# serviceberry3/weiner_slamit_v2

Measured on AMD Instinct MI355X. Metric: frames/sec ORB extract+match @640x480x8lvl, higher is better.
Workload: dtype u8; 1 GPU; BASELINE configs[1]: 640x480 8-level ORB extract (1000 features, FAST 20/7) + brute-force 256-bit Hamming best/second match vs the stream's previous frame; 256 independent streams per GPU per step; distinct_frame_pairs_per_gpu=16, parallelism=streams sharded over 1 GPU(s), no data-path collective

## Files before the change

include/slamit.h:

```cpp
#ifndef SLAMIT_H
#define SLAMIT_H

#include <stddef.h>
#include <stdint.h>

#ifdef __cplusplus
extern "C" {
#endif

#define SLAMIT_OK 0
#define SLAMIT_ERR_ARG (-1)
#define SLAMIT_ERR_DEVICE (-2)
#define SLAMIT_ERR_CAPACITY (-3)
#define SLAMIT_ERR_STATE (-4)

#define SLAMIT_DESC_BYTES 32
#define SLAMIT_EDGE_THRESHOLD 19

typedef struct slamit_kp {
    float x, y;
    float size;
    float angle;
    float response;
    int32_t octave;
    int32_t class_id;
} slamit_kp;


typedef struct slamit_orb_params {
    int32_t nfeatures;
    float scale_factor;
    int32_t nlevels;
    int32_t ini_th_fast;
    int32_t min_th_fast;
    int32_t width, height;
    int32_t max_batch;
} slamit_orb_params;

#define SLAMIT_MAX_LEVELS 16

typedef struct slamit_orb slamit_orb;

int slamit_orb_create(const slamit_orb_params* params, int device, slamit_orb** out);
void slamit_orb_destroy(slamit_orb* h);

int slamit_orb_tables(const slamit_orb* h, float* scale, float* inv_scale, float* sigma2,
                      float* inv_sigma2, int32_t* features_per_level);

int slamit_orb_max_keypoints(const slamit_orb* h);

int slamit_orb_extract(slamit_orb* h, const uint8_t* gray, size_t stride, slamit_kp* kps,
                       uint8_t* desc, int cap, int* n_out);

int slamit_orb_extract_batch(slamit_orb* h, const uint8_t* gray, size_t stride,
                             size_t frame_stride, int nframes, slamit_kp* kps, uint8_t* desc,
                             int cap, int* n_out);

int slamit_orb_extract_batch_dev(slamit_orb* h, const uint8_t* d_gray, size_t stride,
                                 size_t frame_stride, int nframes, slamit_kp* d_kps,
                                 uint8_t* d_desc, int cap, int32_t* d_n_out, void* stream);

#define SLAMIT_ORB_STAGES 6
int slamit_orb_profile(slamit_orb* h, int enable, float* stage_ms, int32_t* stage_calls, int nstages);

int slamit_orb_level(slamit_orb* h, int frame, int level, uint8_t* dst, size_t dst_bytes, int* w,
                     int* h_out);

int slamit_orb_debug_candidates(slamit_orb* h, int frame, int level, int32_t* xys, int cap,
                                int* n_out);
int slamit_orb_debug_blurred(slamit_orb* h, int frame, int level, uint8_t* dst, size_t dst_bytes, int* w,
                             int* h_out);


#define SLAMIT_HAMMING_MAX_TRAIN 65535
int slamit_hamming_best2(const uint8_t* q, int nq, const uint8_t* t, int nt, int32_t* best_idx,
                         int32_t* best, int32_t* second);

int slamit_hamming_best2_batch_dev(const uint8_t* d_q, const int32_t* d_nq, size_t q_stride,
                                   const uint8_t* d_t, const int32_t* d_nt, size_t t_stride,
                                   int npairs, int max_n, int32_t* d_best_idx, int32_t* d_best,
                                   int32_t* d_second, size_t out_stride, int device, void* stream);

#define SLAMIT_DISTINCTIVE_MAX 128
int slamit_distinctive_batch(const uint8_t* desc, const int32_t* offsets, int npoints, int32_t* best_idx,
                             int32_t* best_median);

typedef struct slamit_frame_view {
    int32_t n;
    const float* kp_xy;
    const int32_t* kp_octave;
    const uint8_t* desc;
    const uint8_t* kp_taken;
    float min_x, min_y;
    float inv_w, inv_h;
} slamit_frame_view;

typedef struct slamit_search_queries {
    int32_t m;
    const float* uvr;
    const int32_t* level_min;
    const int32_t* level_max;
    const uint8_t* desc;
    const uint8_t* valid;
    const uint8_t* takes;
} slamit_search_queries;

typedef struct slamit_search_rule {
    int32_t th_dist;
    int32_t use_ratio;
    float nnratio;
    float chi2_gate;
    float inv_level_sigma2[16];
    int32_t mode;
} slamit_search_rule;

#define SLAMIT_SEARCH_MAX_KP 8191
#define SLAMIT_SEARCH_MAX_CAND 1024
int slamit_guided_search(int device, const slamit_frame_view* frame, const slamit_search_queries* queries,
                         const slamit_search_rule* rule, int32_t* match_kp, int32_t* nmatches, int32_t* best_dist,
                         int32_t* best_level, int32_t* second_dist, int32_t* second_level);

typedef struct slamit_bow_groups {
    int32_t n_groups;
    const int32_t* q_ptr;
    const int32_t* q_idx;
    const int32_t* c_ptr;
    const int32_t* c_idx;
} slamit_bow_groups;

typedef struct slamit_bow_rule {
    int32_t mode;
    int32_t th;
    int32_t th_inclusive;
    float nnratio;
    float F12[9];
    float ex, ey;
    const float* kp1_xy;
    const float* kp2_xy;
    const int32_t* kp2_octave;
    float scale_factor[16];
    float level_sigma2[16];
} slamit_bow_rule;

#define SLAMIT_BOW_MAX_GROUP 2048
int slamit_bow_search(int device, const uint8_t* desc1, int32_t n1, const uint8_t* valid1, const uint8_t* desc2, int32_t n2,
                      const uint8_t* valid2, const slamit_bow_groups* groups, const slamit_bow_rule* rule, int32_t* match12,
                      int32_t* dist12, int32_t* nmatches);

#define SLAMIT_VOC_MAX_K 20
#define SLAMIT_VOC_MAX_L 10
#define SLAMIT_VOC_MAX_FEATURES 8191

typedef struct slamit_voc_desc {
    int32_t k, L;
    int32_t scoring;
    int32_t weighting;
    int32_t n_nodes;
    const int32_t* parent;
    const uint8_t* is_leaf;
    const uint8_t* desc;
    const double* weight;
} slamit_voc_desc;

typedef struct slamit_voc slamit_voc;

int slamit_voc_create(const slamit_voc_desc* desc, int device, slamit_voc** out);
int slamit_voc_load_text(const char* path, int device, slamit_voc** out);
void slamit_voc_destroy(slamit_voc* v);
int slamit_voc_info(const slamit_voc* v, int32_t* k, int32_t* L, int32_t* n_nodes, int32_t* n_words);

int slamit_voc_transform(const slamit_voc* v, const uint8_t* desc, int n, int levelsup, int32_t* word_id, int32_t* node_id,
                         int32_t* bow_n, int32_t* bow_word, double* bow_value, int32_t* fv_n, int32_t* fv_node,
                         int32_t* fv_ptr, int32_t* fv_items);

size_t slamit_voc_transform_workspace(int nframes, int cap);
int slamit_voc_transform_batch_dev(const slamit_voc* v, const uint8_t* d_desc, const int32_t* d_n, int cap, int nframes,
                                   int levelsup, int32_t* d_word_id, int32_t* d_node_id, int32_t* d_bow_n,
                                   int32_t* d_bow_word, double* d_bow_value, int32_t* d_fv_n, int32_t* d_fv_node,
                                   int32_t* d_fv_ptr, int32_t* d_fv_items, void* d_workspace, size_t workspace_bytes,
                                   void* stream);

typedef struct slamit_kfdb slamit_kfdb;

int slamit_kfdb_create(int max_kf, int max_words, int device, slamit_kfdb** out);
void slamit_kfdb_destroy(slamit_kfdb* db);
int slamit_kfdb_clear(slamit_kfdb* db);
int slamit_kfdb_info(const slamit_kfdb* db, int32_t* max_kf, int32_t* max_words, int32_t* n_live);
int slamit_kfdb_add(slamit_kfdb* db, const int32_t* bow_word, const double* bow_value, int n, int32_t* slot);
int slamit_kfdb_add_dev(slamit_kfdb* db, const int32_t* d_bow_n, const int32_t* d_bow_word, const double* d_bow_value,
                        void* stream, int32_t* slot);
int slamit_kfdb_erase(slamit_kfdb* db, int slot);
int slamit_kfdb_query(slamit_kfdb* db, const int32_t* bow_word, const double* bow_value, int n, int32_t* common,
                      int32_t* first_word, int64_t* seq, double* score);
int slamit_kfdb_query_batch_dev(slamit_kfdb* db, const int32_t* d_bow_n, const int32_t* d_bow_word, const double* d_bow_value,
                                int cap, int nq, int32_t* d_common, int32_t* d_first_word, double* d_score, void* stream);

typedef struct slamit_camera {
    float fx, fy, cx, cy;
    float k1, k2, p1, p2, k3;
} slamit_camera;

#define SLAMIT_FRAME_GRID_COLS 64
#define SLAMIT_FRAME_GRID_ROWS 48
#define SLAMIT_FRAME_GRID_CELLS (SLAMIT_FRAME_GRID_COLS * SLAMIT_FRAME_GRID_ROWS)
#define SLAMIT_FRAME_MAX_KP 30000

int slamit_undistort_points(int device, const slamit_camera* cam, const float* xy_in, int n, float* xy_out);

int slamit_frame_finish(int device, const slamit_camera* cam, const slamit_kp* kps, int n, float min_x, float min_y,
                        float inv_w, float inv_h, slamit_kp* kps_un, int32_t* cell_start, int32_t* cell_items);

int slamit_frame_finish_batch_dev(int device, const slamit_camera* cam, const slamit_kp* d_kps, const int32_t* d_n, int cap,
                                  int nframes, float min_x, float min_y, float inv_w, float inv_h, slamit_kp* d_kps_un,
                                  int32_t* d_cell_start, int32_t* d_cell_items, void* stream);

#define SLAMIT_SEARCH_BATCH_CAND 128
typedef struct slamit_search_batch {
    int32_t nframes, kp_cap, q_cap;
    const int32_t* d_n;
    const slamit_kp* d_kps_un;
    const uint8_t* d_desc;
    const uint8_t* d_kp_taken;
    float min_x, min_y, inv_w, inv_h;
    const int32_t* d_m;
// ... 256 lines not shown
```

weiner_slamit_v2_amd/api.py:

```python
import ctypes as C
import math
import os

import numpy as np

HERE = os.path.dirname(os.path.abspath(__file__))
LIB_PATH = os.environ.get("SLAMIT_LIB", os.path.join(HERE, "libslamit_hip.so"))

KP_DTYPE = np.dtype(
    [("x", "<f4"), ("y", "<f4"), ("size", "<f4"), ("angle", "<f4"), ("response", "<f4"),
     ("octave", "<i4"), ("class_id", "<i4")]
)

MAX_ITS = 32


class SlamitError(RuntimeError):
    pass


class OrbParams(C.Structure):
    _fields_ = [("nfeatures", C.c_int32), ("scale_factor", C.c_float), ("nlevels", C.c_int32),
                ("ini_th_fast", C.c_int32), ("min_th_fast", C.c_int32), ("width", C.c_int32),
                ("height", C.c_int32), ("max_batch", C.c_int32)]
# ... 18 lines not shown
                ("lambda_", (C.c_double * MAX_ITS) * 2), ("trials", (C.c_int32 * MAX_ITS) * 2),
                ("chi2_init", C.c_double * 2)]


class BaResult(C.Structure):
    _fields_ = [("kf_pose", C.c_void_p), ("pt_xyz", C.c_void_p), ("edge_chi2", C.c_void_p),
                ("edge_outlier", C.c_void_p), ("edge_stage1_outlier", C.c_void_p), ("stats", C.c_void_p)]


class FrameView(C.Structure):
    _fields_ = [("n", C.c_int32), ("kp_xy", C.c_void_p), ("kp_octave", C.c_void_p), ("desc", C.c_void_p),
                ("kp_taken", C.c_void_p), ("min_x", C.c_float), ("min_y", C.c_float), ("inv_w", C.c_float),
                ("inv_h", C.c_float)]


class SearchQueries(C.Structure):
    _fields_ = [("m", C.c_int32), ("uvr", C.c_void_p), ("level_min", C.c_void_p), ("level_max", C.c_void_p),
                ("desc", C.c_void_p), ("valid", C.c_void_p), ("takes", C.c_void_p)]


class SearchRule(C.Structure):
    _fields_ = [("th_dist", C.c_int32), ("use_ratio", C.c_int32), ("nnratio", C.c_float), ("chi2_gate", C.c_float),
                ("inv_level_sigma2", C.c_float * 16), ("mode", C.c_int32)]


def _search_rule(th_dist, use_ratio, nnratio, chi2_gate=0.0, inv_level_sigma2=None, mode=0):
    sig = [1.0] * 16
    if inv_level_sigma2 is not None:
        for i, v in enumerate(list(inv_level_sigma2)[:16]):
            sig[i] = float(v)
    return SearchRule(int(th_dist), int(bool(use_ratio)), float(nnratio), float(chi2_gate), (C.c_float * 16)(*sig), int(mode))


class BowGroups(C.Structure):
    _fields_ = [("n_groups", C.c_int32), ("q_ptr", C.c_void_p), ("q_idx", C.c_void_p), ("c_ptr", C.c_void_p), ("c_idx", C.c_void_p)]


class BowRule(C.Structure):
    _fields_ = [("mode", C.c_int32), ("th", C.c_int32), ("th_inclusive", C.c_int32), ("nnratio", C.c_float),
                ("F12", C.c_float * 9), ("ex", C.c_float), ("ey", C.c_float), ("kp1_xy", C.c_void_p), ("kp2_xy", C.c_void_p),
                ("kp2_octave", C.c_void_p), ("scale_factor", C.c_float * 16), ("level_sigma2", C.c_float * 16)]


class Sim3Problem(C.Structure):
    _fields_ = [("n", C.c_int32), ("p1", C.c_void_p), ("p2", C.c_void_p), ("obs1", C.c_void_p), ("obs2", C.c_void_p),
                ("inv_sigma2_1", C.c_void_p), ("inv_sigma2_2", C.c_void_p), ("intr1", C.c_double * 4), ("intr2", C.c_double * 4),
                ("r12", C.c_double * 9), ("t12", C.c_double * 3), ("s12", C.c_double), ("th2", C.c_double), ("fix_scale", C.c_int32)]


class Sim3Result(C.Structure):
    _fields_ = [("r12", C.c_double * 9), ("t12", C.c_double * 3), ("s12", C.c_double), ("inlier", C.c_void_p), ("n_inliers", C.c_int32),
                ("n_its", C.c_int32 * 2), ("chi2", C.c_double * 2)]


class Sim3RansacProblem(C.Structure):
    _fields_ = [("n", C.c_int32), ("x1", C.c_void_p), ("x2", C.c_void_p), ("max_err1", C.c_void_p), ("max_err2", C.c_void_p),
                ("intr1", C.c_float * 4), ("intr2", C.c_float * 4), ("fix_scale", C.c_int32), ("n_hyp", C.c_int32), ("triples", C.c_void_p)]


class Sim3RansacResult(C.Structure):
    _fields_ = [("t12", C.c_void_p), ("n_inliers", C.c_void_p), ("inlier_bits", C.c_void_p)]


SIM3_RANSAC_MAX_N, SIM3_RANSAC_MAX_HYP = 8192, 1024


class TriangulateProblem(C.Structure):
    _fields_ = [("Tcw1", C.c_float * 12), ("Tcw2", C.c_float * 12), ("intr1", C.c_float * 6), ("intr2", C.c_float * 6), ("n", C.c_int32),
                ("n_levels", C.c_int32), ("kp1_xy", C.c_void_p), ("kp2_xy", C.c_void_p), ("octave1", C.c_void_p), ("octave2", C.c_void_p),
                ("scale_factors1", C.c_void_p), ("level_sigma2_1", C.c_void_p), ("scale_factors2", C.c_void_p), ("level_sigma2_2", C.c_void_p),
                ("ratio_factor", C.c_float)]


class TriangulateResult(C.Structure):
    _fields_ = [("status", C.c_void_p), ("x3d", C.c_void_p), ("n_accepted", C.c_int32)]


TRIANGULATE_MAX_N, MAX_LEVELS = 8192, 16


class FrustumFrame(C.Structure):
    _fields_ = [("Rcw", C.c_float * 9), ("tcw", C.c_float * 3), ("Ow", C.c_float * 3), ("fx", C.c_float), ("fy", C.c_float), ("cx", C.c_float),
                ("cy", C.c_float), ("bf", C.c_float), ("min_x", C.c_float), ("max_x", C.c_float), ("min_y", C.c_float), ("max_y", C.c_float),
                ("view_cos_limit", C.c_float), ("log_scale_factor", C.c_float), ("th", C.c_float), ("n_levels", C.c_int32),
                ("scale_factors", C.c_float * 16)]


class FrustumProblem(C.Structure):
    _fields_ = [("frame", FrustumFrame), ("n", C.c_int32), ("pos", C.c_void_p), ("normal", C.c_void_p), ("max_dist", C.c_void_p),
                ("min_dist", C.c_void_p), ("skip", C.c_void_p)]


class FrustumResult(C.Structure):
    _fields_ = [("status", C.c_void_p), ("proj", C.c_void_p), ("view_cos", C.c_void_p), ("level", C.c_void_p), ("uvr", C.c_void_p),
                ("level_min", C.c_void_p), ("level_max", C.c_void_p), ("valid", C.c_void_p), ("n_in_view", C.c_int32)]


class FrustumBatchRec(C.Structure):
    _fields_ = [("nframes", C.c_int32), ("q_cap", C.c_int32), ("d_frames", C.c_void_p), ("d_m", C.c_void_p), ("d_pos", C.c_void_p),
                ("d_normal", C.c_void_p), ("d_max_dist", C.c_void_p), ("d_min_dist", C.c_void_p), ("d_skip", C.c_void_p), ("d_uvr", C.c_void_p),
                ("d_level_min", C.c_void_p), ("d_level_max", C.c_void_p), ("d_valid", C.c_void_p), ("d_status", C.c_void_p),
                ("d_proj", C.c_void_p), ("d_view_cos", C.c_void_p), ("d_level", C.c_void_p), ("d_n_in_view", C.c_void_p)]


FRUSTUM_MAX_N = 65536
FRUSTUM_FRAME_DTYPE = np.dtype([("Rcw", "<f4", 9), ("tcw", "<f4", 3), ("Ow", "<f4", 3), ("fx", "<f4"), ("fy", "<f4"), ("cx", "<f4"), ("cy", "<f4"),
                                ("bf", "<f4"), ("min_x", "<f4"), ("max_x", "<f4"), ("min_y", "<f4"), ("max_y", "<f4"), ("view_cos_limit", "<f4"),
                                ("log_scale_factor", "<f4"), ("th", "<f4"), ("n_levels", "<i4"), ("scale_factors", "<f4", 16)])


class VocDesc(C.Structure):
    _fields_ = [("k", C.c_int32), ("L", C.c_int32), ("scoring", C.c_int32), ("weighting", C.c_int32), ("n_nodes", C.c_int32),
                ("parent", C.c_void_p), ("is_leaf", C.c_void_p), ("desc", C.c_void_p), ("weight", C.c_void_p)]


VOC_MAX_K, VOC_MAX_L, VOC_MAX_FEATURES = 20, 10, 8191


class SearchBatch(C.Structure):
    _fields_ = [("nframes", C.c_int32), ("kp_cap", C.c_int32), ("q_cap", C.c_int32), ("d_n", C.c_void_p),
                ("d_kps_un", C.c_void_p), ("d_desc", C.c_void_p), ("d_kp_taken", C.c_void_p), ("min_x", C.c_float),
                ("min_y", C.c_float), ("inv_w", C.c_float), ("inv_h", C.c_float), ("d_m", C.c_void_p), ("d_uvr", C.c_void_p),
                ("d_level_min", C.c_void_p), ("d_level_max", C.c_void_p), ("d_qdesc", C.c_void_p), ("d_valid", C.c_void_p),
                ("d_takes", C.c_void_p)]


class Camera(C.Structure):
    _fields_ = [("fx", C.c_float), ("fy", C.c_float), ("cx", C.c_float), ("cy", C.c_float), ("k1", C.c_float),
                ("k2", C.c_float), ("p1", C.c_float), ("p2", C.c_float), ("k3", C.c_float)]


class BaProfile(C.Structure):
    _fields_ = [("phase_ms", C.c_double * 5), ("slots", C.c_int32), ("nwin", C.c_int32), ("schur_exec_mflop", C.c_double)]


BA_PHASES = ("linearize", "schur", "solve", "update", "residuals")


class PoseProblem(C.Structure):
    _fields_ = [("n", C.c_int32), ("pose", C.c_void_p), ("intr", C.c_void_p), ("xw", C.c_void_p),
                ("uv", C.c_void_p), ("inv_sigma2", C.c_void_p), ("ur", C.c_void_p), ("bf", C.c_double)]


class PoseResult(C.Structure):
    _fields_ = [("pose", C.c_void_p), ("outlier", C.c_void_p), ("n_inliers", C.c_int32),
                ("n_its", C.c_int32 * 4), ("chi2", C.c_double * 4)]


_lib = None

EXPORTS = [
    "slamit_orb_create", "slamit_orb_destroy", "slamit_orb_tables", "slamit_orb_max_keypoints",
    "slamit_orb_extract", "slamit_orb_extract_batch", "slamit_orb_extract_batch_dev", "slamit_orb_level",
    "slamit_orb_debug_candidates", "slamit_orb_debug_blurred", "slamit_orb_profile", "slamit_hamming_best2", "slamit_hamming_best2_batch_dev",
    "slamit_hamming_matrix", "slamit_distinctive_batch", "slamit_guided_search", "slamit_guided_search_workspace", "slamit_guided_search_batch_dev", "slamit_bow_search", "slamit_voc_create", "slamit_voc_load_text", "slamit_voc_destroy", "slamit_voc_info",
    "slamit_voc_transform", "slamit_voc_transform_workspace", "slamit_voc_transform_batch_dev",
    "slamit_kfdb_create", "slamit_kfdb_destroy", "slamit_kfdb_clear", "slamit_kfdb_info", "slamit_kfdb_add", "slamit_kfdb_add_dev", "slamit_kfdb_erase",
    "slamit_kfdb_query", "slamit_kfdb_query_batch_dev", "slamit_undistort_points", "slamit_frame_finish",
    "slamit_frame_finish_batch_dev", "slamit_ba_create", "slamit_ba_create_ex", "slamit_ba_destroy", "slamit_ba_solve",
    "slamit_ba_solve_batch", "slamit_ba_profile", "slamit_ba_profile_read", "slamit_pose_optimize", "slamit_pose_optimize_batch", "slamit_sim3_optimize", "slamit_sim3_optimize_batch", "slamit_sim3_ransac", "slamit_sim3_ransac_batch", "slamit_triangulate", "slamit_triangulate_batch", "slamit_frustum", "slamit_frustum_batch", "slamit_frustum_batch_dev", "slamit_last_error", "slamit_version", "slamit_device_count", "slamit_set_device", "slamit_release_thread_scratch",
]


def lib():
    global _lib
    if _lib is None:
        if not os.path.exists(LIB_PATH):
            raise SlamitError(
                "libslamit_hip.so is not built: run `python -m weiner_slamit_v2_amd.build` "
                "(there is no CPU fallback)")
        try:
            import torch
        except ImportError:
            pass
        L = C.CDLL(LIB_PATH)
        vp, i32, sz = C.c_void_p, C.c_int, C.c_size_t
        L.slamit_orb_create.argtypes = [C.POINTER(OrbParams), i32, C.POINTER(vp)]
        L.slamit_orb_destroy.argtypes = [vp]
        L.slamit_orb_destroy.restype = None
        L.slamit_orb_tables.argtypes = [vp] + [vp] * 5
        L.slamit_orb_max_keypoints.argtypes = [vp]
        L.slamit_orb_extract.argtypes = [vp, vp, sz, vp, vp, i32, vp]
        L.slamit_orb_extract_batch.argtypes = [vp, vp, sz, sz, i32, vp, vp, i32, vp]
        L.slamit_orb_extract_batch_dev.argtypes = [vp, vp, sz, sz, i32, vp, vp, i32, vp, vp]
        L.slamit_orb_level.argtypes = [vp, i32, i32, vp, sz, vp, vp]
        L.slamit_orb_debug_blurred.argtypes = [vp, i32, i32, vp, sz, vp, vp]
        L.slamit_orb_profile.argtypes = [vp, i32, vp, vp, i32]
        L.slamit_orb_debug_candidates.argtypes = [vp, i32, i32, vp, i32, vp]
        L.slamit_hamming_best2.argtypes = [vp, i32, vp, i32, vp, vp, vp]
        L.slamit_hamming_best2_batch_dev.argtypes = [vp, vp, sz, vp, vp, sz, i32, i32, vp, vp, vp, sz, i32, vp]
        L.slamit_hamming_matrix.argtypes = [vp, i32, vp, i32, vp]
        L.slamit_distinctive_batch.argtypes = [vp, vp, i32, vp, vp]
        L.slamit_guided_search.argtypes = [i32, C.POINTER(FrameView), C.POINTER(SearchQueries), C.POINTER(SearchRule),
                                           vp, vp, vp, vp, vp, vp]
        L.slamit_guided_search_workspace.argtypes = [i32, i32]
        L.slamit_guided_search_workspace.restype = sz
        L.slamit_guided_search_batch_dev.argtypes = [i32, C.POINTER(SearchBatch), C.POINTER(SearchRule), vp, vp, vp, vp, sz, vp]
        f32 = C.c_float
        L.slamit_sim3_optimize_batch.argtypes = [i32, i32, C.POINTER(Sim3Problem), C.POINTER(Sim3Result)]
        L.slamit_sim3_optimize.argtypes = [i32, C.POINTER(Sim3Problem), C.POINTER(Sim3Result)]
        L.slamit_sim3_ransac_batch.argtypes = [i32, i32, C.POINTER(Sim3RansacProblem), C.POINTER(Sim3RansacResult)]
        L.slamit_sim3_ransac.argtypes = [i32, C.POINTER(Sim3RansacProblem), C.POINTER(Sim3RansacResult)]
        L.slamit_triangulate_batch.argtypes = [i32, i32, C.POINTER(TriangulateProblem), C.POINTER(TriangulateResult)]
        L.slamit_triangulate.argtypes = [i32, C.POINTER(TriangulateProblem), C.POINTER(TriangulateResult)]
        L.slamit_frustum_batch.argtypes = [i32, i32, C.POINTER(FrustumProblem), C.POINTER(FrustumResult)]
        L.slamit_frustum.argtypes = [i32, C.POINTER(FrustumProblem), C.POINTER(FrustumResult)]
        L.slamit_frustum_batch_dev.argtypes = [i32, C.POINTER(FrustumBatchRec), vp]
        L.slamit_bow_search.argtypes = [i32, vp, i32, vp, vp, i32, vp, C.POINTER(BowGroups), C.POINTER(BowRule), vp, vp, vp]
        L.slamit_voc_create.argtypes = [C.POINTER(VocDesc), i32, C.POINTER(vp)]
        L.slamit_voc_load_text.argtypes = [C.c_char_p, i32, C.POINTER(vp)]
        L.slamit_voc_destroy.argtypes = [vp]
        L.slamit_voc_destroy.restype = None
        L.slamit_voc_info.argtypes = [vp, vp, vp, vp, vp]
        L.slamit_voc_transform.argtypes = [vp, vp, i32, i32] + [vp] * 9
        L.slamit_voc_transform_workspace.argtypes = [i32, i32]
        L.slamit_voc_transform_workspace.restype = sz
        L.slamit_voc_transform_batch_dev.argtypes = [vp, vp, vp, i32, i32, i32] + [vp] * 9 + [vp, sz, vp]
        L.slamit_kfdb_create.argtypes = [i32, i32, i32, C.POINTER(vp)]
        L.slamit_kfdb_destroy.argtypes = [vp]
        L.slamit_kfdb_destroy.restype = None
        L.slamit_kfdb_clear.argtypes = [vp]
        L.slamit_kfdb_info.argtypes = [vp, vp, vp, vp]
        L.slamit_kfdb_add.argtypes = [vp, vp, vp, i32, vp]
        L.slamit_kfdb_add_dev.argtypes = [vp, vp, vp, vp, vp, vp]
        L.slamit_kfdb_erase.argtypes = [vp, i32]
        L.slamit_kfdb_query.argtypes = [vp, vp, vp, i32, vp, vp, vp, vp]
        L.slamit_kfdb_query_batch_dev.argtypes = [vp, vp, vp, vp, i32, i32, vp, vp, vp, vp]
        L.slamit_undistort_points.argtypes = [i32, C.POINTER(Camera), vp, i32, vp]
        L.slamit_frame_finish.argtypes = [i32, C.POINTER(Camera), vp, i32, f32, f32, f32, f32, vp, vp, vp]
        L.slamit_frame_finish_batch_dev.argtypes = [i32, C.POINTER(Camera), vp, vp, i32, i32, f32, f32, f32, f32, vp, vp, vp, vp]
        if hasattr(L, "slamit_ba_create"):
            L.slamit_ba_create.argtypes = [i32, i32, i32, i32, i32, C.POINTER(vp)]
            if hasattr(L, "slamit_ba_create_ex"):
                L.slamit_ba_create_ex.argtypes = [i32, i32, i32, i32, i32, i32, C.POINTER(vp)]
            L.slamit_ba_destroy.argtypes = [vp]
            L.slamit_ba_destroy.restype = None
            L.slamit_ba_solve.argtypes = [vp, C.POINTER(BaProblem), C.POINTER(BaOpts), C.POINTER(BaResult)]
            L.slamit_ba_solve_batch.argtypes = [vp, i32, C.POINTER(BaProblem), C.POINTER(BaOpts), C.POINTER(BaResult)]
            if hasattr(L, "slamit_ba_profile"):
                L.slamit_ba_profile.argtypes = [vp, i32]
                L.slamit_ba_profile_read.argtypes = [vp, C.POINTER(BaProfile)]
        if hasattr(L, "slamit_pose_optimize_batch"):
            L.slamit_pose_optimize_batch.argtypes = [i32, i32, C.POINTER(PoseProblem), C.POINTER(PoseResult)]
            L.slamit_pose_optimize.argtypes = [i32, C.POINTER(PoseProblem), C.POINTER(PoseResult)]
        L.slamit_last_error.restype = C.c_char_p
        L.slamit_version.restype = C.c_char_p
        _lib = L
    return _lib


def _check(rc, what):
    if rc != 0:
        raise SlamitError("%s failed (%d): %s" % (what, rc, lib().slamit_last_error().decode()))


def device_count():
    return lib().slamit_device_count()


def _np_ptr(a):
    return a.ctypes.data_as(C.c_void_p)


class ORBextractor:

    def __init__(self, nfeatures=1000, scaleFactor=1.2, nlevels=8, iniThFAST=20, minThFAST=7,
                 device=0, max_batch=1):
        self.params = (int(nfeatures), float(scaleFactor), int(nlevels), int(iniThFAST), int(minThFAST))
        self.device = device
        self.max_batch = max_batch
        self._h = None
        self._geom = None

    def _bind(self, width, height, batch=1):
        if self._h is not None and self._geom == (width, height) and batch <= self.max_batch:
            return
        self.close()
        self.max_batch = max(self.max_batch, batch)
        p = OrbParams(self.params[0], self.params[1], self.params[2], self.params[3], self.params[4],
                      width, height, self.max_batch)
        h = C.c_void_p()
        _check(lib().slamit_orb_create(C.byref(p), self.device, C.byref(h)), "slamit_orb_create")
        self._h = h
        self._geom = (width, height)
        self.max_keypoints = lib().slamit_orb_max_keypoints(h)

    def close(self):
        if self._h is not None:
            lib().slamit_orb_destroy(self._h)
            self._h = None

    def __del__(self):
        try:
            self.close()
        except Exception:
            pass

    def GetLevels(self):
        return self.params[2]

    def GetScaleFactor(self):
        return self.params[1]

    def _tables(self):
        if self._h is None:
            self._bind(640, 480)
        n = self.params[2]
        out = [np.zeros(n, np.float32) for _ in range(4)] + [np.zeros(n, np.int32)]
        _check(lib().slamit_orb_tables(self._h, *[_np_ptr(a) for a in out]), "slamit_orb_tables")
        return out

    def GetScaleFactors(self):
        return self._tables()[0]

    def GetInverseScaleFactors(self):
        return self._tables()[1]

    def GetScaleSigmaSquares(self):
        return self._tables()[2]

    def GetInverseScaleSigmaSquares(self):
        return self._tables()[3]

    def features_per_level(self):
        return self._tables()[4]

    def __call__(self, image, mask=None):
        image = np.asarray(image)
        if image.size == 0:
            return np.zeros(0, KP_DTYPE), np.zeros((0, 32), np.uint8)
        assert image.dtype == np.uint8 and image.ndim == 2, "CV_8UC1 expected (ORBextractor.cc:1075)"
        k, d = self.extract_batch(image[None])
        return k[0], d[0]

    def extract_batch(self, frames):
        frames = np.ascontiguousarray(frames, dtype=np.uint8)
        b, hh, ww = frames.shape
        self._bind(ww, hh, b)
        cap = self.max_keypoints
        kps = np.zeros((b, cap), KP_DTYPE)
        desc = np.zeros((b, cap, 32), np.uint8)
        n = np.zeros(b, np.int32)
        _check(lib().slamit_orb_extract_batch(self._h, _np_ptr(frames), ww, ww * hh, b, _np_ptr(kps), _np_ptr(desc),
                                              cap, _np_ptr(n)), "slamit_orb_extract_batch")
        return [kps[i, :n[i]].copy() for i in range(b)], [desc[i, :n[i]].copy() for i in range(b)]

    def extract_batch_dev(self, d_frames, d_kps, d_desc, d_n, stream=None):
        b, hh, ww = d_frames.shape
        self._bind(ww, hh, b)
        cap = d_kps.shape[1]
        _check(lib().slamit_orb_extract_batch_dev(
            self._h, d_frames.data_ptr(), d_frames.stride(1), d_frames.stride(0), b, d_kps.data_ptr(),
            d_desc.data_ptr(), cap, d_n.data_ptr(), stream), "slamit_orb_extract_batch_dev")

    STAGES = ("resize", "fast", "octree", "angle", "blur", "describe")

    def profile(self, enable):
        ms = np.zeros(6, np.float32)
        calls = np.zeros(6, np.int32)
        _check(lib().slamit_orb_profile(self._h, int(enable), _np_ptr(ms), _np_ptr(calls), 6), "slamit_orb_profile")
        return {s: (float(ms[i]), int(calls[i])) for i, s in enumerate(self.STAGES)}

    def level(self, frame, level):
        w, h = C.c_int(), C.c_int()
        _check(lib().slamit_orb_level(self._h, frame, level, None, 0, C.byref(w), C.byref(h)), "slamit_orb_level")
        out = np.zeros((h.value + 38, w.value + 38), np.uint8)
        _check(lib().slamit_orb_level(self._h, frame, level, _np_ptr(out), out.size, C.byref(w), C.byref(h)),
               "slamit_orb_level")
        return out

    def blurred(self, frame, level):
        w, h = C.c_int(), C.c_int()
        _check(lib().slamit_orb_debug_blurred(self._h, frame, level, None, 0, C.byref(w), C.byref(h)), "slamit_orb_debug_blurred")
        out = np.zeros((h.value, w.value), np.uint8)
        _check(lib().slamit_orb_debug_blurred(self._h, frame, level, _np_ptr(out), out.size, C.byref(w), C.byref(h)),
               "slamit_orb_debug_blurred")
        return out

    def debug_candidates(self, frame, level):
        n = C.c_int()
        _check(lib().slamit_orb_debug_candidates(self._h, frame, level, None, 0, C.byref(n)), "debug_candidates")
        out = np.zeros((max(n.value, 1), 3), np.int32)
        _check(lib().slamit_orb_debug_candidates(self._h, frame, level, _np_ptr(out), n.value, C.byref(n)),
               "debug_candidates")
        return out[:n.value]


GRID_COLS, GRID_ROWS = 64, 48


class Frame:

    @staticmethod
    def undistort_points(cam9, xy, device=0):
        cam = Camera(*[float(v) for v in cam9])
        xy = np.ascontiguousarray(xy, np.float32).reshape(-1, 2)
        out = np.zeros_like(xy)
        _check(lib().slamit_undistort_points(device, C.byref(cam), _np_ptr(xy), len(xy), _np_ptr(out)), "slamit_undistort_points")
        return out

    @staticmethod
    def ComputeImageBounds(cam9, cols, rows, device=0):
        f32 = np.float32
        if f32(cam9[4]) != 0:
            m = Frame.undistort_points(cam9, [[0, 0], [cols, 0], [0, rows], [cols, rows]], device)
            b = (min(m[0, 0], m[2, 0]), max(m[1, 0], m[3, 0]), min(m[0, 1], m[1, 1]), max(m[2, 1], m[3, 1]))
        else:
            b = (f32(0), f32(cols), f32(0), f32(rows))
        b = tuple(f32(v) for v in b)
        return b + (f32(GRID_COLS) / f32(b[1] - b[0]), f32(GRID_ROWS) / f32(b[3] - b[2]))

    @staticmethod
    def finish(cam9, kps, min_x, min_y, inv_w, inv_h, device=0):
        cam = Camera(*[float(v) for v in cam9])
        kps = np.ascontiguousarray(kps)
        n = len(kps)
        un = np.zeros(max(n, 1), KP_DTYPE)
        start, items = np.zeros(GRID_COLS * GRID_ROWS + 1, np.int32), np.zeros(max(n, 1), np.int32)
        _check(lib().slamit_frame_finish(device, C.byref(cam), _np_ptr(kps), n, float(min_x), float(min_y), float(inv_w),
                                         float(inv_h), _np_ptr(un), _np_ptr(start), _np_ptr(items)), "slamit_frame_finish")
        return un[:n], start, items[:start[-1]]

    @staticmethod
    def finish_batch_dev(cam9, d_kps, d_n, min_x, min_y, inv_w, inv_h, d_kps_un, d_cell_start, d_cell_items, device=0, stream=None):
        cam = Camera(*[float(v) for v in cam9])
        b, cap = d_kps.shape[0], d_kps.shape[1]
        _check(lib().slamit_frame_finish_batch_dev(device, C.byref(cam), d_kps.data_ptr(), d_n.data_ptr(), cap, b, float(min_x),
                                                   float(min_y), float(inv_w), float(inv_h), d_kps_un.data_ptr(),
                                                   d_cell_start.data_ptr(), d_cell_items.data_ptr(), stream),
               "slamit_frame_finish_batch_dev")


class ORBmatcher:
    TH_HIGH = 100
    TH_LOW = 50
    HISTO_LENGTH = 30

    def __init__(self, nnratio=0.6, checkOri=True):
        self.mfNNratio = nnratio
        self.mbCheckOrientation = checkOri

    @staticmethod
    def DescriptorDistance(a, b):
        a = np.ascontiguousarray(a, np.uint8).reshape(1, 32)
        b = np.ascontiguousarray(b, np.uint8).reshape(1, 32)
        return int(ORBmatcher.distance_matrix(a, b)[0, 0])

    @staticmethod
    def distance_matrix(q, t):
        q = np.ascontiguousarray(q, np.uint8).reshape(-1, 32)
        t = np.ascontiguousarray(t, np.uint8).reshape(-1, 32)
        out = np.zeros((len(q), len(t)), np.uint16)
        _check(lib().slamit_hamming_matrix(_np_ptr(q), len(q), _np_ptr(t), len(t), _np_ptr(out)), "slamit_hamming_matrix")
        return out

    @staticmethod
    def best2(q, t):
        q = np.ascontiguousarray(q, np.uint8).reshape(-1, 32)
        t = np.ascontiguousarray(t, np.uint8).reshape(-1, 32)
        idx, best, second = (np.zeros(len(q), np.int32) for _ in range(3))
        _check(lib().slamit_hamming_best2(_np_ptr(q), len(q), _np_ptr(t), len(t), _np_ptr(idx), _np_ptr(best),
                                          _np_ptr(second)), "slamit_hamming_best2")
        return idx, best, second

    @staticmethod
    def distinctive(desc, offsets):
        desc = np.ascontiguousarray(desc, np.uint8).reshape(-1, 32)
        offsets = np.ascontiguousarray(offsets, np.int32)
        n = len(offsets) - 1
        idx, med = np.zeros(max(n, 1), np.int32), np.zeros(max(n, 1), np.int32)
        _check(lib().slamit_distinctive_batch(_np_ptr(desc), _np_ptr(offsets), n, _np_ptr(idx), _np_ptr(med)),
               "slamit_distinctive_batch")
        return idx[:n], med[:n]

    @staticmethod
    def guided_search(frame, queries, th_dist=100, use_ratio=True, nnratio=0.8, device=0, chi2_gate=0.0, inv_level_sigma2=None, mode=0):
        f = dict(kp_xy=np.ascontiguousarray(frame["kp_xy"], np.float32).reshape(-1, 2),
                 kp_octave=np.ascontiguousarray(frame["kp_octave"], np.int32),
                 desc=np.ascontiguousarray(frame["desc"], np.uint8).reshape(-1, 32),
                 kp_taken=np.ascontiguousarray(frame["kp_taken"], np.uint8))
        uvr = np.ascontiguousarray(queries["uvr"], np.float32).reshape(-1, 3)
        m, n = len(uvr), len(f["kp_xy"])
        q = dict(level_min=np.ascontiguousarray(queries["level_min"], np.int32),
                 level_max=np.ascontiguousarray(queries["level_max"], np.int32),
                 desc=np.ascontiguousarray(queries["desc"], np.uint8).reshape(-1, 32),
                 valid=np.ascontiguousarray(queries.get("valid", np.ones(m)), np.uint8),
                 takes=np.ascontiguousarray(queries.get("takes", np.ones(m)), np.uint8))
        for k, a in list(f.items())[1:]:
            if len(a) != n:
                raise SlamitError("guided_search: frame[%s] has %d rows, expected %d" % (k, len(a), n))
        for k, a in q.items():
            if len(a) != m:
                raise SlamitError("guided_search: queries[%s] has %d rows, expected %d" % (k, len(a), m))
        fv = FrameView(n, _np_ptr(f["kp_xy"]), _np_ptr(f["kp_octave"]), _np_ptr(f["desc"]), _np_ptr(f["kp_taken"]),
                       frame["min_x"], frame["min_y"], frame["inv_w"], frame["inv_h"])
        sq = SearchQueries(m, _np_ptr(uvr), _np_ptr(q["level_min"]), _np_ptr(q["level_max"]), _np_ptr(q["desc"]),
                           _np_ptr(q["valid"]), _np_ptr(q["takes"]))
        rule = _search_rule(th_dist, use_ratio, nnratio, chi2_gate, inv_level_sigma2, mode)
        match = np.full(max(m, 1), -1, np.int32)
        out4 = np.zeros((4, max(m, 1)), np.int32)
        nm = C.c_int32(0)
        _check(lib().slamit_guided_search(device, C.byref(fv), C.byref(sq), C.byref(rule), _np_ptr(match), C.byref(nm),
                                          _np_ptr(out4[0]), _np_ptr(out4[1]), _np_ptr(out4[2]), _np_ptr(out4[3])),
               "slamit_guided_search")
        return match[:m], nm.value, out4[:, :m].T.copy()

    @staticmethod
    def guided_search_batch_dev(t, bounds, th_dist=100, use_ratio=True, nnratio=0.8, device=0, stream=None, chi2_gate=0.0,
                                inv_level_sigma2=None):
        b, kp_cap, q_cap = t["kps_un"].shape[0], t["kps_un"].shape[1], t["uvr"].shape[1]
        sb = SearchBatch(b, kp_cap, q_cap, t["n"].data_ptr(), t["kps_un"].data_ptr(), t["desc"].data_ptr(), t["kp_taken"].data_ptr(),
                         float(bounds[0]), float(bounds[1]), float(bounds[2]), float(bounds[3]), t["m"].data_ptr(), t["uvr"].data_ptr(),
                         t["level_min"].data_ptr(), t["level_max"].data_ptr(), t["qdesc"].data_ptr(), t["valid"].data_ptr(),
                         t["takes"].data_ptr())
        rule = _search_rule(th_dist, use_ratio, nnratio, chi2_gate, inv_level_sigma2)
        out4 = t.get("out4")
        _check(lib().slamit_guided_search_batch_dev(device, C.byref(sb), C.byref(rule), t["match_kp"].data_ptr(), t["nmatches"].data_ptr(),
                                                    out4.data_ptr() if out4 is not None else None, t["workspace"].data_ptr(),
                                                    t["workspace"].numel(), stream), "slamit_guided_search_batch_dev")

    @staticmethod
    def guided_search_workspace(nframes, q_cap):
        return int(lib().slamit_guided_search_workspace(nframes, q_cap))

    @staticmethod
    def search_for_initialization(f1, prev_xy, f2, window=100, nnratio=0.9, th_low=50, device=0):
        o1 = np.ascontiguousarray(f1["kp_octave"], np.int32)
        n1 = len(o1)
        pv = np.ascontiguousarray(prev_xy, np.float32).reshape(-1, 2)
        q = dict(uvr=np.concatenate([pv, np.full((n1, 1), float(window), np.float32)], 1), level_min=np.zeros(n1, np.int32),
                 level_max=np.zeros(n1, np.int32), desc=f1["desc"], valid=(o1 <= 0).astype(np.uint8), takes=np.zeros(n1, np.uint8))
# ... 715 lines not shown
```

weiner_slamit_v2_amd/csrc/orb_api.hip:

```cpp
#include <hip/hip_runtime.h>
#include <math.h>
#include <stdio.h>
#include <stdlib.h>
#include <string.h>

#include <algorithm>
#include <vector>

#include "../../include/slamit.h"
#include "orb_plan.h"
#include "slamit_internal.h"

hipError_t orbk_upload_pattern(hipStream_t st);
void orbk_resize(hipStream_t st, const uint8_t* src, int sw, int sh, size_t sstride, size_t sframe,
                 uint8_t* dst, int dw, int dh, size_t dstride, size_t dframe, const int* xofs,
                 const short* ialpha, const int* yofs, const short* ibeta, int nframes);
void orbk_resize_rows4(hipStream_t st, const uint8_t* src, size_t sstride, size_t sframe, int sh, uint8_t* dst, int dw, int dh,
                       size_t dstride, size_t dframe, const uint32_t* d_col, const uint32_t* d_row, int nframes);
void orbk_resize_rows8(hipStream_t st, const uint8_t* src, size_t sstride, size_t sframe, int sh, uint8_t* dst, int dw, int dh,
                       size_t dstride, size_t dframe, const uint32_t* d_col8, const uint32_t* d_row, int nframes);
hipError_t orbk_pyramid_bands_prepare(int smem_bytes);
void orbk_pyramid_bands(hipStream_t st, const BandTab& tab, const uint8_t* d_tables, const BandRows* d_rows, int first, int last, int nbands,
                        const uint8_t* src, size_t sstride, size_t sframe, int sh, uint8_t* pyr, size_t pyr_frame, int tile0, int smem, int nframes);
hipError_t orbk_pyramid_prepare(int smem_bytes);
void orbk_pyramid(hipStream_t st, const OrbLevel* levels, int nlevels, const PyrBox* boxes, const PyrTabs* tabs,
                  int nregions, const uint8_t* img0, size_t img0_stride, size_t img0_frame, uint8_t* pyr, int bufA_bytes,
                  int smem_bytes, int nframes, int l_first, int l_last);
hipError_t orbk_fast_prepare(int max_wcell, int max_hcell);
void orbk_fast(hipStream_t st, const FastTab& tab, int nlevels, const uint32_t* d_cells, int cells_per_frame, const uint8_t* img0,
               size_t img0_stride, size_t img0_frame, const uint8_t* pyr, unsigned long long* cand,
               size_t cand_frame_stride, int* cand_count, int iniTh, int minTh, int max_wcell, int max_hcell, int nframes);
hipError_t orbk_octree_prepare(int node_cap, int key_cap);
void orbk_octree(hipStream_t st, const OrbLevel* levels, int nlevels, const unsigned long long* cand,
                 size_t cand_frame_stride, int* cand_count, uint32_t* ws_xy, uint16_t* ws_node,
                 OrbLevelKp* lkp, size_t kp_frame_stride, int* kp_count, int node_cap, int key_cap, int nframes,
                 int level_override);
void orbk_ic_angle(hipStream_t st, const OrbLevel* levels, int nlevels, const uint8_t* img0, size_t img0_stride,
                   size_t img0_frame, const uint8_t* pyr, OrbLevelKp* lkp, size_t kp_frame_stride,
                   const int* kp_count, int max_kp, int nframes);
void orbk_blur_stream(hipStream_t st, const OrbLevel* levels, const uint32_t* d_tiles, int ntiles, const uint8_t* img0,
                      size_t img0_stride, size_t img0_frame, const uint8_t* pyr, uint8_t* blur, int nframes, bool edge);
void orbk_blur(hipStream_t st, const OrbLevel* levels, const uint32_t* d_tiles, int total_tiles, const uint8_t* img0,
               size_t img0_stride, size_t img0_frame, const uint8_t* pyr, uint8_t* blur, int nframes);
void orbk_describe(hipStream_t st, const OrbLevel* levels, int nlevels, const uint8_t* blur,
                   const OrbLevelKp* lkp, size_t kp_frame_stride, const int* kp_count, slamit_kp* out_kps,
                   uint8_t* out_desc, int out_cap, int* out_n, int max_kp, int nframes);
void orbk_pad(hipStream_t st, const uint8_t* src, int w, int h, size_t sstride, uint8_t* dst);
void orbk_decode_candidates(hipStream_t st, const OrbLevel* levels, int level, const unsigned long long* K, int n,
                            unsigned long long* order_out, int* xys);

namespace {

inline size_t round_up(size_t v, size_t a) { return (v + a - 1) / a * a; }

}

#define ORB_BLUR_SPLIT 1

struct slamit_orb {
    slamit_orb_params p;
    int device;
    hipStream_t stream;
    hipStream_t stream_b;
    hipEvent_t ev_pyr, ev_mid, ev_blur;
    SlamitSwitches sw;
    int nlevels;
    OrbPlan pl;
    bool blur_stream_on;
    uint8_t* d_tables;
    const OrbLevel* d_levels;
    uint8_t* d_pyr;
    uint8_t* d_blur;
    unsigned long long* d_cand;
    uint32_t* d_ws_xy;
    uint16_t* d_ws_node;
    int* d_counts;
    bool counters_clean;
    OrbLevelKp* d_lkp;
    uint8_t* d_in;
    size_t d_in_stride, d_in_frame;
    slamit_kp* d_out_kps;
    uint8_t* d_out_desc;
    int* d_out_n;
    uint8_t* h_out;
    uint8_t* d_scratch;
    size_t scratch_bytes;
    int prof_on;
    long prof_call;
    std::vector<hipEvent_t> prof_ev;
    std::vector<int> prof_stage;
    const uint8_t* last_img0;
    size_t last_stride, last_frame;
    int last_nframes;
};

template <typename T>
static const T* dtab(const slamit_orb* h, size_t off) { return reinterpret_cast<const T*>(h->d_tables + off); }

static void orb_free(slamit_orb* h) {
    if (!h) return;
    SlamitDeviceGuard guard(h->device);
    hipFree(h->d_tables); hipFree(h->d_pyr); hipFree(h->d_blur); hipFree(h->d_cand); hipFree(h->d_ws_xy);
    hipFree(h->d_ws_node); hipFree(h->d_counts); hipFree(h->d_lkp); hipFree(h->d_in); hipFree(h->d_out_kps);
    hipFree(h->d_out_desc); hipFree(h->d_out_n); if (h->h_out) hipHostFree(h->h_out); hipFree(h->d_scratch);
    for (hipEvent_t e : h->prof_ev) hipEventDestroy(e);
    if (h->ev_pyr) hipEventDestroy(h->ev_pyr);
    if (h->ev_mid) hipEventDestroy(h->ev_mid);
    if (h->ev_blur) hipEventDestroy(h->ev_blur);
    if (h->stream_b) hipStreamDestroy(h->stream_b);
    if (h->stream) hipStreamDestroy(h->stream);
    delete h;
}

extern "C" {

int slamit_orb_create(const slamit_orb_params* p, int device, slamit_orb** out) {
    if (!p || !out) return slamit_fail(SLAMIT_ERR_ARG, "slamit_orb_create: null argument");
    *out = nullptr;
    if (p->nlevels < 1 || p->nlevels > ORB_MAX_LEVELS || p->nfeatures < 1 || !(p->scale_factor > 1.f) ||
        p->ini_th_fast < 1 || p->ini_th_fast > 255 || p->min_th_fast < 1 || p->min_th_fast > 255 ||
        p->width < 0 || p->height < 0 || p->max_batch < 1)
        return slamit_fail(SLAMIT_ERR_ARG, "slamit_orb_create: parameter out of range");
    SLAMIT_USE_DEVICE(device);
    slamit_orb* h = new slamit_orb();
    h->p = *p;
    h->device = device;
    h->sw = slamit_read_switches();
    const int nl = h->nlevels = p->nlevels;
    const char* why = "";
    if (!orb_plan(*p, OrbPlanOptions{h->sw.resize_no8}, h->pl, &why)) {
        delete h;
        return slamit_fail(SLAMIT_ERR_ARG, why);
    }
    const OrbPlan& P = h->pl;
    const bool empty = P.levels.empty();
    h->blur_stream_on = !empty && !h->sw.blur_no_stream;

    const size_t B = (size_t)p->max_batch;
    const size_t counts_bytes = sizeof(int) * ((ORB_CC_PAD + 1) * B * nl + 2 * ORB_CC_PAD);
    h->d_in_stride = round_up((size_t)std::max(p->width, 1), 64);
    h->d_in_frame = h->d_in_stride * std::max(p->height, 1);
    h->scratch_bytes = std::max<size_t>((size_t)(p->width + 38) * (p->height + 38),
                                        (sizeof(unsigned long long) + 3 * sizeof(int)) * (P.cand_frame_stride + 64));
    hipError_t e = hipSuccess;
#define ALLOC(ptr, bytes) if (e == hipSuccess) e = hipMalloc((void**)&(ptr), std::max<size_t>((bytes), 256))
    ALLOC(h->d_tables, P.table_bytes);
    ALLOC(h->d_pyr, P.pyr_frame_total * B);
    ALLOC(h->d_blur, P.blur_frame_total * B + 256);
    ALLOC(h->d_cand, sizeof(unsigned long long) * P.cand_frame_stride * B);
    ALLOC(h->d_ws_xy, sizeof(uint32_t) * P.cand_frame_stride * B);
    ALLOC(h->d_ws_node, sizeof(uint16_t) * P.cand_frame_stride * B);
    ALLOC(h->d_counts, counts_bytes);
    ALLOC(h->d_lkp, sizeof(OrbLevelKp) * P.kp_frame_stride * B);
    ALLOC(h->d_in, h->d_in_frame * B);
    ALLOC(h->d_out_kps, sizeof(slamit_kp) * (size_t)P.max_out * B);
    ALLOC(h->d_out_desc, (size_t)SLAMIT_DESC_BYTES * P.max_out * B);
    ALLOC(h->d_out_n, sizeof(int) * B);
    ALLOC(h->d_scratch, h->scratch_bytes);
#undef ALLOC
    if (e == hipSuccess) e = hipHostMalloc((void**)&h->h_out, 256 + (size_t)B * 256 + (sizeof(slamit_kp) + SLAMIT_DESC_BYTES) * (size_t)P.max_out * B, hipHostMallocDefault);
    if (e == hipSuccess) e = hipStreamCreateWithFlags(&h->stream, hipStreamNonBlocking);
    if (e == hipSuccess) e = hipStreamCreateWithFlags(&h->stream_b, hipStreamNonBlocking);
    if (e == hipSuccess) e = hipEventCreateWithFlags(&h->ev_pyr, hipEventDisableTiming);
    if (e == hipSuccess) e = hipEventCreateWithFlags(&h->ev_mid, hipEventDisableTiming);
    if (e == hipSuccess) e = hipEventCreateWithFlags(&h->ev_blur, hipEventDisableTiming);
    if (e == hipSuccess && P.table_bytes) {
        std::vector<uint8_t> img;
        orb_plan_image(P, h->d_tables, img);
        e = hipMemcpy(h->d_tables, img.data(), img.size(), hipMemcpyHostToDevice);
    }
    h->d_levels = dtab<OrbLevel>(h, P.levels_off);
    if (e == hipSuccess && P.pyr_regions) e = orbk_pyramid_prepare(P.pyr_smem);
    for (const OrbBandSeg& G : P.bands) if (e == hipSuccess) e = orbk_pyramid_bands_prepare(G.smem);
    if (e == hipSuccess) e = orbk_upload_pattern(h->stream);
    if (e == hipSuccess) e = orbk_octree_prepare(P.node_cap, P.oct_key_cap);
    if (e == hipSuccess && !empty) e = orbk_fast_prepare(P.max_wcell, P.max_hcell);
    if (e == hipSuccess) e = hipMemset(h->d_counts, 0, counts_bytes);
    if (e == hipSuccess) e = hipStreamSynchronize(h->stream);
    if (e != hipSuccess) {
        orb_free(h);
        return slamit_fail_hip(e, "slamit_orb_create");
    }
    *out = h;
    return SLAMIT_OK;
}
void slamit_orb_destroy(slamit_orb* h) { orb_free(h); }

int slamit_orb_tables(const slamit_orb* h, float* scale, float* inv_scale, float* sigma2, float* inv_sigma2,
                      int32_t* features_per_level) {
    if (!h) return slamit_fail(SLAMIT_ERR_ARG, "slamit_orb_tables: null handle");
    for (int i = 0; i < h->nlevels; ++i) {
        if (scale) scale[i] = h->pl.scale[i];
        if (inv_scale) inv_scale[i] = h->pl.inv_scale[i];
        if (sigma2) sigma2[i] = h->pl.sigma2[i];
        if (inv_sigma2) inv_sigma2[i] = h->pl.inv_sigma2[i];
        if (features_per_level) features_per_level[i] = h->pl.per_level[i];
    }
    return SLAMIT_OK;
}

int slamit_orb_max_keypoints(const slamit_orb* h) { return h ? h->pl.max_out : 0; }

enum { ST_RESIZE = 0, ST_FAST, ST_OCTREE, ST_ANGLE, ST_BLUR, ST_DESCRIBE, ST_COUNT };

static void prof_mark(slamit_orb* h, hipStream_t st, int stage, bool begin) {
    if (!h->prof_on || h->prof_ev.size() >= 2 * 16384) return;
    if (h->prof_on >= 2 && (stage != ST_FAST || h->prof_call % (h->prof_on - 1) != 0)) return;
    hipEvent_t e;
    if (hipEventCreate(&e) != hipSuccess) return;
    hipEventRecord(e, st);
    h->prof_ev.push_back(e);
    if (begin) h->prof_stage.push_back(stage);
}

int slamit_orb_extract_batch_dev(slamit_orb* h, const uint8_t* d_gray, size_t stride, size_t frame_stride,
                                 int nframes, slamit_kp* d_kps, uint8_t* d_desc, int cap, int32_t* d_n_out,
                                 void* stream) {
    if (!h || !d_n_out || nframes < 0) return slamit_fail(SLAMIT_ERR_ARG, "slamit_orb_extract_batch_dev: bad argument");
    if (nframes > h->p.max_batch) return slamit_fail(SLAMIT_ERR_CAPACITY, "slamit_orb_extract_batch_dev: nframes > max_batch");
    if (nframes == 0) return SLAMIT_OK;
    SLAMIT_USE_DEVICE(h->device);
    hipStream_t st = stream ? (hipStream_t)stream : h->stream;
    const int nl = h->nlevels;
    const OrbPlan& P = h->pl;
    if (h->p.width == 0 || h->p.height == 0) {
        HIP_TRY(hipMemsetAsync(d_n_out, 0, sizeof(int) * nframes, st));
        h->last_nframes = 0;
        return SLAMIT_OK;
    }
    if (!d_gray || !d_kps || !d_desc) return slamit_fail(SLAMIT_ERR_ARG, "slamit_orb_extract_batch_dev: null buffer");
    if (cap < P.max_out) return slamit_fail(SLAMIT_ERR_CAPACITY, "slamit_orb_extract_batch_dev: cap < slamit_orb_max_keypoints()");
    if (stride < (size_t)h->p.width || (nframes > 1 && frame_stride < stride * (size_t)h->p.height))
        return slamit_fail(SLAMIT_ERR_ARG, "slamit_orb_extract_batch_dev: stride smaller than the frame");
    if (stride >= ((size_t)1 << 24)) return slamit_fail(SLAMIT_ERR_ARG, "slamit_orb_extract_batch_dev: row pitch of 16 MiB or more");
    int* cand_count = h->d_counts;
    int* kp_count = h->d_counts + (size_t)h->p.max_batch * nl * ORB_CC_PAD;
    if (!h->counters_clean) HIP_TRY(hipMemsetAsync(h->d_counts, 0, sizeof(int) * (size_t)h->p.max_batch * nl * ORB_CC_PAD, st));
    h->counters_clean = false;
    const bool blur_src_aligned = ((((uintptr_t)d_gray) | stride | frame_stride) & 3) == 0;
    auto launch_blur = [&](hipStream_t bs, int l0, int l1) {
        auto strips = [&](const OrbStrips& S) { return dtab<uint32_t>(h, S.off) + 4 * (size_t)S.base[l0]; };
        auto nstrips = [&](const OrbStrips& S) { return S.base[l1] - S.base[l0]; };
        if (h->blur_stream_on && blur_src_aligned) {
            orbk_blur_stream(bs, h->d_levels, strips(P.blur_str), nstrips(P.blur_str), d_gray, stride, frame_stride, h->d_pyr, h->d_blur, nframes, false);
            orbk_blur_stream(bs, h->d_levels, strips(P.blur_edge), nstrips(P.blur_edge), d_gray, stride, frame_stride, h->d_pyr, h->d_blur, nframes, true);
        } else {
            orbk_blur(bs, h->d_levels, strips(P.blur_all), nstrips(P.blur_all), d_gray, stride, frame_stride, h->d_pyr, h->d_blur, nframes);
        }
    };
    prof_mark(h, st, ST_RESIZE, true);
    const bool src0_aligned = ((((uintptr_t)d_gray) | stride | frame_stride) & 3) == 0;
    const bool side = h->prof_on != 1;
    const bool early_blur = side && ORB_BLUR_SPLIT < nl - 1;
    int early_done = -1;
    auto fork_early_blur = [&](int l) -> hipError_t {
        hipError_t e = hipEventRecord(h->ev_mid, st);
        if (e == hipSuccess) e = hipStreamWaitEvent(h->stream_b, h->ev_mid, 0);
        if (e != hipSuccess) return e;
        launch_blur(h->stream_b, 0, l + 1);
        early_done = l;
        return hipSuccess;
    };
    if (!P.bands.empty() && src0_aligned) {
        for (const OrbBandSeg& G : P.bands) {
            const OrbLevel& S = P.levels[G.first];
            orbk_pyramid_bands(st, P.band_tab, h->d_tables, dtab<BandRows>(h, G.rows_off), G.first, G.last, G.nbands,
                               G.first == 0 ? d_gray : h->d_pyr + S.plane_off, G.first == 0 ? stride : (size_t)S.stride,
                               G.first == 0 ? frame_stride : P.pyr_frame_total, S.h, h->d_pyr, P.pyr_frame_total, G.tile0, G.smem, nframes);
            if (early_blur && G.last < nl - 1 && early_done < 0) HIP_TRY(fork_early_blur(G.last));
        }
    } else if (P.rows4_ok && src0_aligned) {
        for (int l = 1; l < nl; ++l) {
            const OrbLevel& S = P.levels[l - 1];
            const OrbLevel& D = P.levels[l];
            const uint8_t* src = l == 1 ? d_gray : h->d_pyr + S.plane_off;
            const OrbResizeTabs& T = P.rs[l];
            if (!T.col8.empty())
                orbk_resize_rows8(st, src, l == 1 ? stride : (size_t)S.stride, l == 1 ? frame_stride : P.pyr_frame_total, S.h,
                                  h->d_pyr + D.plane_off, D.w, D.h, (size_t)D.stride, P.pyr_frame_total, dtab<uint32_t>(h, T.col8_off),
                                  dtab<uint32_t>(h, T.row4_off), nframes);
            else
                orbk_resize_rows4(st, src, l == 1 ? stride : (size_t)S.stride, l == 1 ? frame_stride : P.pyr_frame_total, S.h,
                                  h->d_pyr + D.plane_off, D.w, D.h, (size_t)D.stride, P.pyr_frame_total, dtab<uint32_t>(h, T.col4_off),
                                  dtab<uint32_t>(h, T.row4_off), nframes);
            if (early_blur && l == ORB_BLUR_SPLIT) HIP_TRY(fork_early_blur(l));
        }
    } else if (P.pyr_regions) {
        orbk_pyramid(st, h->d_levels, nl, dtab<PyrBox>(h, P.boxes_off), dtab<PyrTabs>(h, P.tabs_off), P.pyr_regions, d_gray, stride, frame_stride,
                     h->d_pyr, P.pyr_bufA, P.pyr_smem, nframes, 0, nl - 1);
    } else {
        for (int l = 1; l < nl; ++l) {
            const OrbLevel& S = P.levels[l - 1];
            const OrbLevel& D = P.levels[l];
            const uint8_t* src = l == 1 ? d_gray : h->d_pyr + S.plane_off;
            size_t sstride = l == 1 ? stride : (size_t)S.stride;
            size_t sframe = l == 1 ? frame_stride : P.pyr_frame_total;
            const OrbResizeTabs& T = P.rs[l];
            orbk_resize(st, src, S.w, S.h, sstride, sframe, h->d_pyr + D.plane_off, D.w, D.h, (size_t)D.stride,
                        P.pyr_frame_total, dtab<int>(h, T.xofs_off), dtab<short>(h, T.ialpha_off), dtab<int>(h, T.yofs_off),
                        dtab<short>(h, T.ibeta_off), nframes);
        }
    }
    prof_mark(h, st, ST_RESIZE, false);
    prof_mark(h, st, ST_FAST, true);
    orbk_fast(st, P.fast, nl, dtab<uint32_t>(h, P.cells_off), (int)(P.cells.size() / 4), d_gray, stride, frame_stride, h->d_pyr, h->d_cand,
              P.cand_frame_stride, cand_count, h->p.ini_th_fast, h->p.min_th_fast, P.max_wcell, P.max_hcell, nframes);
    prof_mark(h, st, ST_FAST, false);
    if (side) {
        HIP_TRY(hipEventRecord(h->ev_pyr, st));
        HIP_TRY(hipStreamWaitEvent(h->stream_b, h->ev_pyr, 0));
        launch_blur(h->stream_b, early_done + 1, nl);
        HIP_TRY(hipEventRecord(h->ev_blur, h->stream_b));
    }
    prof_mark(h, st, ST_OCTREE, true);
    orbk_octree(st, h->d_levels, nl, h->d_cand, P.cand_frame_stride, cand_count, h->d_ws_xy, h->d_ws_node, h->d_lkp,
                P.kp_frame_stride, kp_count, P.node_cap, P.oct_key_cap, nframes, -1);
    prof_mark(h, st, ST_OCTREE, false);
    prof_mark(h, st, ST_ANGLE, true);
    orbk_ic_angle(st, h->d_levels, nl, d_gray, stride, frame_stride, h->d_pyr, h->d_lkp, P.kp_frame_stride, kp_count,
                  P.max_kp_level, nframes);
    prof_mark(h, st, ST_ANGLE, false);
    if (side) {
        HIP_TRY(hipStreamWaitEvent(st, h->ev_blur, 0));
    } else {
        prof_mark(h, st, ST_BLUR, true);
        launch_blur(st, 0, nl);
        prof_mark(h, st, ST_BLUR, false);
    }
    prof_mark(h, st, ST_DESCRIBE, true);
    orbk_describe(st, h->d_levels, nl, h->d_blur, h->d_lkp, P.kp_frame_stride, kp_count, d_kps, d_desc, cap, d_n_out,
                  P.max_kp_level, nframes);
    prof_mark(h, st, ST_DESCRIBE, false);
    ++h->prof_call;
    HIP_TRY(hipGetLastError());
    h->counters_clean = true;
    h->last_img0 = d_gray; h->last_stride = stride; h->last_frame = frame_stride; h->last_nframes = nframes;
    return SLAMIT_OK;
}

int slamit_orb_extract_batch(slamit_orb* h, const uint8_t* gray, size_t stride, size_t frame_stride, int nframes,
                             slamit_kp* kps, uint8_t* desc, int cap, int* n_out) {
    if (!h || !n_out || nframes < 0) return slamit_fail(SLAMIT_ERR_ARG, "slamit_orb_extract_batch: bad argument");
    if (nframes > h->p.max_batch) return slamit_fail(SLAMIT_ERR_CAPACITY, "slamit_orb_extract_batch: nframes > max_batch");
    if (nframes == 0) return SLAMIT_OK;
    if (h->p.width == 0 || h->p.height == 0) {
        for (int f = 0; f < nframes; ++f) n_out[f] = 0;
        return SLAMIT_OK;
    }
    if (!gray || !kps || !desc) return slamit_fail(SLAMIT_ERR_ARG, "slamit_orb_extract_batch: null buffer");
    if (cap < h->pl.max_out) return slamit_fail(SLAMIT_ERR_CAPACITY, "slamit_orb_extract_batch: cap < slamit_orb_max_keypoints()");
    SLAMIT_USE_DEVICE(h->device);
    const int W = h->p.width, H = h->p.height;
    for (int f = 0; f < nframes; ++f)
        HIP_TRY(hipMemcpy2DAsync(h->d_in + f * h->d_in_frame, h->d_in_stride, gray + (size_t)f * frame_stride, stride, W, H,
                                 hipMemcpyHostToDevice, h->stream));
    int rc = slamit_orb_extract_batch_dev(h, h->d_in, h->d_in_stride, h->d_in_frame, nframes, h->d_out_kps, h->d_out_desc,
                                          h->pl.max_out, h->d_out_n, h->stream);
    if (rc != SLAMIT_OK) return rc;
    const size_t o_k = ((sizeof(int) * (size_t)nframes + 255) & ~(size_t)255), kb = sizeof(slamit_kp) * (size_t)h->pl.max_out * nframes;
    const size_t o_d = (o_k + kb + 255) & ~(size_t)255, db = (size_t)SLAMIT_DESC_BYTES * h->pl.max_out * nframes;
    HIP_TRY(hipMemcpyAsync(h->h_out, h->d_out_n, sizeof(int) * nframes, hipMemcpyDeviceToHost, h->stream));
    HIP_TRY(hipMemcpyAsync(h->h_out + o_k, h->d_out_kps, kb, hipMemcpyDeviceToHost, h->stream));
    HIP_TRY(hipMemcpyAsync(h->h_out + o_d, h->d_out_desc, db, hipMemcpyDeviceToHost, h->stream));
    HIP_TRY(hipStreamSynchronize(h->stream));
    memcpy(n_out, h->h_out, sizeof(int) * nframes);
    for (int f = 0; f < nframes; ++f) {
        const int n = n_out[f];
        if (n > 0) {
            memcpy(kps + (size_t)f * cap, h->h_out + o_k + sizeof(slamit_kp) * (size_t)f * h->pl.max_out, sizeof(slamit_kp) * n);
            memcpy(desc + (size_t)f * cap * SLAMIT_DESC_BYTES, h->h_out + o_d + (size_t)SLAMIT_DESC_BYTES * f * h->pl.max_out, (size_t)SLAMIT_DESC_BYTES * n);
        }
    }
    return SLAMIT_OK;
}

int slamit_orb_extract(slamit_orb* h, const uint8_t* gray, size_t stride, slamit_kp* kps, uint8_t* desc, int cap,
                       int* n_out) {
    return slamit_orb_extract_batch(h, gray, stride, stride * (size_t)(h ? h->p.height : 0), 1, kps, desc, cap, n_out);
}

int slamit_orb_profile(slamit_orb* h, int enable, float* stage_ms, int32_t* stage_calls, int nstages) {
    if (!h) return slamit_fail(SLAMIT_ERR_ARG, "slamit_orb_profile: null handle");
    SLAMIT_USE_DEVICE(h->device);
    if (stage_ms || stage_calls) {
        for (int i = 0; i < nstages; ++i) { if (stage_ms) stage_ms[i] = 0.f; if (stage_calls) stage_calls[i] = 0; }
        for (size_t i = 0; i < h->prof_stage.size() && 2 * i + 1 < h->prof_ev.size(); ++i) {
            HIP_TRY(hipEventSynchronize(h->prof_ev[2 * i + 1]));
            float ms = 0.f;
            HIP_TRY(hipEventElapsedTime(&ms, h->prof_ev[2 * i], h->prof_ev[2 * i + 1]));
            int s = h->prof_stage[i];
            if (s < nstages) { if (stage_ms) stage_ms[s] += ms; if (stage_calls) stage_calls[s] += 1; }
        }
    }
    for (hipEvent_t e : h->prof_ev) hipEventDestroy(e);
    h->prof_ev.clear(); h->prof_stage.clear();
    h->prof_on = enable;
    h->prof_call = 0;
    return SLAMIT_OK;
}

int slamit_orb_level(slamit_orb* h, int frame, int level, uint8_t* dst, size_t dst_bytes, int* w, int* h_out) {
    if (!h || level < 0 || level >= h->nlevels) return slamit_fail(SLAMIT_ERR_ARG, "slamit_orb_level: bad level");
    if (h->p.width == 0 || h->p.height == 0) return slamit_fail(SLAMIT_ERR_STATE, "slamit_orb_level: empty image");
    const OrbLevel& L = h->pl.levels[level];
    if (w) *w = L.w;
    if (h_out) *h_out = L.h;
    if (!dst) return SLAMIT_OK;
    if (frame < 0 || frame >= h->last_nframes || !h->last_img0) return slamit_fail(SLAMIT_ERR_STATE, "slamit_orb_level: no such frame in the last extract call");
    size_t need = (size_t)(L.w + 38) * (L.h + 38);
    if (dst_bytes < need) return slamit_fail(SLAMIT_ERR_CAPACITY, "slamit_orb_level: dst too small");
    SLAMIT_USE_DEVICE(h->device);
    const uint8_t* src = level == 0 ? h->last_img0 + (size_t)frame * h->last_frame
                                    : h->d_pyr + L.plane_off + (size_t)frame * h->pl.pyr_frame_total;
    orbk_pad(h->stream, src, L.w, L.h, level == 0 ? h->last_stride : (size_t)L.stride, h->d_scratch);
    HIP_TRY(hipMemcpyAsync(dst, h->d_scratch, need, hipMemcpyDeviceToHost, h->stream));
    HIP_TRY(hipStreamSynchronize(h->stream));
    return SLAMIT_OK;
}

int slamit_orb_debug_blurred(slamit_orb* h, int frame, int level, uint8_t* dst, size_t dst_bytes, int* w, int* h_out) {
    if (!h || level < 0 || level >= h->nlevels) return slamit_fail(SLAMIT_ERR_ARG, "slamit_orb_debug_blurred: bad level");
    if (h->p.width == 0 || h->p.height == 0) return slamit_fail(SLAMIT_ERR_STATE, "slamit_orb_debug_blurred: empty image");
    const OrbLevel& L = h->pl.levels[level];
    if (w) *w = L.w;
    if (h_out) *h_out = L.h;
    if (!dst) return SLAMIT_OK;
    if (frame < 0 || frame >= h->last_nframes) return slamit_fail(SLAMIT_ERR_STATE, "slamit_orb_debug_blurred: no such frame in the last extract call");
    if (dst_bytes < (size_t)L.w * L.h) return slamit_fail(SLAMIT_ERR_CAPACITY, "slamit_orb_debug_blurred: dst too small");
    SLAMIT_USE_DEVICE(h->device);
    HIP_TRY(hipMemcpy2DAsync(dst, (size_t)L.w, h->d_blur + L.blur_off + (size_t)frame * h->pl.blur_frame_total, (size_t)L.stride, (size_t)L.w,
                             (size_t)L.h, hipMemcpyDeviceToHost, h->stream));
    HIP_TRY(hipStreamSynchronize(h->stream));
    return SLAMIT_OK;
}

int slamit_orb_debug_candidates(slamit_orb* h, int frame, int level, int32_t* xys, int cap, int* n_out) {
    if (!h || level < 0 || level >= h->nlevels || !n_out) return slamit_fail(SLAMIT_ERR_ARG, "slamit_orb_debug_candidates: bad argument");
    if (frame < 0 || frame >= h->last_nframes) return slamit_fail(SLAMIT_ERR_STATE, "slamit_orb_debug_candidates: no such frame");
    SLAMIT_USE_DEVICE(h->device);
    const OrbLevel& L = h->pl.levels[level];
    int n = 0;
    HIP_TRY(hipMemcpy(&n, h->d_counts + (size_t)(frame * h->nlevels + level) * ORB_CC_PAD + 1, sizeof(int), hipMemcpyDeviceToHost));
    n = std::min(n, L.cand_cap);
    *n_out = n;
    if (!xys || n == 0) return SLAMIT_OK;
    if (cap < n) return slamit_fail(SLAMIT_ERR_CAPACITY, "slamit_orb_debug_candidates: cap too small");
    unsigned long long* d_order = (unsigned long long*)h->d_scratch;
    int* d_xys = (int*)(d_order + round_up((size_t)n, 64));
    orbk_decode_candidates(h->stream, h->d_levels, level, h->d_cand + L.cand_off + (size_t)frame * h->pl.cand_frame_stride, n, d_order, d_xys);
    std::vector<unsigned long long> order(n);
    std::vector<int> raw(3 * (size_t)n);
    HIP_TRY(hipMemcpyAsync(order.data(), d_order, sizeof(unsigned long long) * n, hipMemcpyDeviceToHost, h->stream));
    HIP_TRY(hipMemcpyAsync(raw.data(), d_xys, sizeof(int) * 3 * n, hipMemcpyDeviceToHost, h->stream));
    HIP_TRY(hipStreamSynchronize(h->stream));
    std::vector<int> idx(n);
    for (int i = 0; i < n; ++i) idx[i] = i;
    std::sort(idx.begin(), idx.end(), [&](int a, int b) { return order[a] < order[b]; });
    for (int i = 0; i < n; ++i) { xys[3 * i] = raw[3 * idx[i]]; xys[3 * i + 1] = raw[3 * idx[i] + 1]; xys[3 * i + 2] = raw[3 * idx[i] + 2]; }
    return SLAMIT_OK;
}

}
```

weiner_slamit_v2_amd/csrc/orb_kernels.hip:

```cpp
#include <hip/hip_runtime.h>
#include <stdint.h>

#include <algorithm>

#include "orb_types.h"
#include "slamit_math.h"
#include "wave_ops.h"
#include "../../include/slamit.h"
#include "../../include/slamit_orb_pattern.h"

#define WAVE 64

__global__ __launch_bounds__(256) void resize_level_kernel(
    const uint8_t* __restrict__ src, int sw, int sh, size_t sstride, size_t sframe,
    uint8_t* __restrict__ dst, int dw, int dh, size_t dstride, size_t dframe,
    const int* __restrict__ xofs, const short* __restrict__ ialpha,
    const int* __restrict__ yofs, const short* __restrict__ ibeta) {
    const int x4 = (blockIdx.x * 64 + (threadIdx.x & 63)) * 4;
    const int y = blockIdx.y * 4 + (threadIdx.x >> 6);
    const int f = blockIdx.z;
    if (x4 >= dw || y >= dh) return;
    const uint8_t* S = src + (size_t)f * sframe;
    int sy = yofs[y];
    int sy0 = min(max(sy, 0), sh - 1), sy1 = min(max(sy + 1, 0), sh - 1);
    const uint8_t* S0 = S + (size_t)sy0 * sstride;
    const uint8_t* S1 = S + (size_t)sy1 * sstride;
    int b0 = ibeta[2 * y], b1 = ibeta[2 * y + 1];
    uint32_t out = 0;
#pragma unroll
    for (int i = 0; i < 4; ++i) {
        int x = x4 + i;
        if (x < dw) {
            int sx = xofs[x];
            int sx1 = min(sx + 1, sw - 1);
            int a0 = ialpha[2 * x], a1 = ialpha[2 * x + 1];
            int r0 = S0[sx] * a0 + S0[sx1] * a1;
            int r1 = S1[sx] * a0 + S1[sx1] * a1;
            int v = ((((b0 * (r0 >> 4)) >> 16) + ((b1 * (r1 >> 4)) >> 16) + 2) >> 2) & 0xFF;
            out |= (uint32_t)v << (8 * i);
        }
    }
    *reinterpret_cast<uint32_t*>(dst + (size_t)f * dframe + (size_t)y * dstride + x4) = out;
}

typedef unsigned short rs_us2 __attribute__((ext_vector_type(2)));
typedef unsigned rs_u3 __attribute__((ext_vector_type(3)));
__device__ __forceinline__ uint32_t rs_dot2(uint32_t taps, uint32_t alpha) {
    return __builtin_amdgcn_udot2(__builtin_bit_cast(rs_us2, taps), __builtin_bit_cast(rs_us2, alpha), 0u, false);
}

#define RS_RP 2

template <int RP>
__device__ __forceinline__ void rs_item(const int item, const uint8_t* S, const unsigned ss, const unsigned sbytes, uint8_t* D, const unsigned dstride,
                                        const uint4* __restrict__ coltab, const uint2* __restrict__ rowtab, const int ngroups,
                                        const unsigned inv_groups, const int dh) {
    const int yq = (int)__umulhi((unsigned)item, inv_groups);
    const int g = item - yq * ngroups;
    const uint8_t* ct = reinterpret_cast<const uint8_t*>(coltab) + 48u * (unsigned)g;
    const uint4 c0 = *reinterpret_cast<const uint4*>(ct), c1 = *reinterpret_cast<const uint4*>(ct + 16u);
    const uint32_t c2x = *reinterpret_cast<const uint32_t*>(ct + 32u);
    int yrow[2 * RP];
    uint2 rt[2 * RP];
    {
        const uint4* rp4 = reinterpret_cast<const uint4*>(reinterpret_cast<const uint8_t*>(rowtab) + 16u * (unsigned)(RP * yq));
#pragma unroll
        for (int r = 0; r < RP; ++r) {
            const uint4 v = rp4[r];
            rt[2 * r] = make_uint2(v.x, v.y); rt[2 * r + 1] = make_uint2(v.z, v.w);
        }
#pragma unroll
        for (int r = 0; r < 2 * RP; ++r) yrow[r] = min(2 * RP * yq + r, dh - 1);
    }
    const unsigned b = c0.x & 0xFFFFu, sh = (c0.x >> 16) & 3u, off1 = (c0.x >> 20) & 15u, off2 = (c0.x >> 24) & 15u;
    const uint32_t sel[4] = {c0.y, c0.z, c0.w, c1.x}, al[4] = {c1.y, c1.z, c1.w, c2x};
    uint32_t w[4 * RP][3];
    const __amdgpu_buffer_rsrc_t rsrc = __builtin_amdgcn_make_buffer_rsrc(const_cast<uint8_t*>(S), 0, sbytes, 0x00020000);
    (void)off1; (void)off2;
#pragma unroll
    for (int r = 0; r < 4 * RP; ++r) {
        const unsigned srow = (r & 1) ? (rt[r >> 1].x >> 16) : (rt[r >> 1].x & 0xFFFFu);
        const unsigned ro = __umul24(srow, ss) + b;
        const rs_u3 v = __builtin_amdgcn_raw_buffer_load_b96(rsrc, (int)ro, 0, 0);
        w[r][0] = v.x; w[r][1] = v.y; w[r][2] = v.z;
    }
#pragma unroll
    for (int k = 0; k < 2 * RP; ++k) {
        uint32_t h[2][4];
#pragma unroll
        for (int r = 0; r < 2; ++r) {
            const uint32_t lo = __builtin_amdgcn_alignbyte(w[2 * k + r][1], w[2 * k + r][0], sh), hi = __builtin_amdgcn_alignbyte(w[2 * k + r][2], w[2 * k + r][1], sh);
#pragma unroll
            for (int j = 0; j < 4; ++j) h[r][j] = rs_dot2(__builtin_amdgcn_perm(hi, lo, sel[j]), al[j]) >> 4;
        }
        const unsigned b0 = rt[k].y & 0xFFFFu, b1 = rt[k].y >> 16;
        uint32_t out = 0;
#pragma unroll
        for (int j = 0; j < 4; ++j) {
            const uint32_t v = ((__umul24(b0, h[0][j]) >> 16) + (__umul24(b1, h[1][j]) >> 16) + 2u) >> 2;
            out |= (v & 0xFFu) << (8 * j);
        }
        *reinterpret_cast<uint32_t*>(D + (__umul24((unsigned)yrow[k], dstride) + 4u * (unsigned)g)) = out;
    }
}

template <int RP>
__global__ __launch_bounds__(256) void resize_rows4_kernel(
    const uint8_t* __restrict__ src, size_t sstride, size_t sframe,
    uint8_t* __restrict__ dst, size_t dstride, size_t dframe,
    const uint4* __restrict__ coltab, const uint2* __restrict__ rowtab, int ngroups, unsigned inv_groups, int nitems, int dh, unsigned sbytes) {
    const int item = blockIdx.x * 256 + threadIdx.x;
    if (item >= nitems) return;
    rs_item<RP>(item, src + (size_t)blockIdx.y * sframe, (unsigned)sstride, sbytes, dst + (size_t)blockIdx.y * dframe, (unsigned)dstride, coltab, rowtab,
                ngroups, inv_groups, dh);
}

typedef unsigned rs_u4 __attribute__((ext_vector_type(4)));
template <int RP>
__device__ __forceinline__ void rs_item8(const int item, const uint8_t* S, const unsigned ss, const unsigned sbytes, uint8_t* D, const unsigned dstride,
                                         const uint4* __restrict__ coltab, const uint2* __restrict__ rowtab, const int ngroups,
                                         const unsigned inv_groups, const int dh) {
    const int yq = (int)__umulhi((unsigned)item, inv_groups);
    const int g = item - yq * ngroups;
    const uint8_t* ct = reinterpret_cast<const uint8_t*>(coltab) + 80u * (unsigned)g;
    const uint4 c0 = *reinterpret_cast<const uint4*>(ct), c1 = *reinterpret_cast<const uint4*>(ct + 16u), c2 = *reinterpret_cast<const uint4*>(ct + 32u),
                c3 = *reinterpret_cast<const uint4*>(ct + 48u);
    const uint32_t c4x = *reinterpret_cast<const uint32_t*>(ct + 64u);
    int yrow[2 * RP];
    uint2 rt[2 * RP];
    {
        const uint4* rp4 = reinterpret_cast<const uint4*>(reinterpret_cast<const uint8_t*>(rowtab) + 16u * (unsigned)(RP * yq));
#pragma unroll
        for (int r = 0; r < RP; ++r) {
            const uint4 v = rp4[r];
            rt[2 * r] = make_uint2(v.x, v.y); rt[2 * r + 1] = make_uint2(v.z, v.w);
        }
#pragma unroll
        for (int r = 0; r < 2 * RP; ++r) yrow[r] = min(2 * RP * yq + r, dh - 1);
    }
    const unsigned b = c0.x & 0xFFFFu, sh = (c0.x >> 16) & 3u;
    const uint32_t sel[8] = {c0.y, c0.z, c0.w, c1.x, c1.y, c1.z, c1.w, c2.x}, al[8] = {c2.y, c2.z, c2.w, c3.x, c3.y, c3.z, c3.w, c4x};
    uint32_t w[4 * RP][4];
    const __amdgpu_buffer_rsrc_t rsrc = __builtin_amdgcn_make_buffer_rsrc(const_cast<uint8_t*>(S), 0, sbytes, 0x00020000);
#pragma unroll
    for (int r = 0; r < 4 * RP; ++r) {
        const unsigned srow = (r & 1) ? (rt[r >> 1].x >> 16) : (rt[r >> 1].x & 0xFFFFu);
        const unsigned ro = __umul24(srow, ss) + b;
        const rs_u4 v = __builtin_amdgcn_raw_buffer_load_b128(rsrc, (int)ro, 0, 0);
        w[r][0] = v.x; w[r][1] = v.y; w[r][2] = v.z; w[r][3] = v.w;
    }
#pragma unroll
    for (int k = 0; k < 2 * RP; ++k) {
        uint32_t h[2][8];
#pragma unroll
        for (int r = 0; r < 2; ++r) {
            const uint32_t* ww = w[2 * k + r];
            const uint32_t a0 = __builtin_amdgcn_alignbyte(ww[1], ww[0], sh), a1 = __builtin_amdgcn_alignbyte(ww[2], ww[1], sh), a2 = __builtin_amdgcn_alignbyte(ww[3], ww[2], sh);
#pragma unroll
            for (int j = 0; j < 4; ++j) h[r][j] = rs_dot2(__builtin_amdgcn_perm(a1, a0, sel[j]), al[j]) >> 4;
#pragma unroll
            for (int j = 4; j < 8; ++j) h[r][j] = rs_dot2(__builtin_amdgcn_perm(a2, a1, sel[j]), al[j]) >> 4;
        }
        const unsigned b0 = rt[k].y & 0xFFFFu, b1 = rt[k].y >> 16;
        uint32_t out[2] = {0, 0};
#pragma unroll
        for (int j = 0; j < 8; ++j) {
            const uint32_t v = ((__umul24(b0, h[0][j]) >> 16) + (__umul24(b1, h[1][j]) >> 16) + 2u) >> 2;
            out[j >> 2] |= (v & 0xFFu) << (8 * (j & 3));
        }
        *reinterpret_cast<uint2*>(D + (__umul24((unsigned)yrow[k], dstride) + 8u * (unsigned)g)) = make_uint2(out[0], out[1]);
    }
}

template <int RP>
__global__ __launch_bounds__(256) void resize_rows8_kernel(
    const uint8_t* __restrict__ src, size_t sstride, size_t sframe,
    uint8_t* __restrict__ dst, size_t dstride, size_t dframe,
    const uint4* __restrict__ coltab, const uint2* __restrict__ rowtab, int ngroups, unsigned inv_groups, int nitems, int dh, unsigned sbytes) {
    const int item = blockIdx.x * 256 + threadIdx.x;
    if (item >= nitems) return;
    rs_item8<RP>(item, src + (size_t)blockIdx.y * sframe, (unsigned)sstride, sbytes, dst + (size_t)blockIdx.y * dframe, (unsigned)dstride, coltab, rowtab,
                 ngroups, inv_groups, dh);
}

void orbk_resize_rows8(hipStream_t st, const uint8_t* src, size_t sstride, size_t sframe, int sh, uint8_t* dst, int dw, int dh,
                       size_t dstride, size_t dframe, const uint32_t* d_col8, const uint32_t* d_row, int nframes) {
    const int ng = (dw + 7) / 8, nitems = ng * ((dh + 2 * RS_RP - 1) / (2 * RS_RP));
    const unsigned inv = (unsigned)((0x100000000ull + (unsigned)ng - 1) / (unsigned)ng);
    hipLaunchKernelGGL(resize_rows8_kernel<RS_RP>, dim3((nitems + 255) / 256, nframes), dim3(256), 0, st, src, sstride, sframe, dst, dstride, dframe,
                       reinterpret_cast<const uint4*>(d_col8), reinterpret_cast<const uint2*>(d_row), ng, inv, nitems, dh, (unsigned)(sstride * (size_t)sh));
}

void orbk_resize_rows4(hipStream_t st, const uint8_t* src, size_t sstride, size_t sframe, int sh, uint8_t* dst, int dw, int dh,
                       size_t dstride, size_t dframe, const uint32_t* d_col, const uint32_t* d_row, int nframes) {
    const int ng = (dw + 3) / 4, nitems = ng * ((dh + 2 * RS_RP - 1) / (2 * RS_RP));
    const unsigned inv = (unsigned)((0x100000000ull + (unsigned)ng - 1) / (unsigned)ng);
    hipLaunchKernelGGL(resize_rows4_kernel<RS_RP>, dim3((nitems + 255) / 256, nframes), dim3(256), 0, st, src, sstride, sframe, dst, dstride, dframe,
                       reinterpret_cast<const uint4*>(d_col), reinterpret_cast<const uint2*>(d_row), ng, inv, nitems, dh, (unsigned)(sstride * (size_t)sh));
}

#define BAND_THREADS 256

template <bool FROM_LDS, bool TO_LDS>
__device__ __forceinline__ void band_item(const int item, const BandLevel& V, const uint8_t* __restrict__ tables, const BandRows R,
                                          const __amdgpu_buffer_rsrc_t rsrc, const unsigned ss, const uint8_t* stile, const int srow0,
                                          const unsigned spitch, uint8_t* dtile, uint8_t* D) {
    const int yq = (int)__umulhi((unsigned)item, V.inv_groups);
    const int g = item - yq * V.ngroups;
    const uint8_t* ct = tables + V.col_off + 80u * (unsigned)g;
    const uint4 c0 = *reinterpret_cast<const uint4*>(ct), c1 = *reinterpret_cast<const uint4*>(ct + 16u), c2 = *reinterpret_cast<const uint4*>(ct + 32u),
                c3 = *reinterpret_cast<const uint4*>(ct + 48u);
    const uint32_t c4x = *reinterpret_cast<const uint32_t*>(ct + 64u);
    int yrow[4];
    uint2 rt[4];
    const uint8_t* rtab = tables + V.row_off;
#pragma unroll
    for (int r = 0; r < 4; ++r) {
        yrow[r] = min((int)R.cmp0 + 4 * yq + r, (int)R.cmp1 - 1);
        rt[r] = *reinterpret_cast<const uint2*>(rtab + 8u * (unsigned)yrow[r]);
    }
    const unsigned b = c0.x & 0xFFFFu, sh = (c0.x >> 16) & 3u;
    const uint32_t sel[8] = {c0.y, c0.z, c0.w, c1.x, c1.y, c1.z, c1.w, c2.x}, al[8] = {c2.y, c2.z, c2.w, c3.x, c3.y, c3.z, c3.w, c4x};
    uint32_t w[8][4];
#pragma unroll
    for (int r = 0; r < 8; ++r) {
        const unsigned srow = (r & 1) ? (rt[r >> 1].x >> 16) : (rt[r >> 1].x & 0xFFFFu);
        if (FROM_LDS) {
            const uint32_t* p = reinterpret_cast<const uint32_t*>(stile + (__umul24(srow - (unsigned)srow0, spitch) + b));
            w[r][0] = p[0]; w[r][1] = p[1]; w[r][2] = p[2]; w[r][3] = p[3];
        } else {
            const rs_u4 v = __builtin_amdgcn_raw_buffer_load_b128(rsrc, (int)(__umul24(srow, ss) + b), 0, 0);
            w[r][0] = v.x; w[r][1] = v.y; w[r][2] = v.z; w[r][3] = v.w;
        }
    }
#pragma unroll
    for (int k = 0; k < 4; ++k) {
        uint32_t h[2][8];
#pragma unroll
        for (int r = 0; r < 2; ++r) {
            const uint32_t* ww = w[2 * k + r];
            const uint32_t a0 = __builtin_amdgcn_alignbyte(ww[1], ww[0], sh), a1 = __builtin_amdgcn_alignbyte(ww[2], ww[1], sh), a2 = __builtin_amdgcn_alignbyte(ww[3], ww[2], sh);
#pragma unroll
            for (int j = 0; j < 4; ++j) h[r][j] = rs_dot2(__builtin_amdgcn_perm(a1, a0, sel[j]), al[j]) >> 4;
#pragma unroll
            for (int j = 4; j < 8; ++j) h[r][j] = rs_dot2(__builtin_amdgcn_perm(a2, a1, sel[j]), al[j]) >> 4;
        }
        const unsigned b0 = rt[k].y & 0xFFFFu, b1 = rt[k].y >> 16;
        uint32_t out[2] = {0, 0};
#pragma unroll
        for (int j = 0; j < 8; ++j) {
            const uint32_t v = ((__umul24(b0, h[0][j]) >> 16) + (__umul24(b1, h[1][j]) >> 16) + 2u) >> 2;
            out[j >> 2] |= (v & 0xFFu) << (8 * (j & 3));
        }
        if (TO_LDS) *reinterpret_cast<uint2*>(dtile + (__umul24((unsigned)(yrow[k] - (int)R.cmp0), (unsigned)V.pitch) + 8u * (unsigned)g)) = make_uint2(out[0], out[1]);
        if (yrow[k] >= (int)R.own0 && yrow[k] < (int)R.own1)
            *reinterpret_cast<uint2*>(D + (__umul24((unsigned)yrow[k], (unsigned)V.dstride) + 8u * (unsigned)g)) = make_uint2(out[0], out[1]);
    }
}

__global__ __launch_bounds__(BAND_THREADS) void pyramid_bands_kernel(
    const BandTab tab, const uint8_t* __restrict__ tables, const BandRows* __restrict__ rows, const int first, const int last, const int nbands,
    const uint8_t* __restrict__ src, const unsigned sstride, const size_t sframe, const unsigned sbytes,
    uint8_t* __restrict__ pyr, const size_t pyr_frame, const int tile0, const int xcd_frames) {
    extern __shared__ __attribute__((aligned(16))) uint8_t band_lds[];
    int frame, band;
    if (xcd_frames) {
        const unsigned w = blockIdx.x, k = w >> 3, fq = k / (unsigned)nbands;
        frame = (int)(8u * fq + ((w + fq) & 7u));
        if (frame >= xcd_frames) return;
        band = (int)(k - fq * (unsigned)nbands);
    } else { band = blockIdx.x; frame = blockIdx.y; }
    const int nlv = last - first;
    const BandRows* BR = rows + (size_t)band * nlv;
    const __amdgpu_buffer_rsrc_t rsrc = __builtin_amdgcn_make_buffer_rsrc(const_cast<uint8_t*>(src + (size_t)frame * sframe), 0, sbytes, 0x00020000);
    uint8_t* planes = pyr + (size_t)frame * pyr_frame;
    int srow0 = 0;
    for (int k = 0; k < nlv; ++k) {
        const BandLevel& V = tab.lv[first + 1 + k];
        const BandRows R = BR[k];
        uint8_t* dtile = band_lds + ((k & 1) ? tile0 : 0);
        const uint8_t* stile = band_lds + ((k & 1) ? 0 : tile0);
        const unsigned spitch = (unsigned)tab.lv[first + k].pitch;
        uint8_t* D = planes + V.plane_off;
        const int nitems = V.ngroups * (((int)R.cmp1 - (int)R.cmp0 + 3) >> 2);
        const bool to_lds = k + 1 < nlv;
        for (int item = threadIdx.x; item < nitems; item += BAND_THREADS) {
            if (k == 0) {
                if (to_lds) band_item<false, true>(item, V, tables, R, rsrc, sstride, stile, srow0, spitch, dtile, D);
                else band_item<false, false>(item, V, tables, R, rsrc, sstride, stile, srow0, spitch, dtile, D);
            } else {
                if (to_lds) band_item<true, true>(item, V, tables, R, rsrc, sstride, stile, srow0, spitch, dtile, D);
                else band_item<true, false>(item, V, tables, R, rsrc, sstride, stile, srow0, spitch, dtile, D);
            }
        }
        srow0 = R.cmp0;
        if (to_lds) __syncthreads();
    }
}

void orbk_pyramid_bands(hipStream_t st, const BandTab& tab, const uint8_t* d_tables, const BandRows* d_rows, int first, int last, int nbands,
                        const uint8_t* src, size_t sstride, size_t sframe, int sh, uint8_t* pyr, size_t pyr_frame, int tile0, int smem, int nframes) {
    const int xcd_frames = nframes >= 16 ? nframes : 0;
    const dim3 grid = xcd_frames ? dim3((unsigned)(((nframes + 7) / 8) * 8) * (unsigned)nbands) : dim3(nbands, nframes);
    hipLaunchKernelGGL(pyramid_bands_kernel, grid, dim3(BAND_THREADS), smem, st, tab, d_tables, d_rows, first, last, nbands, src, (unsigned)sstride, sframe,
                       (unsigned)(sstride * (size_t)sh), pyr, pyr_frame, tile0, xcd_frames);
}

hipError_t orbk_pyramid_bands_prepare(int smem_bytes) {
    static int prepared = 0;
    if (smem_bytes <= prepared) return hipSuccess;
    prepared = smem_bytes;
    return hipFuncSetAttribute(reinterpret_cast<const void*>(pyramid_bands_kernel), hipFuncAttributeMaxDynamicSharedMemorySize, smem_bytes);
}

#define PYR_THREADS 512

__global__ __launch_bounds__(PYR_THREADS) void pyramid_fused_kernel(
    const OrbLevel* __restrict__ levels, int nlevels, const PyrBox* __restrict__ boxes,
    const PyrTabs* __restrict__ tabs, const uint8_t* __restrict__ img0, size_t img0_stride, size_t img0_frame,
    uint8_t* __restrict__ pyr, int bufA_bytes, int l_first, int l_last) {
    extern __shared__ __attribute__((aligned(16))) uint8_t pbuf[];
    uint8_t* buf[2] = {pbuf, pbuf + bufA_bytes};
    const int tx = threadIdx.x & 63, ty = threadIdx.x >> 6;
    const int PYR_ROWS = blockDim.x >> 6, NT = blockDim.x;
    const int frame = blockIdx.y;
    const PyrBox* B = boxes + (size_t)blockIdx.x * nlevels;
    {
        const PyrBox b = B[l_first];
        const int nw = b.nx1 - b.nx0, pitch = (nw + 3) & ~3;
        const uint8_t* S;
        size_t sstride;
        if (l_first == 0) { S = img0 + (size_t)frame * img0_frame; sstride = img0_stride; }
        else { S = pyr + levels[l_first].plane_off + (size_t)frame * levels[l_first].plane_bytes; sstride = (size_t)levels[l_first].stride; }
        const bool aligned = ((((uintptr_t)S) | sstride) & 3) == 0;
        const int w0 = levels[l_first].w;
        if (aligned) {
            const int nd = pitch >> 2;
            for (int y = b.ny0 + ty; y < b.ny1; y += PYR_ROWS)
                for (int d = tx; d < nd; d += 64) {
                    const int x = b.nx0 + 4 * d;
                    uint32_t v;
                    if (x + 4 <= w0) v = *reinterpret_cast<const uint32_t*>(S + (size_t)y * sstride + x);
                    else { v = 0; for (int j = 0; j < 4; ++j) if (x + j < w0) v |= (uint32_t)S[(size_t)y * sstride + x + j] << (8 * j); }
                    *reinterpret_cast<uint32_t*>(&buf[0][(y - b.ny0) * pitch + 4 * d]) = v;
                }
        } else {
            for (int y = b.ny0 + ty; y < b.ny1; y += PYR_ROWS)
                for (int x = b.nx0 + tx; x < b.nx1; x += 64)
                    buf[0][(y - b.ny0) * pitch + (x - b.nx0)] = S[(size_t)y * sstride + x];
        }
    }
    __syncthreads();
    for (int l = l_first + 1; l <= l_last; ++l) {
        const PyrBox b = B[l], pb = B[l - 1];
        const OrbLevel& L = levels[l];
        const int sw = levels[l - 1].w, sh = levels[l - 1].h;
        const PyrTabs T = tabs[l];
        const uint8_t* src = buf[(l - 1 - l_first) & 1];
        uint8_t* dst = buf[(l - l_first) & 1];
        const int spitch = ((pb.nx1 - pb.nx0) + 3) & ~3, dpitch = ((b.nx1 - b.nx0) + 3) & ~3;
        uint8_t* plane = pyr + L.plane_off + (size_t)frame * L.plane_bytes;
        const int nw = b.nx1 - b.nx0;
        int cx0[4], cx1[4], ca0[4], ca1[4];
        unsigned ownmask = 0;
#pragma unroll
        for (int j = 0; j < 4; ++j) {
            const int x = b.nx0 + tx + 64 * j;
            if (tx + 64 * j < nw) {
                const int sx = T.xofs[x];
                cx0[j] = sx - pb.nx0;
                cx1[j] = min(sx + 1, sw - 1) - pb.nx0;
                ca0[j] = T.ialpha[2 * x];
                ca1[j] = T.ialpha[2 * x + 1];
                if (x >= b.ox0 && x < b.ox1) ownmask |= 1u << j;
            } else { cx0[j] = cx1[j] = 0; ca0[j] = ca1[j] = 0; }
        }
        __shared__ int s_sy0[256], s_sy1[256], s_b01[256];
        const int nh = b.ny1 - b.ny0;
        for (int i = threadIdx.x; i < nh; i += NT) {
            const int y = b.ny0 + i, sy = T.yofs[y];
            s_sy0[i] = min(max(sy, 0), sh - 1) - pb.ny0;
            s_sy1[i] = min(max(sy + 1, 0), sh - 1) - pb.ny0;
            s_b01[i] = (int)(unsigned short)T.ibeta[2 * y] | ((int)T.ibeta[2 * y + 1] << 16);
        }
        __syncthreads();
        const int wy = __builtin_amdgcn_readfirstlane(ty);
        for (int y = b.ny0 + wy; y < b.ny1; y += PYR_ROWS) {
            const int sy0 = s_sy0[y - b.ny0], sy1 = s_sy1[y - b.ny0];
            const int b01 = s_b01[y - b.ny0];
            const int b0 = (short)(b01 & 0xFFFF), b1 = b01 >> 16;
            const uint8_t* S0 = src + sy0 * spitch;
            const uint8_t* S1 = src + sy1 * spitch;
            const bool own_y = y >= b.oy0 && y < b.oy1;
            uint8_t* drow = dst + (y - b.ny0) * dpitch + tx;
            uint8_t* prow = plane + (size_t)y * L.stride + b.nx0 + tx;
#pragma unroll
            for (int j = 0; j < 4; ++j) {
                if (tx + 64 * j < nw) {
                    const int r0 = S0[cx0[j]] * ca0[j] + S0[cx1[j]] * ca1[j];
                    const int r1 = S1[cx0[j]] * ca0[j] + S1[cx1[j]] * ca1[j];
                    const int v = ((((b0 * (r0 >> 4)) >> 16) + ((b1 * (r1 >> 4)) >> 16) + 2) >> 2) & 0xFF;
                    drow[64 * j] = (uint8_t)v;
                    if (own_y && ((ownmask >> j) & 1)) prow[64 * j] = (uint8_t)v;
                }
            }
        }
        __syncthreads();
    }
}
// ... 884 lines not shown

__device__ __forceinline__ int reflect101(int p, int len) {
    p = p < 0 ? -p : p;
    p = p >= len ? 2 * len - 2 - p : p;
    return min(max(p, 0), len - 1);
}


typedef unsigned short blur_us2 __attribute__((ext_vector_type(2)));
__device__ __forceinline__ uint32_t udot2(uint32_t a, uint32_t b, uint32_t c) {
    return __builtin_amdgcn_udot2(__builtin_bit_cast(blur_us2, a), __builtin_bit_cast(blur_us2, b), c, false);
}

__device__ __forceinline__ uint32_t blur_fetch(const uint8_t* S, unsigned sstride, bool whole, int w, int h, int gx0, int row) {
    const unsigned ro = (unsigned)reflect101(row, h) * sstride;
    if (whole) return *reinterpret_cast<const uint32_t*>(S + (ro + (unsigned)gx0));
    if (gx0 >= w + 3) return 0u;
    uint32_t v = 0;
#pragma unroll
    for (int j = 0; j < 4; ++j) v |= (uint32_t)S[ro + (unsigned)reflect101(gx0 + j, w)] << (8 * j);
    return v;
}

struct BlurCol { unsigned a0, a1, sel; };
__device__ __forceinline__ BlurCol blur_col(int g, int w, unsigned ss) {
#define BLUR_SEL(i0, i1, i2, i3) ((unsigned)(i0) | ((unsigned)(i1) << 8) | ((unsigned)(i2) << 16) | ((unsigned)(i3) << 24))
    BlurCol c;
    if (g < 0) { c.a0 = 0u; c.a1 = 4u; c.sel = BLUR_SEL(4, 3, 2, 1); }
    else if (g + 4 <= w) { c.a0 = c.a1 = (unsigned)g; c.sel = BLUR_SEL(0, 1, 2, 3); }
    else if (g < w) {
        const int q = w - g;
        unsigned idx[4];
#pragma unroll
        for (int j = 0; j < 4; ++j) idx[j] = (unsigned)(j < q ? 4 + j : 2 * q + 2 - j);
        c.a0 = (unsigned)(g - 4); c.a1 = (unsigned)g; c.sel = BLUR_SEL(idx[0], idx[1], idx[2], idx[3]);
    } else if (g <= w + 2) {
        const int t = g - w, gb = (w - 4) & ~3;
        unsigned idx[4];
#pragma unroll
        for (int j = 0; j < 4; ++j) idx[j] = j <= 2 - t ? (unsigned)(w - 2 - t - j - gb) : 0x0Cu;
        c.a0 = (unsigned)gb; c.a1 = min((unsigned)gb + 4u, ss - 4u); c.sel = BLUR_SEL(idx[0], idx[1], idx[2], idx[3]);
    } else { c.a0 = c.a1 = 0u; c.sel = BLUR_SEL(0x0C, 0x0C, 0x0C, 0x0C); }
#undef BLUR_SEL
    return c;
}
__device__ __forceinline__ uint32_t blur_fetch2(const uint8_t* S, unsigned ss, int h, int row, const BlurCol c) {
    const unsigned ro = __umul24((unsigned)reflect101(row, h), ss);
    return __builtin_amdgcn_perm(*reinterpret_cast<const uint32_t*>(S + (ro + c.a1)), *reinterpret_cast<const uint32_t*>(S + (ro + c.a0)), c.sel);
}

template <bool INTERIOR>
__device__ __forceinline__ void blur_strip(uint8_t (*in)[72], uint32_t (*rp)[64], const uint8_t* S, const size_t sstride, const bool aligned,
                                           uint8_t* D, const unsigned dstride, const int w, const int h, const int bx, const int by0, const int tid) {
    const int i0 = tid, i1 = tid + 256;
    const bool has1 = i1 < 22 * 18;
    const int r0 = i0 / 18, r1 = i1 / 18;
    const int g0 = bx - 4 + 4 * (i0 - r0 * 18), g1 = bx - 4 + 4 * (i1 - r1 * 18);
    const bool whole0 = aligned && g0 >= 0 && g0 + 4 <= w, whole1 = aligned && g1 >= 0 && g1 + 4 <= w;
    uint32_t* const st0 = reinterpret_cast<uint32_t*>(&in[r0][4 * (i0 - r0 * 18)]);
    uint32_t* const st1 = reinterpret_cast<uint32_t*>(&in[has1 ? r1 : 0][has1 ? 4 * (i1 - r1 * 18) : 0]);
    const unsigned ss = (unsigned)sstride;
    const BlurCol bc0 = blur_col(g0, w, ss), bc1 = blur_col(g1, w, ss);
    uint32_t v0 = INTERIOR ? *reinterpret_cast<const uint32_t*>(S + (__umul24((unsigned)(by0 + r0 - 3), ss) + (unsigned)g0))
                           : aligned ? blur_fetch2(S, ss, h, by0 + r0 - 3, bc0) : blur_fetch(S, ss, whole0, w, h, g0, by0 + r0 - 3);
    uint32_t v1 = !has1 ? 0u : INTERIOR ? *reinterpret_cast<const uint32_t*>(S + (__umul24((unsigned)(by0 + r1 - 3), ss) + (unsigned)g1))
                                        : aligned ? blur_fetch2(S, ss, h, by0 + r1 - 3, bc1) : blur_fetch(S, ss, whole1, w, h, g1, by0 + r1 - 3);
    *st0 = v0;
    if (has1) *st1 = v1;
    __syncthreads();
    const uint32_t TA = 18u | (34u << 8) | (49u << 16) | (55u << 24), TB = 49u | (34u << 8) | (18u << 16);
    const int cy = tid >> 4, cx4 = (tid & 15) * 4;
    const bool odd = cy & 1;
    const uint32_t k0 = odd ? (18u << 16) : (18u | (34u << 16)), k1 = odd ? (34u | (49u << 16)) : (49u | (55u << 16));
    const uint32_t k2 = odd ? (55u | (49u << 16)) : (49u | (34u << 16)), k3 = odd ? (34u | (18u << 16)) : 18u;
#pragma unroll 1
    for (int s = 0; s < BLUR_STEPS; ++s) {
        const int by = by0 + 16 * s;
        const bool more = s + 1 < BLUR_STEPS && (INTERIOR || by + 16 < h);
        if (more) {
            if (INTERIOR) {
                v0 = *reinterpret_cast<const uint32_t*>(S + (__umul24((unsigned)(by + 16 + r0 - 3), ss) + (unsigned)g0));
                if (has1) v1 = *reinterpret_cast<const uint32_t*>(S + (__umul24((unsigned)(by + 16 + r1 - 3), ss) + (unsigned)g1));
            } else {
                if (aligned) {
                    v0 = blur_fetch2(S, ss, h, by + 16 + r0 - 3, bc0);
                    if (has1) v1 = blur_fetch2(S, ss, h, by + 16 + r1 - 3, bc1);
                } else {
                    v0 = blur_fetch(S, ss, whole0, w, h, g0, by + 16 + r0 - 3);
                    if (has1) v1 = blur_fetch(S, ss, whole1, w, h, g1, by + 16 + r1 - 3);
                }
            }
        }
        if (tid < 11 * 16) {
            const int p = tid >> 4, c = (tid & 15) * 4;
            uint32_t o[2][4];
#pragma unroll
            for (int rr = 0; rr < 2; ++rr) {
                const uint32_t* pw = reinterpret_cast<const uint32_t*>(&in[2 * p + rr][c]);
                const uint32_t w0 = pw[0], w1 = pw[1], w2 = pw[2];
                o[rr][0] = __builtin_amdgcn_udot4(__builtin_amdgcn_alignbyte(w2, w1, 1), TB, __builtin_amdgcn_udot4(__builtin_amdgcn_alignbyte(w1, w0, 1), TA, 0u, false), false);
                o[rr][1] = __builtin_amdgcn_udot4(__builtin_amdgcn_alignbyte(w2, w1, 2), TB, __builtin_amdgcn_udot4(__builtin_amdgcn_alignbyte(w1, w0, 2), TA, 0u, false), false);
                o[rr][2] = __builtin_amdgcn_udot4(__builtin_amdgcn_alignbyte(w2, w1, 3), TB, __builtin_amdgcn_udot4(__builtin_amdgcn_alignbyte(w1, w0, 3), TA, 0u, false), false);
                o[rr][3] = __builtin_amdgcn_udot4(w2, TB, __builtin_amdgcn_udot4(w1, TA, 0u, false), false);
            }
            *reinterpret_cast<uint4*>(&rp[p][c]) = make_uint4(o[0][0] | (o[1][0] << 16), o[0][1] | (o[1][1] << 16),
                                                               o[0][2] | (o[1][2] << 16), o[0][3] | (o[1][3] << 16));
        }
        __syncthreads();
        if (more) {
            *st0 = v0;
            if (has1) *st1 = v1;
        }
        if (INTERIOR || (bx + cx4 < w && by + cy < h)) {
            const int pb = cy >> 1;
            const uint4 a0 = *reinterpret_cast<const uint4*>(&rp[pb][cx4]), a1 = *reinterpret_cast<const uint4*>(&rp[pb + 1][cx4]);
            const uint4 a2 = *reinterpret_cast<const uint4*>(&rp[pb + 2][cx4]), a3 = *reinterpret_cast<const uint4*>(&rp[pb + 3][cx4]);
#define BLUR_COL(f) min((udot2(a3.f, k3, udot2(a2.f, k2, udot2(a1.f, k1, udot2(a0.f, k0, 1u << 15)))) >> 16), 255u)
            const uint32_t out = BLUR_COL(x) | (BLUR_COL(y) << 8) | (BLUR_COL(z) << 16) | (BLUR_COL(w) << 24);
#undef BLUR_COL
            *reinterpret_cast<uint32_t*>(D + (__umul24((unsigned)(by + cy), dstride) + (unsigned)(bx + cx4))) = out;
        }
        if (!more) break;
        __syncthreads();
    }
}

__global__ __launch_bounds__(256) void blur_all_kernel(
    const OrbLevel* __restrict__ levels, const uint4* __restrict__ tiles,
    const uint8_t* __restrict__ img0, size_t img0_stride, size_t img0_frame,
    const uint8_t* __restrict__ pyr, uint8_t* __restrict__ blur, unsigned ntiles, unsigned inv_tiles, unsigned total) {
    __shared__ __attribute__((aligned(16))) uint8_t in[22][72];
    __shared__ __attribute__((aligned(16))) uint32_t rp[11][64];
    const int tid = threadIdx.x;
    const unsigned lin = blockIdx.x, per_xcd = (total + 7u) >> 3;
    const unsigned logical = (lin & 7u) * per_xcd + (lin >> 3);
    if (logical >= total) return;
    int frame = (int)__umulhi(logical, inv_tiles);
    if ((unsigned)frame * ntiles > logical) --frame;
    const uint4 tt = tiles[logical - (unsigned)frame * ntiles];
    const int level = (int)tt.x, bx = (int)tt.y, by0 = (int)tt.z;
    const OrbLevel& L = levels[level];
    const int w = L.w, h = L.h;
    const uint8_t* S;
    size_t sstride;
    if (level == 0) { S = img0 + (size_t)frame * img0_frame; sstride = img0_stride; }
    else { S = pyr + L.plane_off + (size_t)frame * L.plane_bytes; sstride = (size_t)L.stride; }
    const bool aligned = ((((uintptr_t)S) | sstride) & 3) == 0;
    uint8_t* D = blur + L.blur_off + (size_t)frame * L.blur_bytes;
    const bool interior = aligned && bx >= 4 && bx + 68 <= w && by0 >= 3 && by0 + ORB_BLUR_STRIP_H + 3 <= h;
    if (interior) blur_strip<true>(in, rp, S, sstride, aligned, D, (unsigned)L.stride, w, h, bx, by0, tid);
    else blur_strip<false>(in, rp, S, sstride, aligned, D, (unsigned)L.stride, w, h, bx, by0, tid);
}

template <bool EDGE>
__global__ __launch_bounds__(256) void blur_stream_kernel(
    const OrbLevel* __restrict__ levels, const uint4* __restrict__ tiles,
    const uint8_t* __restrict__ img0, size_t img0_stride, size_t img0_frame,
    const uint8_t* __restrict__ pyr, uint8_t* __restrict__ blur, unsigned ntiles) {
    const unsigned tile = blockIdx.x * 16u + (threadIdx.x >> 4);
    if (tile >= ntiles) return;
    const int frame = blockIdx.y;
    const uint4 tt = tiles[tile];
    const int level = (int)tt.x, by0 = (int)tt.z;
    const int x0 = (int)tt.y + 4 * (int)(threadIdx.x & 15);
    const OrbLevel& L = levels[level];
    const int h = L.h;
    const uint8_t* S;
    unsigned ss;
    if (level == 0) { S = img0 + (size_t)frame * img0_frame; ss = (unsigned)img0_stride; }
    else { S = pyr + L.plane_off + (size_t)frame * L.plane_bytes; ss = (unsigned)L.stride; }
    if (EDGE && x0 >= L.w) return;
    BlurCol bc[3];
    if (EDGE) {
#pragma unroll
        for (int k = 0; k < 3; ++k) bc[k] = blur_col(x0 - 4 + 4 * k, L.w, ss);
    } else S += x0 - 4;
    uint8_t* D = blur + L.blur_off + (size_t)frame * L.blur_bytes + x0;
    const unsigned ds = (unsigned)L.stride;
    const uint32_t TA = 18u | (34u << 8) | (49u << 16) | (55u << 24), TB = 49u | (34u << 8) | (18u << 16);
    const uint32_t kA0 = 18u | (34u << 16), kA1 = 49u | (55u << 16), kA2 = 49u | (34u << 16), kA3 = 18u;
    const uint32_t kB0 = 18u << 16, kB1 = 34u | (49u << 16), kB2 = 55u | (49u << 16), kB3 = 34u | (18u << 16);
    const int ylast = min(by0 + ORB_BLUR_STRIP_H, h) - 1;
    const int p0 = (by0 - 3) >> 1, p1 = (ylast + 3) >> 1;
    typedef unsigned blur_u3 __attribute__((ext_vector_type(3)));
    auto fetch = [&](int yy) -> blur_u3 {
        int r = yy < 0 ? -yy : yy;
        r = r >= h ? 2 * h - 2 - r : r;
        r = min(max(r, 0), h - 1);
        if (EDGE) {
            const uint8_t* R = S + __umul24((unsigned)r, ss);
            blur_u3 v;
            v.x = __builtin_amdgcn_perm(*reinterpret_cast<const uint32_t*>(R + bc[0].a1), *reinterpret_cast<const uint32_t*>(R + bc[0].a0), bc[0].sel);
            v.y = __builtin_amdgcn_perm(*reinterpret_cast<const uint32_t*>(R + bc[1].a1), *reinterpret_cast<const uint32_t*>(R + bc[1].a0), bc[1].sel);
            v.z = __builtin_amdgcn_perm(*reinterpret_cast<const uint32_t*>(R + bc[2].a1), *reinterpret_cast<const uint32_t*>(R + bc[2].a0), bc[2].sel);
            return v;
        }
        return *reinterpret_cast<const blur_u3*>(S + __umul24((unsigned)r, ss));
    };
    auto rowpass = [&](const blur_u3 v, uint32_t* o) {
        o[0] = __builtin_amdgcn_udot4(__builtin_amdgcn_alignbyte(v.z, v.y, 1), TB, __builtin_amdgcn_udot4(__builtin_amdgcn_alignbyte(v.y, v.x, 1), TA, 0u, false), false);
        o[1] = __builtin_amdgcn_udot4(__builtin_amdgcn_alignbyte(v.z, v.y, 2), TB, __builtin_amdgcn_udot4(__builtin_amdgcn_alignbyte(v.y, v.x, 2), TA, 0u, false), false);
        o[2] = __builtin_amdgcn_udot4(__builtin_amdgcn_alignbyte(v.z, v.y, 3), TB, __builtin_amdgcn_udot4(__builtin_amdgcn_alignbyte(v.y, v.x, 3), TA, 0u, false), false);
        o[3] = __builtin_amdgcn_udot4(v.z, TB, __builtin_amdgcn_udot4(v.y, TA, 0u, false), false);
    };
    uint32_t P0[4] = {0, 0, 0, 0}, P1[4] = {0, 0, 0, 0}, P2[4] = {0, 0, 0, 0}, P3[4];
    blur_u3 va = fetch(2 * p0), vb = fetch(2 * p0 + 1), va1 = fetch(2 * p0 + 2), vb1 = fetch(2 * p0 + 3), va2 = fetch(2 * p0 + 4), vb2 = fetch(2 * p0 + 5);
#pragma unroll 4
    for (int p = p0; p <= p1; ++p) {
        const blur_u3 ca = va, cb = vb;
        va = va1; vb = vb1; va1 = va2; vb1 = vb2;
        va2 = fetch(2 * p + 6); vb2 = fetch(2 * p + 7);
        uint32_t oa[4], ob[4];
        rowpass(ca, oa); rowpass(cb, ob);
#pragma unroll
        for (int j = 0; j < 4; ++j) P3[j] = oa[j] | (ob[j] << 16);
        const int ya = 2 * p - 3, yb = 2 * p - 2;
#define BLUR_OUT(k0, k1, k2, k3, j) min((udot2(P3[j], k3, udot2(P2[j], k2, udot2(P1[j], k1, udot2(P0[j], k0, 1u << 15)))) >> 16), 255u)
        if (ya >= by0 && ya <= ylast)
            *reinterpret_cast<uint32_t*>(D + __umul24((unsigned)ya, ds)) = BLUR_OUT(kA0, kA1, kA2, kA3, 0) | (BLUR_OUT(kA0, kA1, kA2, kA3, 1) << 8) | (BLUR_OUT(kA0, kA1, kA2, kA3, 2) << 16) | (BLUR_OUT(kA0, kA1, kA2, kA3, 3) << 24);
        if (yb >= by0 && yb <= ylast)
            *reinterpret_cast<uint32_t*>(D + __umul24((unsigned)yb, ds)) = BLUR_OUT(kB0, kB1, kB2, kB3, 0) | (BLUR_OUT(kB0, kB1, kB2, kB3, 1) << 8) | (BLUR_OUT(kB0, kB1, kB2, kB3, 2) << 16) | (BLUR_OUT(kB0, kB1, kB2, kB3, 3) << 24);
#undef BLUR_OUT
#pragma unroll
        for (int j = 0; j < 4; ++j) { P0[j] = P1[j]; P1[j] = P2[j]; P2[j] = P3[j]; }
    }
}

__constant__ __attribute__((aligned(16))) signed char c_pattern[SLAMIT_ORB_PATTERN_INTS];
#define DESC_KP_PER_WAVE 4
#define DESC_R 18
#define DESC_ROWS (2 * DESC_R + 1)
#define DESC_PITCH 48
#define DESC_LOADS 2

__global__ __launch_bounds__(256) void describe_kernel(
    const OrbLevel* __restrict__ levels, int nlevels,
    const uint8_t* __restrict__ blur,
    const OrbLevelKp* __restrict__ lkp, size_t kp_frame_stride, const int* __restrict__ kp_count,
    slamit_kp* __restrict__ out_kps, uint8_t* __restrict__ out_desc, int out_cap,
    int* __restrict__ out_n, int xcd_frames , int kblocks) {
    const int lane = threadIdx.x & 63;
    int level, frame, kb;
    if (xcd_frames) {
        const unsigned w = blockIdx.x, k = w >> 3, P = (unsigned)(nlevels * kblocks), fq = k / P, local = k - fq * P;
        frame = (int)(8u * fq + ((w + fq) & 7u));
        if (frame >= xcd_frames) return;
        level = (int)(local / (unsigned)kblocks); kb = (int)(local - (unsigned)level * (unsigned)kblocks);
    } else { level = blockIdx.y; frame = blockIdx.z; kb = blockIdx.x; }
    const int i0 = (kb * 4 + (threadIdx.x >> 6)) * DESC_KP_PER_WAVE;
    const OrbLevel& L = levels[level];
    const int* counts = kp_count + frame * nlevels;
    int offset = 0, total = 0;
    for (int l = 0; l < nlevels; ++l) {
        int c = counts[l];
        if (l < level) offset += c;
        total += c;
    }
    if (level == 0 && i0 == 0 && lane == 0) out_n[frame] = min(total, out_cap);
    const int count = counts[level];
    if (i0 >= count) return;
    const int4 pw = reinterpret_cast<const int4*>(c_pattern)[lane];
    const int pt[4] = {pw.x, pw.y, pw.z, pw.w};
    float px0[4], py0[4], px1[4], py1[4];
#pragma unroll
    for (int t = 0; t < 4; ++t) {
        px0[t] = (float)(signed char)(pt[t] & 0xFF); py0[t] = (float)(signed char)((pt[t] >> 8) & 0xFF);
        px1[t] = (float)(signed char)((pt[t] >> 16) & 0xFF); py1[t] = (float)(signed char)((pt[t] >> 24) & 0xFF);
    }
    const uint8_t* img = blur + L.blur_off + (size_t)frame * L.blur_bytes;
    const unsigned step = (unsigned)L.stride;
    const OrbLevelKp* KP = lkp + L.kp_off + (size_t)frame * kp_frame_stride;
    OrbLevelKp kp[DESC_KP_PER_WAVE];
#pragma unroll
    for (int k = 0; k < DESC_KP_PER_WAVE; ++k) kp[k] = KP[min(i0 + k, count - 1)];
    __shared__ __attribute__((aligned(16))) uint8_t s_patch[4][DESC_KP_PER_WAVE][DESC_ROWS * DESC_PITCH];
    const int wv = threadIdx.x >> 6;
    int lrow[DESC_LOADS], lcol[DESC_LOADS];
    unsigned poff[DESC_LOADS];
#pragma unroll
    for (int it = 0; it < DESC_LOADS; ++it) {
        const int idx = lane + 64 * it;
        lrow[it] = (int)(((unsigned)idx * 21846u) >> 16);
        lcol[it] = idx - 3 * lrow[it];
        poff[it] = __umul24((unsigned)min(lrow[it], DESC_ROWS - 1), step) + 16u * (unsigned)lcol[it];
    }
    const __amdgpu_buffer_rsrc_t rsrc = __builtin_amdgcn_make_buffer_rsrc(const_cast<uint8_t*>(img), 0, (unsigned)L.stride * (unsigned)L.h, 0x00020000);
    typedef unsigned desc_u4 __attribute__((ext_vector_type(4)));
    desc_u4 ld[DESC_KP_PER_WAVE][DESC_LOADS];
#pragma unroll
    for (int k = 0; k < DESC_KP_PER_WAVE; ++k) {
        const unsigned base = __umul24((unsigned)(kp[k].y - DESC_R), step) + (unsigned)((kp[k].x - DESC_R) & ~3);
#pragma unroll
        for (int it = 0; it < DESC_LOADS; ++it) ld[k][it] = __builtin_amdgcn_raw_buffer_load_b128(rsrc, (int)(base + poff[it]), 0, 0);
    }
#pragma unroll
    for (int k = 0; k < DESC_KP_PER_WAVE; ++k)
#pragma unroll
        for (int it = 0; it < DESC_LOADS; ++it)
            if (lrow[it] < DESC_ROWS) *reinterpret_cast<desc_u4*>(&s_patch[wv][k][__mul24(lrow[it], DESC_PITCH) + 16 * lcol[it]]) = ld[k][it];
    __builtin_amdgcn_fence(__ATOMIC_ACQ_REL, "wavefront");
    __builtin_amdgcn_wave_barrier();
    typedef float desc_f2 __attribute__((ext_vector_type(2)));
    const desc_f2 magic = {12582912.0f, 12582912.0f};
    const unsigned DESC_BIAS = 0x400000u * (unsigned)DESC_PITCH + 0x4B400000u;
    int tv0[DESC_KP_PER_WAVE][4], tv1[DESC_KP_PER_WAVE][4];
#pragma unroll
    for (int k = 0; k < DESC_KP_PER_WAVE; ++k) {
        const float a = kp[k].cs, b = kp[k].sn;
        const desc_f2 ba = {b, a}, anb = {a, -b};
        const uint8_t* center = &s_patch[wv][k][DESC_R * DESC_PITCH + DESC_R + ((kp[k].x - DESC_R) & 3)];
        const uint8_t* biased = center - DESC_BIAS;
#pragma unroll
        for (int t = 0; t < 4; ++t) {
            const desc_f2 p0 = {px0[t], px0[t]}, q0 = {py0[t], py0[t]}, p1 = {px1[t], px1[t]}, q1 = {py1[t], py1[t]};
            const desc_f2 m0 = (p0 * ba + q0 * anb) + magic, m1 = (p1 * ba + q1 * anb) + magic;
            tv0[k][t] = biased[__umul24(__float_as_uint(m0.x), (unsigned)DESC_PITCH) + __float_as_uint(m0.y)];
            tv1[k][t] = biased[__umul24(__float_as_uint(m1.x), (unsigned)DESC_PITCH) + __float_as_uint(m1.y)];
        }
    }
#pragma unroll
    for (int k = 0; k < DESC_KP_PER_WAVE; ++k) {
        const int i = i0 + k, o = offset + i;
        unsigned nib = 0;
#pragma unroll
// ... 9 lines not shown
            kk.x = fx; kk.y = fy; kk.size = L.patch_size; kk.angle = kp[k].angle; kk.response = kp[k].response;
            kk.octave = level; kk.class_id = -1;
            out_kps[(size_t)frame * out_cap + o] = kk;
        }
    }
}

__global__ __launch_bounds__(256) void pad_level_kernel(const uint8_t* __restrict__ src, int w, int h,
                                                        size_t sstride, uint8_t* __restrict__ dst) {
    const int B = SLAMIT_EDGE_THRESHOLD;
    const int pw = w + 2 * B, ph = h + 2 * B;
    int x = blockIdx.x * 64 + (threadIdx.x & 63), y = blockIdx.y * 4 + (threadIdx.x >> 6);
    if (x >= pw || y >= ph) return;
    dst[(size_t)y * pw + x] = src[(size_t)reflect101(y - B, h) * sstride + reflect101(x - B, w)];
}

__global__ void decode_candidates_kernel(const OrbLevel* __restrict__ levels, int level,
                                         const unsigned long long* __restrict__ K, int n,
                                         unsigned long long* __restrict__ order_out, int* __restrict__ xys) {
    int k = blockIdx.x * blockDim.x + threadIdx.x;
    if (k >= n) return;
    const OrbLevel& L = levels[level];
    unsigned long long c = K[k];
    unsigned order = (unsigned)c;
    int lx = order & 63, ly = (order >> 6) & 63, cell = order >> 12;
    int ci = cell / L.nCols, cj = cell - ci * L.nCols;
    xys[3 * k + 0] = cj * L.wCell + lx;
    xys[3 * k + 1] = ci * L.hCell + ly;
    xys[3 * k + 2] = (int)(c >> 32);
    order_out[k] = order;
}

extern "C++" {

hipError_t orbk_upload_pattern(hipStream_t st) {
    static const DiscTable disc = make_disc();
    hipError_t e = hipMemcpyToSymbolAsync(HIP_SYMBOL(c_disc), &disc, sizeof(disc), 0, hipMemcpyHostToDevice, st);
    if (e != hipSuccess) return e;
    return hipMemcpyToSymbolAsync(HIP_SYMBOL(c_pattern), slamit_orb_pattern, SLAMIT_ORB_PATTERN_INTS, 0,
                                  hipMemcpyHostToDevice, st);
}

void orbk_resize(hipStream_t st, const uint8_t* src, int sw, int sh, size_t sstride, size_t sframe,
                 uint8_t* dst, int dw, int dh, size_t dstride, size_t dframe, const int* xofs,
                 const short* ialpha, const int* yofs, const short* ibeta, int nframes) {
    dim3 grid((dw + 255) / 256, (dh + 3) / 4, nframes);
    hipLaunchKernelGGL(resize_level_kernel, grid, dim3(256), 0, st, src, sw, sh, sstride, sframe, dst, dw,
                       dh, dstride, dframe, xofs, ialpha, yofs, ibeta);
}

hipError_t orbk_pyramid_prepare(int smem_bytes) {
    return hipFuncSetAttribute(reinterpret_cast<const void*>(pyramid_fused_kernel),
                               hipFuncAttributeMaxDynamicSharedMemorySize, smem_bytes);
}

void orbk_pyramid(hipStream_t st, const OrbLevel* levels, int nlevels, const PyrBox* boxes, const PyrTabs* tabs,
                  int nregions, const uint8_t* img0, size_t img0_stride, size_t img0_frame, uint8_t* pyr, int bufA_bytes,
                  int smem_bytes, int nframes, int l_first, int l_last) {
    hipLaunchKernelGGL(pyramid_fused_kernel, dim3(nregions, nframes), dim3(PYR_THREADS), smem_bytes, st, levels, nlevels, boxes,
                       tabs, img0, img0_stride, img0_frame, pyr, bufA_bytes, l_first, l_last);
}

#ifndef FAST_PS
#define FAST_PS 48
#define FAST_PL 80
#endif
static int fast_pitch(int max_wcell) { return max_wcell + 11 <= FAST_PS ? FAST_PS : FAST_PL; }

size_t orbk_fast_smem(int max_wcell, int max_hcell) {
    const int P = fast_pitch(max_wcell);
    const int tile_rows = max_hcell + 6, sc_rows = max_hcell + 2;
    const int kp_cap = ((max_wcell + 1) / 2) * ((max_hcell + 1) / 2);
    return (size_t)4 * fast_wave_bytes(P, tile_rows, sc_rows, kp_cap);
}

hipError_t orbk_fast_prepare(int max_wcell, int max_hcell) {
    const int smem = (int)orbk_fast_smem(max_wcell, max_hcell);
    hipError_t e;
    if (fast_pitch(max_wcell) == FAST_PS) {
        e = hipFuncSetAttribute(reinterpret_cast<const void*>(fast_cells_kernel<FAST_PS>), hipFuncAttributeMaxDynamicSharedMemorySize, smem);
    } else {
        e = hipFuncSetAttribute(reinterpret_cast<const void*>(fast_cells_kernel<FAST_PL>), hipFuncAttributeMaxDynamicSharedMemorySize, smem);
    }
    return e;
}

void orbk_fast(hipStream_t st, const FastTab& tab, int nlevels, const uint32_t* d_cells, int cells_per_frame,
               const uint8_t* img0, size_t img0_stride, size_t img0_frame, const uint8_t* pyr,
               unsigned long long* cand, size_t cand_frame_stride, int* cand_count, int iniTh, int minTh,
               int max_wcell, int max_hcell, int nframes) {
    const int tile_rows = max_hcell + 6, sc_rows = max_hcell + 2;
    const int kp_cap = ((max_wcell + 1) / 2) * ((max_hcell + 1) / 2);
    const int wpb = cells_per_frame < 1600 ? 1 : 4;
    const int xcd_frames = nframes >= 16 ? nframes : 0;
    const dim3 grid = xcd_frames ? dim3((unsigned)(((nframes + 7) / 8) * 8) * (unsigned)((cells_per_frame + wpb - 1) / wpb))
                                 : dim3(wpb == 1 ? (unsigned)((cells_per_frame + 31) & ~31) : (unsigned)((cells_per_frame + wpb - 1) / wpb), nframes);
    const size_t smem = orbk_fast_smem(max_wcell, max_hcell) / 4 * wpb;
    if (fast_pitch(max_wcell) == FAST_PS)
        hipLaunchKernelGGL(fast_cells_kernel<FAST_PS>, grid, dim3(64 * wpb), smem, st, tab, reinterpret_cast<const uint4*>(d_cells), nlevels, cells_per_frame, img0,
                           (unsigned)img0_stride, img0_frame, pyr, cand, cand_frame_stride, cand_count, iniTh, minTh, tile_rows,
                           sc_rows, kp_cap, xcd_frames);
    else
        hipLaunchKernelGGL(fast_cells_kernel<FAST_PL>, grid, dim3(64 * wpb), smem, st, tab, reinterpret_cast<const uint4*>(d_cells), nlevels, cells_per_frame, img0,
                           (unsigned)img0_stride, img0_frame, pyr, cand, cand_frame_stride, cand_count, iniTh, minTh, tile_rows,
                           sc_rows, kp_cap, xcd_frames);
}

hipError_t orbk_octree_prepare(int node_cap, int key_cap) {
    static int prepared = 0;
    const int want = (int)orbk_octree_smem(node_cap, key_cap);
    if (want <= prepared) return hipSuccess;
    prepared = want;
    hipError_t e = hipFuncSetAttribute(reinterpret_cast<const void*>(octree_kernel<256>), hipFuncAttributeMaxDynamicSharedMemorySize, want);
    if (e != hipSuccess) return e;
    e = hipFuncSetAttribute(reinterpret_cast<const void*>(octree_kernel<OCT_THREADS>), hipFuncAttributeMaxDynamicSharedMemorySize, want);
    if (e != hipSuccess) return e;
    return hipFuncSetAttribute(reinterpret_cast<const void*>(octree_kernel<1024>), hipFuncAttributeMaxDynamicSharedMemorySize, want);
}

void orbk_octree(hipStream_t st, const OrbLevel* levels, int nlevels, const unsigned long long* cand,
                 size_t cand_frame_stride, int* cand_count, uint32_t* ws_xy, uint16_t* ws_node,
                 OrbLevelKp* lkp, size_t kp_frame_stride, int* kp_count, int node_cap, int key_cap, int nframes,
                 int level_override) {
    dim3 grid(nframes, level_override >= 0 ? 1 : nlevels);
    const int nt = nframes >= 96 ? 256 : nframes <= 16 ? 1024 : OCT_THREADS;
    if (nframes >= 96) key_cap = std::min(key_cap, 2048);
    if (nt == 1024)
        hipLaunchKernelGGL(octree_kernel<1024>, grid, dim3(1024), orbk_octree_smem(node_cap, key_cap), st, levels, nlevels, cand,
                           cand_frame_stride, cand_count, ws_xy, ws_node, lkp, kp_frame_stride, kp_count, node_cap,
                           key_cap, level_override);
    else if (nt == 256)
        hipLaunchKernelGGL(octree_kernel<256>, grid, dim3(256), orbk_octree_smem(node_cap, key_cap), st, levels, nlevels, cand,
                           cand_frame_stride, cand_count, ws_xy, ws_node, lkp, kp_frame_stride, kp_count, node_cap,
                           key_cap, level_override);
    else
        hipLaunchKernelGGL(octree_kernel<OCT_THREADS>, grid, dim3(OCT_THREADS), orbk_octree_smem(node_cap, key_cap), st, levels, nlevels, cand,
                           cand_frame_stride, cand_count, ws_xy, ws_node, lkp, kp_frame_stride, kp_count, node_cap,
                           key_cap, level_override);
}

void orbk_ic_angle(hipStream_t st, const OrbLevel* levels, int nlevels, const uint8_t* img0,
                   size_t img0_stride, size_t img0_frame, const uint8_t* pyr, OrbLevelKp* lkp,
                   size_t kp_frame_stride, const int* kp_count, int max_kp, int nframes) {
    const int kblocks = (max_kp + 4 * IC_KP_PER_WAVE - 1) / (4 * IC_KP_PER_WAVE);
    if (nframes >= 16)
        hipLaunchKernelGGL(ic_angle_kernel, dim3((unsigned)(((nframes + 7) / 8) * 8 * nlevels * kblocks)), dim3(256), 0, st, levels,
                           nlevels, img0, img0_stride, img0_frame, pyr, lkp, kp_frame_stride, kp_count, nframes, kblocks);
    else
        hipLaunchKernelGGL(ic_angle_kernel, dim3(kblocks, nlevels, nframes), dim3(256), 0, st, levels,
                           nlevels, img0, img0_stride, img0_frame, pyr, lkp, kp_frame_stride, kp_count, 0, kblocks);
}

void orbk_blur_stream(hipStream_t st, const OrbLevel* levels, const uint32_t* d_tiles, int ntiles, const uint8_t* img0,
                      size_t img0_stride, size_t img0_frame, const uint8_t* pyr, uint8_t* blur, int nframes, bool edge) {
    if (ntiles <= 0) return;
    if (edge)
        hipLaunchKernelGGL(blur_stream_kernel<true>, dim3((ntiles + 15) / 16, nframes), dim3(256), 0, st, levels, reinterpret_cast<const uint4*>(d_tiles), img0,
                           img0_stride, img0_frame, pyr, blur, (unsigned)ntiles);
    else
        hipLaunchKernelGGL(blur_stream_kernel<false>, dim3((ntiles + 15) / 16, nframes), dim3(256), 0, st, levels, reinterpret_cast<const uint4*>(d_tiles), img0,
                           img0_stride, img0_frame, pyr, blur, (unsigned)ntiles);
}

void orbk_blur(hipStream_t st, const OrbLevel* levels, const uint32_t* d_tiles, int total_tiles, const uint8_t* img0,
               size_t img0_stride, size_t img0_frame, const uint8_t* pyr, uint8_t* blur, int nframes) {
    if (total_tiles <= 0) return;
    const unsigned total = (unsigned)total_tiles * (unsigned)nframes, grid = ((total + 7u) >> 3) << 3;
    const unsigned inv = (unsigned)((0x100000000ull + (unsigned)total_tiles - 1) / (unsigned)total_tiles);
    hipLaunchKernelGGL(blur_all_kernel, dim3(grid), dim3(256), 0, st, levels, reinterpret_cast<const uint4*>(d_tiles), img0,
                       img0_stride, img0_frame, pyr, blur, (unsigned)total_tiles, inv, total);
}

void orbk_describe(hipStream_t st, const OrbLevel* levels, int nlevels, const uint8_t* blur,
                   const OrbLevelKp* lkp, size_t kp_frame_stride, const int* kp_count, slamit_kp* out_kps,
                   uint8_t* out_desc, int out_cap, int* out_n, int max_kp, int nframes) {
    const int kblocks = (max_kp + 4 * DESC_KP_PER_WAVE - 1) / (4 * DESC_KP_PER_WAVE);
    if (nframes >= 16)
        hipLaunchKernelGGL(describe_kernel, dim3((unsigned)(((nframes + 7) / 8) * 8 * nlevels * kblocks)), dim3(256), 0, st, levels,
                           nlevels, blur, lkp, kp_frame_stride, kp_count, out_kps, out_desc, out_cap, out_n, nframes, kblocks);
    else
        hipLaunchKernelGGL(describe_kernel, dim3(kblocks, nlevels, nframes), dim3(256), 0, st, levels,
                           nlevels, blur, lkp, kp_frame_stride, kp_count, out_kps, out_desc, out_cap, out_n, 0, kblocks);
}

void orbk_pad(hipStream_t st, const uint8_t* src, int w, int h, size_t sstride, uint8_t* dst) {
    hipLaunchKernelGGL(pad_level_kernel, dim3((w + 38 + 63) / 64, (h + 38 + 3) / 4), dim3(256), 0, st, src, w, h,
                       sstride, dst);
}

void orbk_decode_candidates(hipStream_t st, const OrbLevel* levels, int level, const unsigned long long* K,
                            int n, unsigned long long* order_out, int* xys) {
    if (n <= 0) return;
    hipLaunchKernelGGL(decode_candidates_kernel, dim3((n + 255) / 256), dim3(256), 0, st, levels, level, K, n,
                       order_out, xys);
}

}
```

weiner_slamit_v2_amd/csrc/orb_plan.cc:

```cpp
#include "orb_plan.h"

#include <math.h>
#include <string.h>

#include <algorithm>

namespace {

inline int cv_round(double v) { return (int)lrint(v); }
inline size_t round_up(size_t v, size_t a) { return (v + a - 1) / a * a; }

inline short sat_short(float v) {
    int iv = cv_round((double)v);
    return (short)(iv < -32768 ? -32768 : iv > 32767 ? 32767 : iv);
}

void plan_scales(const slamit_orb_params& p, OrbPlan& P) {
    const int nl = p.nlevels;
    const double scaleFactor = (double)p.scale_factor;
    P.scale.assign(nl, 1.f); P.sigma2.assign(nl, 1.f); P.inv_scale.assign(nl, 1.f); P.inv_sigma2.assign(nl, 1.f);
    for (int i = 1; i < nl; ++i) {
        P.scale[i] = (float)(P.scale[i - 1] * scaleFactor);
        P.sigma2[i] = P.scale[i] * P.scale[i];
    }
    for (int i = 0; i < nl; ++i) { P.inv_scale[i] = 1.0f / P.scale[i]; P.inv_sigma2[i] = 1.0f / P.sigma2[i]; }
    P.per_level.assign(nl, 0);
    float factor = (float)(1.0f / scaleFactor);
    float nDesired = p.nfeatures * (1 - factor) / (1 - (float)pow((double)factor, (double)nl));
    int sum = 0;
    for (int l = 0; l < nl - 1; ++l) {
        P.per_level[l] = cv_round(nDesired);
        sum += P.per_level[l];
        nDesired *= factor;
    }
    P.per_level[nl - 1] = std::max(p.nfeatures - sum, 0);
}

bool plan_levels(const slamit_orb_params& p, OrbPlan& P, const char** why) {
    const int nl = p.nlevels;
    size_t pyr_off = 0, blur_off = 0, cand_off = 0;
    int kp_off = 0, cell_base = 0, sum_cap = 0;
    P.levels.assign(nl, OrbLevel());
    for (int l = 0; l < nl; ++l) {
        OrbLevel& L = P.levels[l];
        float sc = P.inv_scale[l];
        L.w = cv_round((float)p.width * sc);
        L.h = cv_round((float)p.height * sc);
        L.stride = (int)round_up((size_t)std::max(L.w, 1), 64);
        L.quota = P.per_level[l];
        const size_t plane = (size_t)L.stride * std::max(L.h, 1);
        L.plane_off = l >= 1 ? pyr_off : 0;
        if (l >= 1) pyr_off += round_up(plane, 256);
        L.blur_off = blur_off; blur_off += round_up(plane, 256);
        L.maxBorderX = L.w - ORB_MIN_BORDER; L.maxBorderY = L.h - ORB_MIN_BORDER;
        const float width = (float)(L.maxBorderX - ORB_MIN_BORDER), height = (float)(L.maxBorderY - ORB_MIN_BORDER);
        L.nCols = (int)(width / 30.f); L.nRows = (int)(height / 30.f);
        if (L.w < 1 || L.h < 1 || L.nCols < 1 || L.nRows < 1) {
            *why = "slamit_orb_create: pyramid level smaller than one 30x30 FAST cell";
            return false;
        }
        L.wCell = (int)ceil(width / L.nCols); L.hCell = (int)ceil(height / L.nRows);
        L.cell_base = cell_base; L.ncells = L.nCols * L.nRows; cell_base += L.ncells;
        P.max_wcell = std::max(P.max_wcell, L.wCell); P.max_hcell = std::max(P.max_hcell, L.hCell);
        L.cand_cap = L.ncells * ((L.wCell + 1) / 2) * ((L.hCell + 1) / 2);
        L.cand_off = cand_off; cand_off += round_up((size_t)L.cand_cap, 64);
        const int bw = L.maxBorderX - ORB_MIN_BORDER, bh = L.maxBorderY - ORB_MIN_BORDER;
        L.nIni = (int)round(static_cast<float>(bw) / bh);
        if (L.nIni < 1 || L.nIni > ORB_MAX_ROOTS) {
            *why = "slamit_orb_create: unsupported aspect ratio (octree roots)";
            return false;
        }
        L.hX = static_cast<float>(bw) / L.nIni;
        for (int i = 0; i < L.nIni; ++i) {
            L.rootUL[i] = (int)(L.hX * static_cast<float>(i));
            L.rootUR[i] = (int)(L.hX * static_cast<float>(i + 1));
        }
        L.boxH = bh;
        L.kp_cap = std::max(L.quota, 4 * L.nIni) + 4;
        L.kp_off = kp_off; kp_off += L.kp_cap;
        L.scale = P.scale[l];
        L.patch_size = (float)(int)(31 * P.scale[l]);
        P.node_cap = std::max(P.node_cap, L.kp_cap);
        P.max_kp_level = std::max(P.max_kp_level, L.kp_cap);
        sum_cap += L.kp_cap;
    }
    for (OrbLevel& L : P.levels) { L.plane_bytes = pyr_off; L.blur_bytes = blur_off; }
    P.max_out = std::max(P.max_out, sum_cap);
    P.pyr_frame_total = pyr_off; P.blur_frame_total = blur_off;
    P.cand_frame_stride = cand_off; P.kp_frame_stride = (size_t)kp_off;
    return true;
}

int octree_key_cap(int node_cap, int width, int height) {
    long budget = (long)width * height <= 640L * 480L * 3 / 2 ? 48L * 1024 : (long)OCT_LDS_BUDGET;
    const long room = budget - (long)orbk_octree_node_bytes(node_cap);
    return (int)std::min<long>(OCT_LDS_KEYS_MAX, std::max<long>(OCT_LDS_KEYS_MIN, room / 6)) & ~7;
}

void fast_cells(OrbPlan& P) {
    auto magic = [](int g) { return (uint32_t)((1u << 20) / (unsigned)std::max(g, 1) + 1u); };
    for (int l = 0; l < (int)P.levels.size(); ++l) {
        const OrbLevel& L = P.levels[l];
        for (int c = 0; c < L.ncells; ++c) {
            const int ci = c / L.nCols, cj = c - ci * L.nCols;
            const int iniX = ORB_MIN_BORDER + cj * L.wCell, iniY = ORB_MIN_BORDER + ci * L.hCell;
            if (iniY >= L.maxBorderY - 3 || iniX >= L.maxBorderX - 6) continue;
            const int cw = std::min(L.wCell + 6, L.maxBorderX - iniX), ch = std::min(L.hCell + 6, L.maxBorderY - iniY);
            const int sw = cw - 6, sh = ch - 6;
            if (sw <= 0 || sh <= 0) continue;
            const uint32_t w[4] = {(uint32_t)l | ((uint32_t)c << 8), (uint32_t)iniX | ((uint32_t)iniY << 16),
                                   (uint32_t)cw | ((uint32_t)ch << 8), magic((sw + 3) >> 2)};
            P.cells.insert(P.cells.end(), w, w + 4);
        }
        FastLevel& D = P.fast.lv[l];
        D.cell_base = L.cell_base; D.nCols = L.nCols; D.wCell = L.wCell; D.hCell = L.hCell;
        D.maxBorderX = L.maxBorderX; D.maxBorderY = L.maxBorderY; D.stride = L.stride; D.cand_cap = L.cand_cap;
        D.plane_off = L.plane_off; D.plane_bytes = L.plane_bytes; D.cand_off = L.cand_off;
    }
}

void blur_strips(OrbPlan& P) {
    const int nl = (int)P.levels.size();
    for (int l = 0; l < nl; ++l) {
        OrbLevel& L = P.levels[l];
        L.blur_tile_base = (int)(P.blur_all.tab.size() / 4);
        for (int by = 0; by < L.h; by += ORB_BLUR_STRIP_H)
            for (int bx = 0; bx < L.w; bx += 64) {
                const uint32_t t[4] = {(uint32_t)l, (uint32_t)bx, (uint32_t)by, 0u};
                const bool inside = bx >= 4 && bx + 68 <= L.w && (L.stride & 3) == 0;
                for (OrbStrips* S : {&P.blur_all, inside ? &P.blur_str : &P.blur_edge}) S->tab.insert(S->tab.end(), t, t + 4);
            }
        for (OrbStrips* S : {&P.blur_all, &P.blur_str, &P.blur_edge}) S->base[l + 1] = (int)(S->tab.size() / 4);
    }
}

void resize_axis(int dn, int sn, bool clampx, std::vector<int32_t>& ofs, std::vector<int16_t>& coef) {
    double inv_scale = (double)dn / sn;
    double scale = 1. / inv_scale;
    ofs.resize(dn);
    coef.resize(2 * (size_t)dn);
    for (int d = 0; d < dn; ++d) {
        float f = (float)((d + 0.5) * scale - 0.5);
        int s = (int)floor(f);
        f -= s;
        if (clampx) {
            if (s < 0) { f = 0; s = 0; }
            if (s >= sn - 1) { f = 0; s = sn - 1; }
        }
        ofs[d] = s;
        coef[2 * d] = sat_short((1.f - f) * 2048.f);
        coef[2 * d + 1] = sat_short(f * 2048.f);
    }
}

bool rows4_tables(int dw, int dh, int sw, int sh, const int* xofs, const short* ialpha, const int* yofs,
                  const short* ibeta, std::vector<uint32_t>& col, std::vector<uint32_t>& row) {
    const int ng = (dw + 3) / 4, row_end = (sw + 3) & ~3;
    if (sw >= 65536 || sh >= 65536) return false;
    col.assign((size_t)ng * 12, 0u);
    for (int g = 0; g < ng; ++g) {
        int L[4], R[4];
        uint32_t a[4];
        for (int j = 0; j < 4; ++j) {
            const int x = 4 * g + j;
            if (x < dw) {
                L[j] = xofs[x]; R[j] = std::min(xofs[x] + 1, sw - 1);
                a[j] = (uint32_t)(unsigned short)ialpha[2 * x] | ((uint32_t)(unsigned short)ialpha[2 * x + 1] << 16);
            } else { L[j] = L[0]; R[j] = L[0]; a[j] = 0; }
        }
        const int base = L[0] & ~3, s = L[0] & 3;
        const int off1 = base + 8 <= row_end ? 4 : 0, off2 = base + 12 <= row_end ? 8 : off1;
        uint32_t* c = &col[(size_t)g * 12];
        c[0] = (uint32_t)base | ((uint32_t)s << 16) | ((uint32_t)off1 << 20) | ((uint32_t)off2 << 24);
        for (int j = 0; j < 4; ++j) {
            if (L[j] < L[0] || R[j] < L[0] || L[j] - L[0] > 7 || R[j] - L[0] > 7 || ialpha[0] < 0) return false;
            c[1 + j] = (uint32_t)(L[j] - L[0]) | 0x0C00u | ((uint32_t)(R[j] - L[0]) << 16) | 0x0C000000u;
            c[5 + j] = a[j];
        }
    }
    row.assign((size_t)(dh + 7) * 2, 0u);
    for (int y = 0; y < dh; ++y) {
        const int sy0 = std::min(std::max(yofs[y], 0), sh - 1), sy1 = std::min(std::max(yofs[y] + 1, 0), sh - 1);
        row[2 * (size_t)y] = (uint32_t)sy0 | ((uint32_t)sy1 << 16);
        row[2 * (size_t)y + 1] = (uint32_t)(unsigned short)ibeta[2 * y] | ((uint32_t)(unsigned short)ibeta[2 * y + 1] << 16);
        if (ibeta[2 * y] < 0 || ibeta[2 * y + 1] < 0) return false;
    }
    for (int y = dh; y < dh + 7; ++y) { row[2 * (size_t)y] = row[2 * (size_t)(dh - 1)]; row[2 * (size_t)y + 1] = row[2 * (size_t)(dh - 1) + 1]; }
    for (int x = 0; x < dw; ++x) if (ialpha[2 * x] < 0 || ialpha[2 * x + 1] < 0) return false;
    return true;
}

bool rows8_table(int dw, int sw, size_t dstride, const int* xofs, const short* ialpha, std::vector<uint32_t>& col) {
    const int ng = (dw + 7) / 8;
    if (sw >= 65536 || (size_t)ng * 8 > dstride) return false;
    col.assign((size_t)ng * 20, 0u);
    for (int g = 0; g < ng; ++g) {
        int L[8], R[8];
        uint32_t a[8];
        const int L0 = xofs[8 * g];
        for (int j = 0; j < 8; ++j) {
            const int x = 8 * g + j;
            if (x < dw) {
                L[j] = xofs[x]; R[j] = std::min(xofs[x] + 1, sw - 1);
                if (ialpha[2 * x] < 0 || ialpha[2 * x + 1] < 0) return false;
                a[j] = (uint32_t)(unsigned short)ialpha[2 * x] | ((uint32_t)(unsigned short)ialpha[2 * x + 1] << 16);
            } else { L[j] = R[j] = L0 + (j >= 4 ? 4 : 0); a[j] = 0; }
        }
        uint32_t* c = &col[(size_t)g * 20];
        c[0] = (uint32_t)(L0 & ~3) | ((uint32_t)(L0 & 3) << 16);
        for (int j = 0; j < 8; ++j) {
            const int lo = j >= 4 ? 4 : 0;
            const int bl = L[j] - L0 - lo, br = R[j] - L0 - lo;
            if (bl < 0 || bl > 7 || br < 0 || br > 7) return false;
            c[1 + j] = (uint32_t)bl | 0x0C00u | ((uint32_t)br << 16) | 0x0C000000u;
            c[9 + j] = a[j];
        }
    }
    return true;
}

void plan_resize(const OrbPlanOptions& o, OrbPlan& P) {
    const int nl = (int)P.levels.size();
    P.rs.assign(nl, OrbResizeTabs());
    for (int l = 1; l < nl; ++l) {
        const OrbLevel &S = P.levels[l - 1], &D = P.levels[l];
        OrbResizeTabs& T = P.rs[l];
        resize_axis(D.w, S.w, true, T.xofs, T.ialpha);
        resize_axis(D.h, S.h, false, T.yofs, T.ibeta);
        if (!rows4_tables(D.w, D.h, S.w, S.h, T.xofs.data(), T.ialpha.data(), T.yofs.data(), T.ibeta.data(), T.col4, T.row4)) {
            P.rows4_ok = false;
            T.col4.clear(); T.row4.clear();
        }
        if (o.resize_no8 || !rows8_table(D.w, S.w, (size_t)D.stride, T.xofs.data(), T.ialpha.data(), T.col8)) T.col8.clear();
    }
}

void plan_pyramid_boxes(const slamit_orb_params& p, OrbPlan& P) {
    const int nl = (int)P.levels.size(), last = nl - 1;
    if (nl < 2) return;
    const int GX = std::max(1, (p.width + 127) / 128), GY = std::max(1, (p.height + 95) / 96);
    std::vector<PyrBox> boxes((size_t)GX * GY * nl);
    bool ok = true;
    size_t capA = 16, capB = 16;
    for (int gy = 0; gy < GY && ok; ++gy)
        for (int gx = 0; gx < GX && ok; ++gx) {
            PyrBox* B = &boxes[((size_t)gy * GX + gx) * nl];
            for (int l = 0; l <= last; ++l) {
                const OrbLevel& L = P.levels[l];
                B[l].ox0 = (int16_t)((long)gx * L.w / GX); B[l].ox1 = (int16_t)((long)(gx + 1) * L.w / GX);
                B[l].oy0 = (int16_t)((long)gy * L.h / GY); B[l].oy1 = (int16_t)((long)(gy + 1) * L.h / GY);
                if (l == 0) { B[l].ox0 = B[l].ox1 = B[l].oy0 = B[l].oy1 = 0; }
                else if (B[l].ox1 <= B[l].ox0 || B[l].oy1 <= B[l].oy0) ok = false;
            }
            B[last].nx0 = B[last].ox0; B[last].nx1 = B[last].ox1;
            B[last].ny0 = B[last].oy0; B[last].ny1 = B[last].oy1;
            for (int l = last; l > 0 && ok; --l) {
                const std::vector<int32_t> &XO = P.rs[l].xofs, &YO = P.rs[l].yofs;
                const int sw = P.levels[l - 1].w, sh = P.levels[l - 1].h;
                int sx0 = XO[B[l].nx0], sx1 = std::min(XO[B[l].nx1 - 1] + 1, sw - 1) + 1;
                int sy0 = std::min(std::max(YO[B[l].ny0], 0), sh - 1);
                int sy1 = std::min(std::max(YO[B[l].ny1 - 1] + 1, 0), sh - 1) + 1;
                if (l - 1 > 0) {
                    sx0 = std::min(sx0, (int)B[l - 1].ox0); sx1 = std::max(sx1, (int)B[l - 1].ox1);
                    sy0 = std::min(sy0, (int)B[l - 1].oy0); sy1 = std::max(sy1, (int)B[l - 1].oy1);
                }
                if (l - 1 == 0) sx0 &= ~3;
                B[l - 1].nx0 = (int16_t)sx0; B[l - 1].nx1 = (int16_t)sx1; B[l - 1].ny0 = (int16_t)sy0; B[l - 1].ny1 = (int16_t)sy1;
            }
            for (int l = 0; l <= last; ++l) {
                if (l > 0 && (B[l].nx1 - B[l].nx0 > 256 || B[l].ny1 - B[l].ny0 > 256)) ok = false;
                size_t bytes = (size_t)(((B[l].nx1 - B[l].nx0) + 3) & ~3) * (B[l].ny1 - B[l].ny0);
                if (l & 1) capB = std::max(capB, bytes); else capA = std::max(capA, bytes);
            }
        }
    const int bufA = (int)round_up(capA, 16), smem = bufA + (int)round_up(capB, 16);
    if (!ok || smem > 150 * 1024) return;
    P.pyr_regions = GX * GY;
    P.pyr_bufA = bufA;
    P.pyr_smem = smem;
    P.boxes.swap(boxes);
}

#ifndef ORB_BAND_COUNT
#define ORB_BAND_COUNT 8
#define ORB_BAND_SPLIT 2
#endif

inline int band_pitch(int w) { return (int)round_up((size_t)((w + 7) / 8) * 8, 16); }

void plan_bands(OrbPlan& P) {
    const int nl = (int)P.levels.size();
    if (nl < 2 || !P.rows4_ok) return;
    for (int l = 1; l < nl; ++l) {
        const OrbResizeTabs& T = P.rs[l];
        if (T.col8.empty() || T.row4.empty() || P.levels[l].h >= 65536) return;
        BandLevel& V = P.band_tab.lv[l];
        V.ngroups = (P.levels[l].w + 7) / 8;
        V.inv_groups = (uint32_t)((0x100000000ull + (unsigned)V.ngroups - 1) / (unsigned)V.ngroups);
        V.dstride = P.levels[l].stride;
        V.pitch = band_pitch(P.levels[l].w);
        V.plane_off = P.levels[l].plane_off;
    }
    const int split = ORB_BAND_SPLIT > 0 && ORB_BAND_SPLIT < nl - 1 ? ORB_BAND_SPLIT : nl - 1;
    std::vector<OrbBandSeg> segs;
    for (int first = 0; first < nl - 1; first = segs.back().last) {
        segs.emplace_back();
        int nb = ORB_BAND_COUNT;
        while (!orb_plan_band_segment(P, first, first == 0 ? split : nl - 1, nb, ORB_BAND_LDS_BUDGET, segs.back()))
            if ((nb *= 2) > 8 * ORB_BAND_COUNT) return;
    }
    P.bands.swap(segs);
}

void plan_table_block(OrbPlan& P) {
    size_t off = 0;
    auto take = [&](size_t bytes) { const size_t at = round_up(off, 256); off = at + bytes; return at; };
    const int nl = (int)P.levels.size();
    P.levels_off = take(sizeof(OrbLevel) * nl);
    P.cells_off = take(sizeof(uint32_t) * P.cells.size());
    for (OrbStrips* S : {&P.blur_all, &P.blur_str, &P.blur_edge}) S->off = take(sizeof(uint32_t) * S->tab.size());
    for (int l = 1; l < nl; ++l) {
        OrbResizeTabs& T = P.rs[l];
        T.xofs_off = take(sizeof(int32_t) * T.xofs.size()); T.ialpha_off = take(sizeof(int16_t) * T.ialpha.size());
        T.yofs_off = take(sizeof(int32_t) * T.yofs.size()); T.ibeta_off = take(sizeof(int16_t) * T.ibeta.size());
        T.col4_off = take(sizeof(uint32_t) * T.col4.size()); T.row4_off = take(sizeof(uint32_t) * T.row4.size());
        T.col8_off = take(sizeof(uint32_t) * T.col8.size());
    }
    P.boxes_off = take(sizeof(PyrBox) * P.boxes.size());
    P.tabs_off = take(P.pyr_regions ? sizeof(PyrTabs) * nl : 0);
    for (OrbBandSeg& G : P.bands) G.rows_off = take(sizeof(BandRows) * G.rows.size());
    if (!P.bands.empty())
        for (int l = 1; l < nl; ++l) { P.band_tab.lv[l].col_off = P.rs[l].col8_off; P.band_tab.lv[l].row_off = P.rs[l].row4_off; }
    P.table_bytes = round_up(off, 256);
}

}

bool orb_plan(const slamit_orb_params& p, const OrbPlanOptions& o, OrbPlan& plan, const char** why) {
    plan = OrbPlan();
    OrbPlan& P = plan;
    P.node_cap = 8; P.max_kp_level = 1;
    P.rows4_ok = true;
    plan_scales(p, P);
    P.max_out = p.nfeatures + 3 * p.nlevels;
    const bool empty = p.width == 0 || p.height == 0;
    if (!empty && !plan_levels(p, P, why)) return false;
    P.oct_key_cap = octree_key_cap(P.node_cap, p.width, p.height);
    if (orbk_octree_smem(P.node_cap, P.oct_key_cap) > 160 * 1024 - 1024 || P.node_cap >= 4096) {
        *why = "slamit_orb_create: nfeatures too large for the LDS octree";
        return false;
    }
    fast_cells(P);
    blur_strips(P);
    plan_resize(o, P);
    plan_pyramid_boxes(p, P);
    plan_bands(P);
    plan_table_block(P);
    return true;
}

bool orb_plan_band_segment(const OrbPlan& P, int first, int last, int nbands, size_t lds_budget, OrbBandSeg& seg) {
    const int nl = (int)P.levels.size(), nlv = last - first;
    if (first < 0 || last >= nl || nlv < 1 || nbands < 1) return false;
    seg = OrbBandSeg();
    seg.first = first; seg.last = last; seg.nbands = nbands;
    seg.rows.assign((size_t)nbands * nlv, BandRows());
    size_t tile[2] = {0, 0};
    for (int b = 0; b < nbands; ++b) {
        BandRows* R = &seg.rows[(size_t)b * nlv];
        int need0 = 0, need1 = 0;
        for (int l = last; l > first; --l) {
            const int h = P.levels[l].h;
            if (h < nbands || h >= 65536 || P.rs[l].row4.size() < 2 * (size_t)h) return false;
            const int own0 = (int)((long)b * h / nbands), own1 = (int)((long)(b + 1) * h / nbands);
            const int cmp0 = l == last ? own0 : std::min(own0, need0), cmp1 = l == last ? own1 : std::max(own1, need1);
            R[l - first - 1] = BandRows{(uint16_t)own0, (uint16_t)own1, (uint16_t)cmp0, (uint16_t)cmp1};
            need0 = 65535; need1 = 0;
            for (int y = cmp0; y < cmp1; ++y) {
                const uint32_t s = P.rs[l].row4[2 * (size_t)y];
                need0 = std::min(need0, (int)(s & 0xFFFFu)); need1 = std::max(need1, (int)(s >> 16) + 1);
            }
            if (l < last) {
                size_t& t = tile[(l - first - 1) & 1];
                t = std::max(t, (size_t)(cmp1 - cmp0) * band_pitch(P.levels[l].w) + ORB_BAND_SLACK);
            }
        }
    }
    seg.tile0 = (int)round_up(tile[0], 16);
    seg.smem = seg.tile0 + (int)round_up(tile[1], 16);
    return (size_t)seg.smem <= lds_budget;
}

void orb_plan_image(const OrbPlan& P, const uint8_t* base, std::vector<uint8_t>& img) {
    img.assign(P.table_bytes, 0);
    auto put = [&](size_t off, const void* src, size_t bytes) { if (bytes) memcpy(img.data() + off, src, bytes); };
    auto put_vec = [&](size_t off, const auto& v) { put(off, v.data(), sizeof(v[0]) * v.size()); };
    put(P.levels_off, P.levels.data(), sizeof(OrbLevel) * P.levels.size());
    put_vec(P.cells_off, P.cells);
    for (const OrbStrips* S : {&P.blur_all, &P.blur_str, &P.blur_edge}) put_vec(S->off, S->tab);
    for (size_t l = 1; l < P.rs.size(); ++l) {
        const OrbResizeTabs& T = P.rs[l];
        put_vec(T.xofs_off, T.xofs); put_vec(T.ialpha_off, T.ialpha); put_vec(T.yofs_off, T.yofs); put_vec(T.ibeta_off, T.ibeta);
        put_vec(T.col4_off, T.col4); put_vec(T.row4_off, T.row4); put_vec(T.col8_off, T.col8);
    }
    put_vec(P.boxes_off, P.boxes);
    for (const OrbBandSeg& G : P.bands) put_vec(G.rows_off, G.rows);
    if (!P.pyr_regions) return;
    std::vector<PyrTabs> tabs(P.levels.size(), PyrTabs{nullptr, nullptr, nullptr, nullptr});
    auto at = [&](size_t off) { return (uintptr_t)base + off; };
    for (size_t l = 1; l < tabs.size(); ++l) {
        const OrbResizeTabs& T = P.rs[l];
        tabs[l].xofs = reinterpret_cast<const int32_t*>(at(T.xofs_off)); tabs[l].ialpha = reinterpret_cast<const int16_t*>(at(T.ialpha_off));
        tabs[l].yofs = reinterpret_cast<const int32_t*>(at(T.yofs_off)); tabs[l].ibeta = reinterpret_cast<const int16_t*>(at(T.ibeta_off));
    }
    put_vec(P.tabs_off, tabs);
}
```

weiner_slamit_v2_amd/csrc/orb_plan.h:

```cpp
#ifndef SLAMIT_ORB_PLAN_H
#define SLAMIT_ORB_PLAN_H

#include <stddef.h>
#include <stdint.h>

#include <vector>

#include "../../include/slamit.h"
#include "orb_types.h"

struct OrbPlanOptions {
    bool resize_no8;
};

struct OrbStrips {
    std::vector<uint32_t> tab;
    int base[ORB_MAX_LEVELS + 1];
    size_t off;
};

struct OrbResizeTabs {
    std::vector<int32_t> xofs, yofs;
    std::vector<int16_t> ialpha, ibeta;
    std::vector<uint32_t> col4, row4;
    std::vector<uint32_t> col8;
    size_t xofs_off, ialpha_off, yofs_off, ibeta_off, col4_off, row4_off, col8_off;
};

struct OrbBandSeg {
    int first, last, nbands;
    std::vector<BandRows> rows;
    int tile0, smem;
    size_t rows_off;
};

struct OrbPlan {
    std::vector<float> scale, inv_scale, sigma2, inv_sigma2;
    std::vector<int> per_level;
    std::vector<OrbLevel> levels;
    size_t pyr_frame_total, blur_frame_total, cand_frame_stride, kp_frame_stride;
    int max_out, node_cap, oct_key_cap, max_kp_level, max_wcell, max_hcell;
    std::vector<uint32_t> cells;
    size_t cells_off;
    FastTab fast;
    OrbStrips blur_all, blur_str, blur_edge;
    std::vector<OrbResizeTabs> rs;
    bool rows4_ok;
    int pyr_regions, pyr_bufA, pyr_smem;
    std::vector<PyrBox> boxes;
    size_t levels_off, boxes_off, tabs_off;
    std::vector<OrbBandSeg> bands;
    BandTab band_tab;
    size_t table_bytes;
};

bool orb_plan(const slamit_orb_params& p, const OrbPlanOptions& o, OrbPlan& plan, const char** why);

bool orb_plan_band_segment(const OrbPlan& plan, int first, int last, int nbands, size_t lds_budget, OrbBandSeg& seg);

void orb_plan_image(const OrbPlan& plan, const uint8_t* base, std::vector<uint8_t>& img);

#endif
```

weiner_slamit_v2_amd/csrc/orb_types.h:

```cpp
#ifndef SLAMIT_ORB_TYPES_H
#define SLAMIT_ORB_TYPES_H

#include <stddef.h>
#include <stdint.h>

#ifdef __HIPCC__
#define ORB_HD __host__ __device__
#else
#define ORB_HD
#endif

#define ORB_MAX_LEVELS 16
#define ORB_MAX_ROOTS 8
#define ORB_MIN_BORDER 16
#define ORB_CELL_MAX 59
#define ORB_TILE_MAX (ORB_CELL_MAX + 6)
#define ORB_CC_PAD 32
#define BLUR_STEPS 4
#define ORB_BLUR_STRIP_H (16 * BLUR_STEPS)

ORB_HD inline size_t orbk_octree_node_bytes(int node_cap) {
    return ((size_t)node_cap * (8 + 2 * 8 + 2 * 4 + 4 * 4 + 5 * 4 + 4 + 4) + 64 + 15) & ~(size_t)15;
}
ORB_HD inline size_t orbk_octree_smem(int node_cap, int key_cap) { return orbk_octree_node_bytes(node_cap) + (size_t)key_cap * 6; }
#define OCT_LDS_KEYS_MAX 10240
#define OCT_LDS_KEYS_MIN 2048
#define OCT_LDS_BUDGET (78 * 1024)

struct OrbLevel {
    int32_t w, h;
    int32_t stride;
    int32_t quota;
    uint64_t plane_off;
    uint64_t plane_bytes;
    uint64_t blur_off;
    uint64_t blur_bytes;
    int32_t nCols, nRows, wCell, hCell;
    int32_t maxBorderX, maxBorderY;
    int32_t cell_base;
    int32_t ncells;
    int32_t blur_tile_base;
    uint64_t cand_off;
    int32_t cand_cap;
    int32_t nIni;
    float hX;
    int32_t rootUL[ORB_MAX_ROOTS], rootUR[ORB_MAX_ROOTS];
    int32_t boxH;
    int32_t kp_off, kp_cap;
    float scale;
    float patch_size;
};

struct FastLevel {
    int32_t cell_base, nCols, wCell, hCell, maxBorderX, maxBorderY, stride, cand_cap;
    uint64_t plane_off, plane_bytes, cand_off;
};
struct FastTab { FastLevel lv[ORB_MAX_LEVELS]; };

struct PyrBox {
    int16_t ox0, oy0, ox1, oy1;
    int16_t nx0, ny0, nx1, ny1;
};
struct PyrTabs {
    const int32_t* xofs; const int16_t* ialpha;
    const int32_t* yofs; const int16_t* ibeta;
};

struct BandLevel {
    uint64_t col_off, row_off;
    uint64_t plane_off;
    int32_t ngroups, dstride, pitch;
    uint32_t inv_groups;
};
struct BandTab { BandLevel lv[ORB_MAX_LEVELS]; };
struct BandRows { uint16_t own0, own1, cmp0, cmp1; };
#define ORB_BAND_LDS_BUDGET (78 * 1024)
#define ORB_BAND_SLACK 16

struct OrbLevelKp {
    int16_t x, y;
    float response;
    float angle;
    float cs, sn;
};

#endif
```

Before: 315,900 frames/s.

## Write reflect-border pads in pyramid resize so blur treats padded levels as interior

The pyramid resize kernels now write reflected border bytes just outside each row, to the left and right, using byte permutes. On levels where those pads fit within the stride, the blur stream kernel can use the cheaper interior path for strips that previously needed the edge-handling variant. The plan builds separate pad-aware strip tables and checks that pad writes will not overwrite neighbouring planes, and the pyramid allocation gains a leading slack region. The cost is extra neighbour shuffles and a recomputed group in resize, plus more complex planning, with a risk of subtle border correctness bugs.

```diff
diff --git a/include/slamit.h b/include/slamit.h
--- a/include/slamit.h
+++ b/include/slamit.h
@@ -70,6 +70,8 @@
                                 int* n_out);
 int slamit_orb_debug_blurred(slamit_orb* h, int frame, int level, uint8_t* dst, size_t dst_bytes, int* w,
                              int* h_out);
+int slamit_orb_debug_plane(slamit_orb* h, int frame, int level, uint8_t* dst, size_t dst_bytes, int* w, int* h_out,
+                           int* stride, int* padded);
 
 
 #define SLAMIT_HAMMING_MAX_TRAIN 65535
diff --git a/weiner_slamit_v2_amd/api.py b/weiner_slamit_v2_amd/api.py
--- a/weiner_slamit_v2_amd/api.py
+++ b/weiner_slamit_v2_amd/api.py
@@ -194,7 +194,7 @@
 EXPORTS = [
     "slamit_orb_create", "slamit_orb_destroy", "slamit_orb_tables", "slamit_orb_max_keypoints",
     "slamit_orb_extract", "slamit_orb_extract_batch", "slamit_orb_extract_batch_dev", "slamit_orb_level",
-    "slamit_orb_debug_candidates", "slamit_orb_debug_blurred", "slamit_orb_profile", "slamit_hamming_best2", "slamit_hamming_best2_batch_dev",
+    "slamit_orb_debug_candidates", "slamit_orb_debug_blurred", "slamit_orb_debug_plane", "slamit_orb_profile", "slamit_hamming_best2", "slamit_hamming_best2_batch_dev",
     "slamit_hamming_matrix", "slamit_distinctive_batch", "slamit_guided_search", "slamit_guided_search_workspace", "slamit_guided_search_batch_dev", "slamit_bow_search", "slamit_voc_create", "slamit_voc_load_text", "slamit_voc_destroy", "slamit_voc_info",
     "slamit_voc_transform", "slamit_voc_transform_workspace", "slamit_voc_transform_batch_dev",
     "slamit_kfdb_create", "slamit_kfdb_destroy", "slamit_kfdb_clear", "slamit_kfdb_info", "slamit_kfdb_add", "slamit_kfdb_add_dev", "slamit_kfdb_erase",
@@ -227,6 +227,7 @@
         L.slamit_orb_extract_batch_dev.argtypes = [vp, vp, sz, sz, i32, vp, vp, i32, vp, vp]
         L.slamit_orb_level.argtypes = [vp, i32, i32, vp, sz, vp, vp]
         L.slamit_orb_debug_blurred.argtypes = [vp, i32, i32, vp, sz, vp, vp]
+        L.slamit_orb_debug_plane.argtypes = [vp, i32, i32, vp, sz, vp, vp, vp, vp]
         L.slamit_orb_profile.argtypes = [vp, i32, vp, vp, i32]
         L.slamit_orb_debug_candidates.argtypes = [vp, i32, i32, vp, i32, vp]
         L.slamit_hamming_best2.argtypes = [vp, i32, vp, i32, vp, vp, vp]
@@ -419,6 +420,14 @@
                "slamit_orb_debug_blurred")
         return out
 
+    def plane(self, frame, level):
+        w, h, st, pd = C.c_int(), C.c_int(), C.c_int(), C.c_int()
+        args = (C.byref(w), C.byref(h), C.byref(st), C.byref(pd))
+        _check(lib().slamit_orb_debug_plane(self._h, frame, level, None, 0, *args), "slamit_orb_debug_plane")
+        out = np.zeros(4 + st.value * h.value, np.uint8)
+        _check(lib().slamit_orb_debug_plane(self._h, frame, level, _np_ptr(out), out.size, *args), "slamit_orb_debug_plane")
+        return out[:4], out[4:].reshape(h.value, st.value), w.value, bool(pd.value)
+
     def debug_candidates(self, frame, level):
         n = C.c_int()
         _check(lib().slamit_orb_debug_candidates(self._h, frame, level, None, 0, C.byref(n)), "debug_candidates")
diff --git a/weiner_slamit_v2_amd/csrc/orb_api.hip b/weiner_slamit_v2_amd/csrc/orb_api.hip
--- a/weiner_slamit_v2_amd/csrc/orb_api.hip
+++ b/weiner_slamit_v2_amd/csrc/orb_api.hip
@@ -16,9 +16,9 @@
                  uint8_t* dst, int dw, int dh, size_t dstride, size_t dframe, const int* xofs,
                  const short* ialpha, const int* yofs, const short* ibeta, int nframes);
 void orbk_resize_rows4(hipStream_t st, const uint8_t* src, size_t sstride, size_t sframe, int sh, uint8_t* dst, int dw, int dh,
-                       size_t dstride, size_t dframe, const uint32_t* d_col, const uint32_t* d_row, int nframes);
+                       size_t dstride, size_t dframe, const uint32_t* d_col, const uint32_t* d_row, int nframes, bool pads);
 void orbk_resize_rows8(hipStream_t st, const uint8_t* src, size_t sstride, size_t sframe, int sh, uint8_t* dst, int dw, int dh,
-                       size_t dstride, size_t dframe, const uint32_t* d_col8, const uint32_t* d_row, int nframes);
+                       size_t dstride, size_t dframe, const uint32_t* d_col8, const uint32_t* d_row, int nframes, bool pads);
 hipError_t orbk_pyramid_bands_prepare(int smem_bytes);
 void orbk_pyramid_bands(hipStream_t st, const BandTab& tab, const uint8_t* d_tables, const BandRows* d_rows, int first, int last, int nbands,
                         const uint8_t* src, size_t sstride, size_t sframe, int sh, uint8_t* pyr, size_t pyr_frame, int tile0, int smem, int nframes);
@@ -39,7 +39,7 @@
                    size_t img0_frame, const uint8_t* pyr, OrbLevelKp* lkp, size_t kp_frame_stride,
                    const int* kp_count, int max_kp, int nframes);
 void orbk_blur_stream(hipStream_t st, const OrbLevel* levels, const uint32_t* d_tiles, int ntiles, const uint8_t* img0,
-                      size_t img0_stride, size_t img0_frame, const uint8_t* pyr, uint8_t* blur, int nframes, bool edge);
+                      size_t img0_stride, size_t img0_frame, const uint8_t* pyr, uint8_t* blur, int nframes, bool edge, bool pads);
 void orbk_blur(hipStream_t st, const OrbLevel* levels, const uint32_t* d_tiles, int total_tiles, const uint8_t* img0,
                size_t img0_stride, size_t img0_frame, const uint8_t* pyr, uint8_t* blur, int nframes);
 void orbk_describe(hipStream_t st, const OrbLevel* levels, int nlevels, const uint8_t* blur,
@@ -92,6 +92,7 @@
     const uint8_t* last_img0;
     size_t last_stride, last_frame;
     int last_nframes;
+    bool last_pads;
 };
 
 template <typename T>
@@ -100,7 +101,7 @@
 static void orb_free(slamit_orb* h) {
     if (!h) return;
     SlamitDeviceGuard guard(h->device);
-    hipFree(h->d_tables); hipFree(h->d_pyr); hipFree(h->d_blur); hipFree(h->d_cand); hipFree(h->d_ws_xy);
+    hipFree(h->d_tables); if (h->d_pyr) hipFree(h->d_pyr - ORB_PYR_LEAD); hipFree(h->d_blur); hipFree(h->d_cand); hipFree(h->d_ws_xy);
     hipFree(h->d_ws_node); hipFree(h->d_counts); hipFree(h->d_lkp); hipFree(h->d_in); hipFree(h->d_out_kps);
     hipFree(h->d_out_desc); hipFree(h->d_out_n); if (h->h_out) hipHostFree(h->h_out); hipFree(h->d_scratch);
     for (hipEvent_t e : h->prof_ev) hipEventDestroy(e);
@@ -145,7 +146,8 @@
     hipError_t e = hipSuccess;
 #define ALLOC(ptr, bytes) if (e == hipSuccess) e = hipMalloc((void**)&(ptr), std::max<size_t>((bytes), 256))
     ALLOC(h->d_tables, P.table_bytes);
-    ALLOC(h->d_pyr, P.pyr_frame_total * B);
+    ALLOC(h->d_pyr, P.pyr_frame_total * B + ORB_PYR_LEAD);
+    if (e == hipSuccess) h->d_pyr += ORB_PYR_LEAD;
     ALLOC(h->d_blur, P.blur_frame_total * B + 256);
     ALLOC(h->d_cand, sizeof(unsigned long long) * P.cand_frame_stride * B);
     ALLOC(h->d_ws_xy, sizeof(uint32_t) * P.cand_frame_stride * B);
@@ -238,12 +240,14 @@
     if (!h->counters_clean) HIP_TRY(hipMemsetAsync(h->d_counts, 0, sizeof(int) * (size_t)h->p.max_batch * nl * ORB_CC_PAD, st));
     h->counters_clean = false;
     const bool blur_src_aligned = ((((uintptr_t)d_gray) | stride | frame_stride) & 3) == 0;
+    const bool pads = P.pads_ok && blur_src_aligned && (!P.bands.empty() || P.rows4_ok);
     auto launch_blur = [&](hipStream_t bs, int l0, int l1) {
         auto strips = [&](const OrbStrips& S) { return dtab<uint32_t>(h, S.off) + 4 * (size_t)S.base[l0]; };
         auto nstrips = [&](const OrbStrips& S) { return S.base[l1] - S.base[l0]; };
         if (h->blur_stream_on && blur_src_aligned) {
-            orbk_blur_stream(bs, h->d_levels, strips(P.blur_str), nstrips(P.blur_str), d_gray, stride, frame_stride, h->d_pyr, h->d_blur, nframes, false);
-            orbk_blur_stream(bs, h->d_levels, strips(P.blur_edge), nstrips(P.blur_edge), d_gray, stride, frame_stride, h->d_pyr, h->d_blur, nframes, true);
+            const OrbStrips &SI = pads ? P.blur_str_pad : P.blur_str, &SE = pads ? P.blur_edge_pad : P.blur_edge;
+            orbk_blur_stream(bs, h->d_levels, strips(SI), nstrips(SI), d_gray, stride, frame_stride, h->d_pyr, h->d_blur, nframes, false, pads);
+            orbk_blur_stream(bs, h->d_levels, strips(SE), nstrips(SE), d_gray, stride, frame_stride, h->d_pyr, h->d_blur, nframes, true, false);
         } else {
             orbk_blur(bs, h->d_levels, strips(P.blur_all), nstrips(P.blur_all), d_gray, stride, frame_stride, h->d_pyr, h->d_blur, nframes);
         }
@@ -278,11 +282,11 @@
             if (!T.col8.empty())
                 orbk_resize_rows8(st, src, l == 1 ? stride : (size_t)S.stride, l == 1 ? frame_stride : P.pyr_frame_total, S.h,
                                   h->d_pyr + D.plane_off, D.w, D.h, (size_t)D.stride, P.pyr_frame_total, dtab<uint32_t>(h, T.col8_off),
-                                  dtab<uint32_t>(h, T.row4_off), nframes);
+                                  dtab<uint32_t>(h, T.row4_off), nframes, pads && D.padded);
             else
                 orbk_resize_rows4(st, src, l == 1 ? stride : (size_t)S.stride, l == 1 ? frame_stride : P.pyr_frame_total, S.h,
                                   h->d_pyr + D.plane_off, D.w, D.h, (size_t)D.stride, P.pyr_frame_total, dtab<uint32_t>(h, T.col4_off),
-                                  dtab<uint32_t>(h, T.row4_off), nframes);
+                                  dtab<uint32_t>(h, T.row4_off), nframes, pads && D.padded);
             if (early_blur && l == ORB_BLUR_SPLIT) HIP_TRY(fork_early_blur(l));
         }
     } else if (P.pyr_regions) {
@@ -335,6 +339,7 @@
     HIP_TRY(hipGetLastError());
     h->counters_clean = true;
     h->last_img0 = d_gray; h->last_stride = stride; h->last_frame = frame_stride; h->last_nframes = nframes;
+    h->last_pads = pads;
     return SLAMIT_OK;
 }
 
@@ -434,6 +439,24 @@
     return SLAMIT_OK;
 }
 
+int slamit_orb_debug_plane(slamit_orb* h, int frame, int level, uint8_t* dst, size_t dst_bytes, int* w, int* h_out, int* stride, int* padded) {
+    if (!h || level < 1 || level >= h->nlevels) return slamit_fail(SLAMIT_ERR_ARG, "slamit_orb_debug_plane: bad level");
+    if (h->p.width == 0 || h->p.height == 0) return slamit_fail(SLAMIT_ERR_STATE, "slamit_orb_debug_plane: empty image");
+    const OrbLevel& L = h->pl.levels[level];
+    if (w) *w = L.w;
+    if (h_out) *h_out = L.h;
+    if (stride) *stride = L.stride;
+    if (padded) *padded = h->last_pads && L.padded;
+    if (!dst) return SLAMIT_OK;
+    if (frame < 0 || frame >= h->last_nframes) return slamit_fail(SLAMIT_ERR_STATE, "slamit_orb_debug_plane: no such frame in the last extract call");
+    const size_t need = 4 + (size_t)L.stride * L.h;
+    if (dst_bytes < need) return slamit_fail(SLAMIT_ERR_CAPACITY, "slamit_orb_debug_plane: dst too small");
+    SLAMIT_USE_DEVICE(h->device);
+    HIP_TRY(hipMemcpyAsync(dst, h->d_pyr + L.plane_off + (size_t)frame * h->pl.pyr_frame_total - 4, need, hipMemcpyDeviceToHost, h->stream));
+    HIP_TRY(hipStreamSynchronize(h->stream));
+    return SLAMIT_OK;
+}
+
 int slamit_orb_debug_candidates(slamit_orb* h, int frame, int level, int32_t* xys, int cap, int* n_out) {
     if (!h || level < 0 || level >= h->nlevels || !n_out) return slamit_fail(SLAMIT_ERR_ARG, "slamit_orb_debug_candidates: bad argument");
     if (frame < 0 || frame >= h->last_nframes) return slamit_fail(SLAMIT_ERR_STATE, "slamit_orb_debug_candidates: no such frame");
diff --git a/weiner_slamit_v2_amd/csrc/orb_kernels.hip b/weiner_slamit_v2_amd/csrc/orb_kernels.hip
--- a/weiner_slamit_v2_amd/csrc/orb_kernels.hip
+++ b/weiner_slamit_v2_amd/csrc/orb_kernels.hip
@@ -51,16 +51,29 @@
 
 #define RS_RP 2
 
+template <int N>
+__device__ __forceinline__ void rs_store_row(uint8_t* row, const unsigned goff, const uint32_t* d, const uint32_t prev, const bool first, const bool last,
+                                             const RowPads& Pd) {
+    uint32_t e[3] = {d[0], N == 2 ? d[1] : 0u, 0u};
+    if (Pd.on && last) {
+        const uint32_t cur = Pd.idx == 0 ? e[0] : Pd.idx == 1 ? e[1] : 0u, prv = Pd.idx == 0 ? prev : Pd.idx == 1 ? e[0] : e[1];
+        const uint32_t fa = __builtin_amdgcn_perm(cur, prv, Pd.selA), fb = __builtin_amdgcn_perm(cur, prv, Pd.selB);
+        if (Pd.idx == 0) { e[0] = fa; e[1] = fb; }
+        else if (Pd.idx == 1) { e[1] = fa; e[2] = fb; }
+        else e[2] = fa;
+        if (Pd.behind) *reinterpret_cast<uint32_t*>(row + goff + 4u * N) = e[N];
+    }
+    if (N == 2) *reinterpret_cast<uint2*>(row + goff) = make_uint2(e[0], e[1]);
+    else *reinterpret_cast<uint32_t*>(row + goff) = e[0];
+    if (Pd.on && first) *(reinterpret_cast<uint32_t*>(row) - 1) = __builtin_amdgcn_perm(0u, d[0], 0x0102030Cu);
+}
+
 template <int RP>
-__device__ __forceinline__ void rs_item(const int item, const uint8_t* S, const unsigned ss, const unsigned sbytes, uint8_t* D, const unsigned dstride,
-                                        const uint4* __restrict__ coltab, const uint2* __restrict__ rowtab, const int ngroups,
-                                        const unsigned inv_groups, const int dh) {
-    const int yq = (int)__umulhi((unsigned)item, inv_groups);
-    const int g = item - yq * ngroups;
+__device__ __forceinline__ void rs_group(const int g, const int yq, const uint8_t* S, const unsigned ss, const unsigned sbytes,
+                                         const uint4* __restrict__ coltab, const uint2* __restrict__ rowtab, uint32_t* outs) {
     const uint8_t* ct = reinterpret_cast<const uint8_t*>(coltab) + 48u * (unsigned)g;
     const uint4 c0 = *reinterpret_cast<const uint4*>(ct), c1 = *reinterpret_cast<const uint4*>(ct + 16u);
     const uint32_t c2x = *reinterpret_cast<const uint32_t*>(ct + 32u);
-    int yrow[2 * RP];
     uint2 rt[2 * RP];
     {
         const uint4* rp4 = reinterpret_cast<const uint4*>(reinterpret_cast<const uint8_t*>(rowtab) + 16u * (unsigned)(RP * yq));
@@ -69,8 +82,6 @@
             const uint4 v = rp4[r];
             rt[2 * r] = make_uint2(v.x, v.y); rt[2 * r + 1] = make_uint2(v.z, v.w);
         }
-#pragma unroll
-        for (int r = 0; r < 2 * RP; ++r) yrow[r] = min(2 * RP * yq + r, dh - 1);
     }
     const unsigned b = c0.x & 0xFFFFu, sh = (c0.x >> 16) & 3u, off1 = (c0.x >> 20) & 15u, off2 = (c0.x >> 24) & 15u;
     const uint32_t sel[4] = {c0.y, c0.z, c0.w, c1.x}, al[4] = {c1.y, c1.z, c1.w, c2x};
@@ -100,33 +111,47 @@
             const uint32_t v = ((__umul24(b0, h[0][j]) >> 16) + (__umul24(b1, h[1][j]) >> 16) + 2u) >> 2;
             out |= (v & 0xFFu) << (8 * j);
         }
-        *reinterpret_cast<uint32_t*>(D + (__umul24((unsigned)yrow[k], dstride) + 4u * (unsigned)g)) = out;
-    }
+        outs[k] = out;
+    }
+}
+
+template <int RP>
+__device__ __forceinline__ void rs_item(const int item, const uint8_t* S, const unsigned ss, const unsigned sbytes, uint8_t* D, const unsigned dstride,
+                                        const uint4* __restrict__ coltab, const uint2* __restrict__ rowtab, const int ngroups,
+                                        const unsigned inv_groups, const int dh, const RowPads Pd) {
+    const int yq = (int)__umulhi((unsigned)item, inv_groups);
+    const int g = item - yq * ngroups;
+    uint32_t out[2 * RP], prev[2 * RP];
+    rs_group<RP>(g, yq, S, ss, sbytes, coltab, rowtab, out);
+    const bool first = g == 0, last = g == ngroups - 1, need_prev = Pd.on && Pd.idx == 0;
+#pragma unroll
+    for (int k = 0; k < 2 * RP; ++k) prev[k] = need_prev ? (uint32_t)__shfl_up((int)out[k], 1) : 0u;
+    if (need_prev && last && (threadIdx.x & (WAVE - 1)) == 0) rs_group<RP>(g - 1, yq, S, ss, sbytes, coltab, rowtab, prev);
+#pragma unroll
+    for (int k = 0; k < 2 * RP; ++k)
+        rs_store_row<1>(D + __umul24((unsigned)min(2 * RP * yq + k, dh - 1), dstride), 4u * (unsigned)g, &out[k], prev[k], first, last, Pd);
 }
 
 template <int RP>
 __global__ __launch_bounds__(256) void resize_rows4_kernel(
     const uint8_t* __restrict__ src, size_t sstride, size_t sframe,
     uint8_t* __restrict__ dst, size_t dstride, size_t dframe,
-    const uint4* __restrict__ coltab, const uint2* __restrict__ rowtab, int ngroups, unsigned inv_groups, int nitems, int dh, unsigned sbytes) {
+    const uint4* __restrict__ coltab, const uint2* __restrict__ rowtab, int ngroups, unsigned inv_groups, int nitems, int dh, unsigned sbytes,
+    const RowPads pads) {
     const int item = blockIdx.x * 256 + threadIdx.x;
     if (item >= nitems) return;
     rs_item<RP>(item, src + (size_t)blockIdx.y * sframe, (unsigned)sstride, sbytes, dst + (size_t)blockIdx.y * dframe, (unsigned)dstride, coltab, rowtab,
-                ngroups, inv_groups, dh);
+                ngroups, inv_groups, dh, pads);
 }
 
 typedef unsigned rs_u4 __attribute__((ext_vector_type(4)));
 template <int RP>
-__device__ __forceinline__ void rs_item8(const int item, const uint8_t* S, const unsigned ss, const unsigned sbytes, uint8_t* D, const unsigned dstride,
-                                         const uint4* __restrict__ coltab, const uint2* __restrict__ rowtab, const int ngroups,
-                                         const unsigned inv_groups, const int dh) {
-    const int yq = (int)__umulhi((unsigned)item, inv_groups);
-    const int g = item - yq * ngroups;
+__device__ __forceinline__ void rs_group8(const int g, const int yq, const uint8_t* S, const unsigned ss, const unsigned sbytes,
+                                          const uint4* __restrict__ coltab, const uint2* __restrict__ rowtab, uint32_t (*outs)[2]) {
     const uint8_t* ct = reinterpret_cast<const uint8_t*>(coltab) + 80u * (unsigned)g;
     const uint4 c0 = *reinterpret_cast<const uint4*>(ct), c1 = *reinterpret_cast<const uint4*>(ct + 16u), c2 = *reinterpret_cast<const uint4*>(ct + 32u),
                 c3 = *reinterpret_cast<const uint4*>(ct + 48u);
     const uint32_t c4x = *reinterpret_cast<const uint32_t*>(ct + 64u);
-    int yrow[2 * RP];
     uint2 rt[2 * RP];
     {
         const uint4* rp4 = reinterpret_cast<const uint4*>(reinterpret_cast<const uint8_t*>(rowtab) + 16u * (unsigned)(RP * yq));
@@ -135,8 +160,6 @@
             const uint4 v = rp4[r];
             rt[2 * r] = make_uint2(v.x, v.y); rt[2 * r + 1] = make_uint2(v.z, v.w);
         }
-#pragma unroll
-        for (int r = 0; r < 2 * RP; ++r) yrow[r] = min(2 * RP * yq + r, dh - 1);
     }
     const unsigned b = c0.x & 0xFFFFu, sh = (c0.x >> 16) & 3u;
     const uint32_t sel[8] = {c0.y, c0.z, c0.w, c1.x, c1.y, c1.z, c1.w, c2.x}, al[8] = {c2.y, c2.z, c2.w, c3.x, c3.y, c3.z, c3.w, c4x};
@@ -168,57 +191,76 @@
             const uint32_t v = ((__umul24(b0, h[0][j]) >> 16) + (__umul24(b1, h[1][j]) >> 16) + 2u) >> 2;
             out[j >> 2] |= (v & 0xFFu) << (8 * (j & 3));
         }
-        *reinterpret_cast<uint2*>(D + (__umul24((unsigned)yrow[k], dstride) + 8u * (unsigned)g)) = make_uint2(out[0], out[1]);
-    }
+        outs[k][0] = out[0]; outs[k][1] = out[1];
+    }
+}
+
+template <int RP>
+__device__ __forceinline__ void rs_item8(const int item, const uint8_t* S, const unsigned ss, const unsigned sbytes, uint8_t* D, const unsigned dstride,
+                                         const uint4* __restrict__ coltab, const uint2* __restrict__ rowtab, const int ngroups,
+                                         const unsigned inv_groups, const int dh, const RowPads Pd) {
+    const int yq = (int)__umulhi((unsigned)item, inv_groups);
+    const int g = item - yq * ngroups;
+    uint32_t out[2 * RP][2], prev[2 * RP];
+    rs_group8<RP>(g, yq, S, ss, sbytes, coltab, rowtab, out);
+    const bool first = g == 0, last = g == ngroups - 1, need_prev = Pd.on && Pd.idx == 0;
+#pragma unroll
+    for (int k = 0; k < 2 * RP; ++k) prev[k] = need_prev ? (uint32_t)__shfl_up((int)out[k][1], 1) : 0u;
+    if (need_prev && last && (threadIdx.x & (WAVE - 1)) == 0) {
+        uint32_t o2[2 * RP][2];
+        rs_group8<RP>(g - 1, yq, S, ss, sbytes, coltab, rowtab, o2);
+#pragma unroll
+        for (int k = 0; k < 2 * RP; ++k) prev[k] = o2[k][1];
+    }
+#pragma unroll
+    for (int k = 0; k < 2 * RP; ++k)
+        rs_store_row<2>(D + __umul24((unsigned)min(2 * RP * yq + k, dh - 1), dstride), 8u * (unsigned)g, out[k], prev[k], first, last, Pd);
 }
 
 template <int RP>
 __global__ __launch_bounds__(256) void resize_rows8_kernel(
     const uint8_t* __restrict__ src, size_t sstride, size_t sframe,
     uint8_t* __restrict__ dst, size_t dstride, size_t dframe,
-    const uint4* __restrict__ coltab, const uint2* __restrict__ rowtab, int ngroups, unsigned inv_groups, int nitems, int dh, unsigned sbytes) {
+    const uint4* __restrict__ coltab, const uint2* __restrict__ rowtab, int ngroups, unsigned inv_groups, int nitems, int dh, unsigned sbytes,
+    const RowPads pads) {
     const int item = blockIdx.x * 256 + threadIdx.x;
     if (item >= nitems) return;
     rs_item8<RP>(item, src + (size_t)blockIdx.y * sframe, (unsigned)sstride, sbytes, dst + (size_t)blockIdx.y * dframe, (unsigned)dstride, coltab, rowtab,
-                 ngroups, inv_groups, dh);
+                 ngroups, inv_groups, dh, pads);
 }
 
 void orbk_resize_rows8(hipStream_t st, const uint8_t* src, size_t sstride, size_t sframe, int sh, uint8_t* dst, int dw, int dh,
-                       size_t dstride, size_t dframe, const uint32_t* d_col8, const uint32_t* d_row, int nframes) {
+                       size_t dstride, size_t dframe, const uint32_t* d_col8, const uint32_t* d_row, int nframes, bool pads) {
     const int ng = (dw + 7) / 8, nitems = ng * ((dh + 2 * RS_RP - 1) / (2 * RS_RP));
     const unsigned inv = (unsigned)((0x100000000ull + (unsigned)ng - 1) / (unsigned)ng);
     hipLaunchKernelGGL(resize_rows8_kernel<RS_RP>, dim3((nitems + 255) / 256, nframes), dim3(256), 0, st, src, sstride, sframe, dst, dstride, dframe,
-                       reinterpret_cast<const uint4*>(d_col8), reinterpret_cast<const uint2*>(d_row), ng, inv, nitems, dh, (unsigned)(sstride * (size_t)sh));
+                       reinterpret_cast<const uint4*>(d_col8), reinterpret_cast<const uint2*>(d_row), ng, inv, nitems, dh, (unsigned)(sstride * (size_t)sh),
+                       orb_row_pads(pads, dw, 8));
 }
 
 void orbk_resize_rows4(hipStream_t st, const uint8_t* src, size_t sstride, size_t sframe, int sh, uint8_t* dst, int dw, int dh,
-                       size_t dstride, size_t dframe, const uint32_t* d_col, const uint32_t* d_row, int nframes) {
+                       size_t dstride, size_t dframe, const uint32_t* d_col, const uint32_t* d_row, int nframes, bool pads) {
     const int ng = (dw + 3) / 4, nitems = ng * ((dh + 2 * RS_RP - 1) / (2 * RS_RP));
     const unsigned inv = (unsigned)((0x100000000ull + (unsigned)ng - 1) / (unsigned)ng);
     hipLaunchKernelGGL(resize_rows4_kernel<RS_RP>, dim3((nitems + 255) / 256, nframes), dim3(256), 0, st, src, sstride, sframe, dst, dstride, dframe,
-                       reinterpret_cast<const uint4*>(d_col), reinterpret_cast<const uint2*>(d_row), ng, inv, nitems, dh, (unsigned)(sstride * (size_t)sh));
+                       reinterpret_cast<const uint4*>(d_col), reinterpret_cast<const uint2*>(d_row), ng, inv, nitems, dh, (unsigned)(sstride * (size_t)sh),
+                       orb_row_pads(pads, dw, 4));
 }
 
 #define BAND_THREADS 256
 
-template <bool FROM_LDS, bool TO_LDS>
-__device__ __forceinline__ void band_item(const int item, const BandLevel& V, const uint8_t* __restrict__ tables, const BandRows R,
-                                          const __amdgpu_buffer_rsrc_t rsrc, const unsigned ss, const uint8_t* stile, const int srow0,
-                                          const unsigned spitch, uint8_t* dtile, uint8_t* D) {
-    const int yq = (int)__umulhi((unsigned)item, V.inv_groups);
-    const int g = item - yq * V.ngroups;
+template <bool FROM_LDS>
+__device__ __forceinline__ void band_group(const int g, const int* yrow, const BandLevel& V, const uint8_t* __restrict__ tables,
+                                           const __amdgpu_buffer_rsrc_t rsrc, const unsigned ss, const uint8_t* stile, const int srow0,
+                                           const unsigned spitch, uint32_t (*outs)[2]) {
     const uint8_t* ct = tables + V.col_off + 80u * (unsigned)g;
     const uint4 c0 = *reinterpret_cast<const uint4*>(ct), c1 = *reinterpret_cast<const uint4*>(ct + 16u), c2 = *reinterpret_cast<const uint4*>(ct + 32u),
                 c3 = *reinterpret_cast<const uint4*>(ct + 48u);
     const uint32_t c4x = *reinterpret_cast<const uint32_t*>(ct + 64u);
-    int yrow[4];
     uint2 rt[4];
     const uint8_t* rtab = tables + V.row_off;
 #pragma unroll
-    for (int r = 0; r < 4; ++r) {
-        yrow[r] = min((int)R.cmp0 + 4 * yq + r, (int)R.cmp1 - 1);
-        rt[r] = *reinterpret_cast<const uint2*>(rtab + 8u * (unsigned)yrow[r]);
-    }
+    for (int r = 0; r < 4; ++r) rt[r] = *reinterpret_cast<const uint2*>(rtab + 8u * (unsigned)yrow[r]);
     const unsigned b = c0.x & 0xFFFFu, sh = (c0.x >> 16) & 3u;
     const uint32_t sel[8] = {c0.y, c0.z, c0.w, c1.x, c1.y, c1.z, c1.w, c2.x}, al[8] = {c2.y, c2.z, c2.w, c3.x, c3.y, c3.z, c3.w, c4x};
     uint32_t w[8][4];
@@ -252,9 +294,36 @@
             const uint32_t v = ((__umul24(b0, h[0][j]) >> 16) + (__umul24(b1, h[1][j]) >> 16) + 2u) >> 2;
             out[j >> 2] |= (v & 0xFFu) << (8 * (j & 3));
         }
-        if (TO_LDS) *reinterpret_cast<uint2*>(dtile + (__umul24((unsigned)(yrow[k] - (int)R.cmp0), (unsigned)V.pitch) + 8u * (unsigned)g)) = make_uint2(out[0], out[1]);
+        outs[k][0] = out[0]; outs[k][1] = out[1];
+    }
+}
+
+template <bool FROM_LDS, bool TO_LDS>
+__device__ __forceinline__ void band_item(const int item, const BandLevel& V, const uint8_t* __restrict__ tables, const BandRows R,
+                                          const __amdgpu_buffer_rsrc_t rsrc, const unsigned ss, const uint8_t* stile, const int srow0,
+                                          const unsigned spitch, uint8_t* dtile, uint8_t* D) {
+    const int yq = (int)__umulhi((unsigned)item, V.inv_groups);
+    const int g = item - yq * V.ngroups;
+    int yrow[4];
+#pragma unroll
+    for (int r = 0; r < 4; ++r) yrow[r] = min((int)R.cmp0 + 4 * yq + r, (int)R.cmp1 - 1);
+    uint32_t out[4][2], prev[4];
+    band_group<FROM_LDS>(g, yrow, V, tables, rsrc, ss, stile, srow0, spitch, out);
+    const RowPads& Pd = V.pads;
+    const bool first = g == 0, last = g == V.ngroups - 1, need_prev = Pd.on && Pd.idx == 0;
+#pragma unroll
+    for (int k = 0; k < 4; ++k) prev[k] = need_prev ? (uint32_t)__shfl_up((int)out[k][1], 1) : 0u;
+    if (need_prev && last && (threadIdx.x & (WAVE - 1)) == 0) {
+        uint32_t o2[4][2];
+        band_group<FROM_LDS>(g - 1, yrow, V, tables, rsrc, ss, stile, srow0, spitch, o2);
+#pragma unroll
+        for (int k = 0; k < 4; ++k) prev[k] = o2[k][1];
+    }
+#pragma unroll
+    for (int k = 0; k < 4; ++k) {
+        if (TO_LDS) *reinterpret_cast<uint2*>(dtile + (__umul24((unsigned)(yrow[k] - (int)R.cmp0), (unsigned)V.pitch) + 8u * (unsigned)g)) = make_uint2(out[k][0], out[k][1]);
         if (yrow[k] >= (int)R.own0 && yrow[k] < (int)R.own1)
-            *reinterpret_cast<uint2*>(D + (__umul24((unsigned)yrow[k], (unsigned)V.dstride) + 8u * (unsigned)g)) = make_uint2(out[0], out[1]);
+            rs_store_row<2>(D + __umul24((unsigned)yrow[k], (unsigned)V.dstride), 8u * (unsigned)g, out[k], prev[k], first, last, Pd);
     }
 }
 
@@ -1445,7 +1514,7 @@
     else blur_strip<false>(in, rp, S, sstride, aligned, D, (unsigned)L.stride, w, h, bx, by0, tid);
 }
 
-template <bool EDGE>
+template <bool EDGE, bool PADS>
 __global__ __launch_bounds__(256) void blur_stream_kernel(
     const OrbLevel* __restrict__ levels, const uint4* __restrict__ tiles,
     const uint8_t* __restrict__ img0, size_t img0_stride, size_t img0_frame,
@@ -1462,7 +1531,7 @@
     unsigned ss;
     if (level == 0) { S = img0 + (size_t)frame * img0_frame; ss = (unsigned)img0_stride; }
     else { S = pyr + L.plane_off + (size_t)frame * L.plane_bytes; ss = (unsigned)L.stride; }
-    if (EDGE && x0 >= L.w) return;
+    if ((EDGE || PADS) && x0 >= L.w) return;
     BlurCol bc[3];
     if (EDGE) {
 #pragma unroll
@@ -1778,14 +1847,13 @@
 }
 
 void orbk_blur_stream(hipStream_t st, const OrbLevel* levels, const uint32_t* d_tiles, int ntiles, const uint8_t* img0,
-                      size_t img0_stride, size_t img0_frame, const uint8_t* pyr, uint8_t* blur, int nframes, bool edge) {
+                      size_t img0_stride, size_t img0_frame, const uint8_t* pyr, uint8_t* blur, int nframes, bool edge, bool pads) {
     if (ntiles <= 0) return;
-    if (edge)
-        hipLaunchKernelGGL(blur_stream_kernel<true>, dim3((ntiles + 15) / 16, nframes), dim3(256), 0, st, levels, reinterpret_cast<const uint4*>(d_tiles), img0,
-                           img0_stride, img0_frame, pyr, blur, (unsigned)ntiles);
-    else
-        hipLaunchKernelGGL(blur_stream_kernel<false>, dim3((ntiles + 15) / 16, nframes), dim3(256), 0, st, levels, reinterpret_cast<const uint4*>(d_tiles), img0,
-                           img0_stride, img0_frame, pyr, blur, (unsigned)ntiles);
+    const dim3 grid((ntiles + 15) / 16, nframes);
+    const uint4* tiles = reinterpret_cast<const uint4*>(d_tiles);
+    if (edge) hipLaunchKernelGGL((blur_stream_kernel<true, false>), grid, dim3(256), 0, st, levels, tiles, img0, img0_stride, img0_frame, pyr, blur, (unsigned)ntiles);
+    else if (pads) hipLaunchKernelGGL((blur_stream_kernel<false, true>), grid, dim3(256), 0, st, levels, tiles, img0, img0_stride, img0_frame, pyr, blur, (unsigned)ntiles);
+    else hipLaunchKernelGGL((blur_stream_kernel<false, false>), grid, dim3(256), 0, st, levels, tiles, img0, img0_stride, img0_frame, pyr, blur, (unsigned)ntiles);
 }
 
 void orbk_blur(hipStream_t st, const OrbLevel* levels, const uint32_t* d_tiles, int total_tiles, const uint8_t* img0,
diff --git a/weiner_slamit_v2_amd/csrc/orb_plan.cc b/weiner_slamit_v2_amd/csrc/orb_plan.cc
--- a/weiner_slamit_v2_amd/csrc/orb_plan.cc
+++ b/weiner_slamit_v2_amd/csrc/orb_plan.cc
@@ -47,6 +47,7 @@
         L.w = cv_round((float)p.width * sc);
         L.h = cv_round((float)p.height * sc);
         L.stride = (int)round_up((size_t)std::max(L.w, 1), 64);
+        L.padded = orb_level_padded(l, L.w, L.stride);
         L.quota = P.per_level[l];
         const size_t plane = (size_t)L.stride * std::max(L.h, 1);
         L.plane_off = l >= 1 ? pyr_off : 0;
@@ -128,10 +129,27 @@
             for (int bx = 0; bx < L.w; bx += 64) {
                 const uint32_t t[4] = {(uint32_t)l, (uint32_t)bx, (uint32_t)by, 0u};
                 const bool inside = bx >= 4 && bx + 68 <= L.w && (L.stride & 3) == 0;
-                for (OrbStrips* S : {&P.blur_all, inside ? &P.blur_str : &P.blur_edge}) S->tab.insert(S->tab.end(), t, t + 4);
-            }
-        for (OrbStrips* S : {&P.blur_all, &P.blur_str, &P.blur_edge}) S->base[l + 1] = (int)(S->tab.size() / 4);
-    }
+                const bool as_inside = inside || (L.padded && (L.stride & 3) == 0);
+                for (OrbStrips* S : {&P.blur_all, inside ? &P.blur_str : &P.blur_edge, as_inside ? &P.blur_str_pad : &P.blur_edge_pad})
+                    S->tab.insert(S->tab.end(), t, t + 4);
+            }
+        for (OrbStrips* S : {&P.blur_all, &P.blur_str, &P.blur_edge, &P.blur_str_pad, &P.blur_edge_pad}) S->base[l + 1] = (int)(S->tab.size() / 4);
+    }
+}
+
+void plan_pads(OrbPlan& P) {
+    const int nl = (int)P.levels.size();
+    bool any = false, ok = true;
+    for (int l = 1; l < nl; ++l) {
+        if (!P.levels[l].padded) continue;
+        any = true;
+        const OrbLevel& V = P.levels[l == 1 ? nl - 1 : l - 1];
+        if (l == 1 && nl == 2) continue;
+        const size_t end = (size_t)V.plane_off + (size_t)V.stride * V.h, next = l == 1 ? P.pyr_frame_total : (size_t)P.levels[l].plane_off;
+        const size_t row_free = (size_t)V.stride - round_up((size_t)V.w, 8);
+        if (!V.padded && next - end + row_free < 4) ok = false;
+    }
+    P.pads_ok = any && ok;
 }
 
 void resize_axis(int dn, int sn, bool clampx, std::vector<int32_t>& ofs, std::vector<int16_t>& coef) {
@@ -300,6 +318,7 @@
         V.dstride = P.levels[l].stride;
         V.pitch = band_pitch(P.levels[l].w);
         V.plane_off = P.levels[l].plane_off;
+        V.pads = orb_row_pads(P.pads_ok && P.levels[l].padded, P.levels[l].w, 8);
     }
     const int split = ORB_BAND_SPLIT > 0 && ORB_BAND_SPLIT < nl - 1 ? ORB_BAND_SPLIT : nl - 1;
     std::vector<OrbBandSeg> segs;
@@ -331,6 +350,7 @@
     for (OrbBandSeg& G : P.bands) G.rows_off = take(sizeof(BandRows) * G.rows.size());
     if (!P.bands.empty())
         for (int l = 1; l < nl; ++l) { P.band_tab.lv[l].col_off = P.rs[l].col8_off; P.band_tab.lv[l].row_off = P.rs[l].row4_off; }
+    for (OrbStrips* S : {&P.blur_str_pad, &P.blur_edge_pad}) S->off = take(sizeof(uint32_t) * S->tab.size());
     P.table_bytes = round_up(off, 256);
 }
 
@@ -352,6 +372,7 @@
     }
     fast_cells(P);
     blur_strips(P);
+    plan_pads(P);
     plan_resize(o, P);
     plan_pyramid_boxes(p, P);
     plan_bands(P);
@@ -397,7 +418,7 @@
     auto put_vec = [&](size_t off, const auto& v) { put(off, v.data(), sizeof(v[0]) * v.size()); };
     put(P.levels_off, P.levels.data(), sizeof(OrbLevel) * P.levels.size());
     put_vec(P.cells_off, P.cells);
-    for (const OrbStrips* S : {&P.blur_all, &P.blur_str, &P.blur_edge}) put_vec(S->off, S->tab);
+    for (const OrbStrips* S : {&P.blur_all, &P.blur_str, &P.blur_edge, &P.blur_str_pad, &P.blur_edge_pad}) put_vec(S->off, S->tab);
     for (size_t l = 1; l < P.rs.size(); ++l) {
         const OrbResizeTabs& T = P.rs[l];
         put_vec(T.xofs_off, T.xofs); put_vec(T.ialpha_off, T.ialpha); put_vec(T.yofs_off, T.yofs); put_vec(T.ibeta_off, T.ibeta);
diff --git a/weiner_slamit_v2_amd/csrc/orb_plan.h b/weiner_slamit_v2_amd/csrc/orb_plan.h
--- a/weiner_slamit_v2_amd/csrc/orb_plan.h
+++ b/weiner_slamit_v2_amd/csrc/orb_plan.h
@@ -44,6 +44,8 @@
     size_t cells_off;
     FastTab fast;
     OrbStrips blur_all, blur_str, blur_edge;
+    OrbStrips blur_str_pad, blur_edge_pad;
+    bool pads_ok;
     std::vector<OrbResizeTabs> rs;
     bool rows4_ok;
     int pyr_regions, pyr_bufA, pyr_smem;
diff --git a/weiner_slamit_v2_amd/csrc/orb_types.h b/weiner_slamit_v2_amd/csrc/orb_types.h
--- a/weiner_slamit_v2_amd/csrc/orb_types.h
+++ b/weiner_slamit_v2_amd/csrc/orb_types.h
@@ -40,6 +40,7 @@
     int32_t cell_base;
     int32_t ncells;
     int32_t blur_tile_base;
+    int32_t padded;
     uint64_t cand_off;
     int32_t cand_cap;
     int32_t nIni;
@@ -50,6 +51,34 @@
     float scale;
     float patch_size;
 };
+
+ORB_HD inline bool orb_level_padded(int level, int w, int stride) {
+#ifdef ORB_NO_PADS
+    return false;
+#endif
+    return level >= 1 && ((w + 7) / 8) * 8 + 4 <= stride && w + 3 <= stride - 4;
+}
+struct RowPads {
+    int32_t on;
+    int32_t idx, behind;
+    uint32_t selA, selB;
+};
+ORB_HD inline RowPads orb_row_pads(bool padded, int w, int group_px) {
+    RowPads R = {0, 0, 0, 0u, 0u};
+    if (!padded) return R;
+    const int r = w - (w - 1) / group_px * group_px;
+    const int rl = r & 3;
+    R.on = 1; R.idx = r >> 2;
+    for (int i = 0; i < 4; ++i) {
+        const int tA = i - rl, tB = i + 4 - rl;
+        const unsigned a = i < rl ? 4u + (unsigned)i : tA < 3 ? (unsigned)(rl + 2 - tA) : 0x0Cu;
+        const unsigned b = tB < 3 ? (unsigned)(rl + 2 - tB) : 0x0Cu;
+        R.selA |= a << (8 * i); R.selB |= b << (8 * i);
+    }
+    R.behind = R.idx * 4 + rl + 3 > group_px;
+    return R;
+}
+#define ORB_PYR_LEAD 256
 
 struct FastLevel {
     int32_t cell_base, nCols, wCell, hCell, maxBorderX, maxBorderY, stride, cand_cap;
@@ -71,6 +100,8 @@
     uint64_t plane_off;
     int32_t ngroups, dstride, pitch;
     uint32_t inv_groups;
+    RowPads pads;
+    int32_t reserved;
 };
 struct BandTab { BandLevel lv[ORB_MAX_LEVELS]; };
 struct BandRows { uint16_t own0, own1, cmp0, cmp1; };
```

Measured after the change: 314,500 frames/s. About the same (-0.4%).
